# VIS4ROB-lab/covins

Measured on AMD Instinct MI355X. Metric: GBA iterations/sec, 5-agent EuRoC merged map, higher is better.
Workload: dtype f64

## Files before the change

### covins_amd/csrc/common.hpp

```cpp
#pragma once
#include <hip/hip_runtime.h>
#include <algorithm>
#include <atomic>
#include <cstdlib>
#include <stdint.h>

#include <map>
#include <unordered_map>
#include <utility>
#include <vector>

#include "../../include/covgpu.h"
#include "batch_limits.hpp"

namespace covgpu {

constexpr int kEdgeRec = 132;
constexpr int kTile = 128;

struct DevProblem {
  int K, A, L, O, I, E, S;
  int D;
  int n;
  int npad;
// ... 29 lines not shown
  double *imu_noise;
  double *pre_delta;
  double *pre_J;
  double *pre_P;
  double *pre_W;
  double *pre_bias;
  double *imu_Jw;

  int *edge_i, *edge_j;
  double *edge_meas, *edge_sqrt_info, *edge_loss_a;

  int nchains;
  int max_chain_len;
  int* perm;
  int* pos_kf;
  int* chain_ptr;
  int* pos_chain_end;

  double* Sred;
  double* bred;
  double *Ad, *Ae;
  double *Bp, *Bs, *Bn;
  int* pos_chain_begin;
  double* bp;
  double* grad;
  double* hdiag;
  double* HllInv;
  double* gn;
  double* step;
  double* vtmp;
  double* Linv;
  double* scal;
  double* part;
  int part_n, part_imu, part_edge, part_vec;
  double *imuAd, *imuBs, *imuCd, *imuG;
  double* edgeOut;
  int *kf_edge_ptr, *kf_edge_ent;
  int nepairs;
  int *epair_ptr, *epair_i, *epair_j, *epair_ent;
  int* flag;

  int shard;
  double* vw;

  int nd, nd_nnodes, nd_nlev, nd_maxd;
  int *nd_vnode, *nd_voff, *nd_vord;
  int *nd_vown;
  int *nd_ndepth, *nd_nI;
  long long* nd_ntab;
  int* nd_abase;
  int* nd_fidx;
  double *nd_M, *nd_rhs, *nd_Linv;
  double* nd_dummy;

  double* tr;
  double* scal_r; int* flag_r;

  int uni;
  int* cam_model;
  double* cam_xi;
};

enum {
  TR_RADIUS = 0, TR_MU, TR_LMDF, TR_COST, TR_ALPHA, TR_GG, TR_GN2, TR_GDOT, TR_DNORM, TR_CG, TR_CN, TR_MODEL, TR_SN, TR_RHO, TR_COSTNEW,
  TR_OK, TR_VALID, TR_ACC, TR_TERM, TR_FNCONV, TR_RETRY, TR_FIRST, TR_INITCOST, TR_REUSE,
  TR_JA, TR_JB, TR_JC, TR_VV, TR_VG, TR_NN, TR_XN2,
  TR_COUNT = 32
};
static_assert(TR_XN2 < TR_COUNT, "trust-region state slots");
struct TrConsts {
  int strategy;
  double max_radius, min_relative_decrease, function_tolerance, parameter_tolerance, gradient_tolerance;
};

__device__ __forceinline__ double* nd_entry(const DevProblem& P, int va, int vb, int ra, int rb) {
  const int na = P.nd_vnode[va], nb = P.nd_vnode[vb];
  if (na < 0 || nb < 0) return P.nd_dummy;
  if (na == nb) {
    const int oa = P.nd_voff[va] + ra, ob = P.nd_voff[vb] + rb;
    const int hi = oa > ob ? oa : ob, lo = oa > ob ? ob : oa;
    return P.nd_M + P.nd_ntab[2 * na] + (size_t)hi * (size_t)P.nd_ntab[2 * na + 1] + lo;
  }
  const int da = P.nd_ndepth[na], db = P.nd_ndepth[nb];
  const int no = da > db ? na : nb, vo = da > db ? va : vb, ro = da > db ? ra : rb;
  const int vA = da > db ? vb : va, rA = da > db ? rb : ra, dA = da > db ? db : da;
  const int base = P.nd_abase[(size_t)no * P.nd_maxd + dA];
  const int row = base < 0 ? -1 : P.nd_fidx[base + P.nd_vord[vA]];
  if (row < 0) return P.nd_dummy;
  return P.nd_M + P.nd_ntab[2 * no] + (size_t)(row + rA) * (size_t)P.nd_ntab[2 * no + 1] + (P.nd_voff[vo] + ro);
}

__device__ __forceinline__ double* c_entry(const DevProblem& P, int pi, int pj, int r, int c) {
  if (P.nd) return nd_entry(P, 2 * pi, 2 * pj, r, c);
  return P.Sred + (size_t)(6 * pi + r) * P.npad + (6 * pj + c);
}

enum { SC_COST = 0, SC_JV2 = 1, SC_GG = 2, SC_GN2 = 3, SC_GDOT = 4, SC_GMAX = 5, SC_GS = 6, SC_SN2 = 7, SC_XN2 = 8,
       SC_VV = 9, SC_VG = 10, SC_NN = 11, SC_JA = 12, SC_JB = 13, SC_JC = 14,
       SC_COUNT = 16 };

struct CholAux;
inline bool first_use_on_device(std::atomic<unsigned long long>& seen) {
  int d = 0;
  if (hipGetDevice(&d) != hipSuccess || d < 0 || d > 63) return true;
  const unsigned long long bit = 1ull << d;
  return (seen.fetch_or(bit, std::memory_order_acq_rel) & bit) == 0;
}
struct DevSignal { long long* flag = nullptr; long long seq = 0; };
inline int env_int(const char* name, int fallback) {
  const char* e = getenv(name);
  return e != nullptr ? atoi(e) : fallback;
}
size_t pair_order_slots(int npairs);
void launch_kobs_build(const DevProblem& P, int* pair_oa, int* pair_ob, size_t nent, hipStream_t st);
void launch_lm_lin(const DevProblem& P, double mu, hipStream_t st, DevSignal sig = DevSignal());
void launch_lm_build(const DevProblem& P, double mu, hipStream_t st, hipEvent_t pose_system_cleared = nullptr, hipStream_t side = nullptr,
                     hipEvent_t ev_lin = nullptr, hipEvent_t ev_kf = nullptr, CholAux* ax = nullptr);
void launch_lm_backsub(const DevProblem& P, const double* dp, double* out_all, hipStream_t st);
void launch_obs_jvp(const DevProblem& P, const double* v_all, hipStream_t st);
void launch_obs_cost(const DevProblem& P, const double* pose, const double* lm, hipStream_t st);
void launch_obs_linearize(const DevProblem& P, double* r, double* Jp, double* Jl, double* cost, hipStream_t st);
void launch_obs_norms(const DevProblem& P, double* norms, hipStream_t st);
void launch_lm_outliers(const DevProblem& P, double th, unsigned char* erase, int* left, unsigned long long* counts, hipStream_t st);

void launch_preintegrate(const DevProblem& P, hipStream_t st);
void launch_imu_build(const DevProblem& P, hipStream_t st);
void launch_imu_jvp(const DevProblem& P, const double* v_all, hipStream_t st);
void launch_imu_cost(const DevProblem& P, const double* pose, const double* sb, hipStream_t st);
void launch_imu_linearize(const DevProblem& P, double* r, double* J, hipStream_t st);

void launch_edge_build(const DevProblem& P, hipStream_t st);
void launch_edge_jvp(const DevProblem& P, const double* v_all, hipStream_t st);
void launch_edge_cost(const DevProblem& P, const double* pose, hipStream_t st);
void launch_edge_linearize(const DevProblem& P, double* r, double* J, double* cost, hipStream_t st);

void launch_finalize_diag(const DevProblem& P, double mu, int which, hipStream_t st);
void launch_part_clear(const DevProblem& P, int slot0, int nslots, hipStream_t st);
void launch_part_finish(const DevProblem& P, int slot0, int nslots, hipStream_t st);
void launch_imu_gather(const DevProblem& P, int which, hipStream_t st);
void launch_edge_gather(const DevProblem& P, hipStream_t st);
void launch_pose_finish(const DevProblem& P, double mu, hipStream_t st);
struct PgoPlan;
void launch_pose_graph_solve(const DevProblem& P, double* dst, hipStream_t st, CholAux& ax, PgoPlan* pgo);
void launch_zero_system(const DevProblem& P, hipStream_t st);
enum KernelForm {
  KF_POTRF_PANEL = 0, KF_POTRF_PANEL_FRONTS, KF_POTRF_PANEL4, KF_POTRF_PANEL4_FRONTS, KF_POTRF_SKIPPED,
  KF_TRSM_SUB4_4, KF_TRSM_SUB4_8, KF_TRSM_SUB4_12, KF_TRSM_SUB4_16,
  KF_GEMM_TRI_FULL, KF_GEMM_TRI_QUAD, KF_GEMM_TRI_GRID, KF_GEMM_RECT_FULL, KF_GEMM_RECT_QUAD, KF_DIAG_UPDATE,
  KF_BULK_ONE_LAUNCH, KF_BULK_TWO_LAUNCHES, KF_LAST_UPDATE_WHOLE, KF_LAST_UPDATE_SPLIT, KF_PANEL_ONE_TILE, KF_KD_CUT, KF_KD_ZERO, KF_GEMM_BETA0,
  KF_BWD_FRONT, KF_BWD_PIPE, KF_BWD_PIPE64, KF_BWD_TREE, KF_BWD_TREE64, KF_BWD_GIVEN, KF_BWD_STEP_SUB,
  KF_ND_EXTEND_REC, KF_ND_EXTEND, KF_ND_EXTEND_SPLIT,
  KF_ND_TOP_PACK, KF_ND_GH, KF_ND_TOP_DAMP, KF_ND_PANEL_XFER, KF_DIST_PANEL,
  KF_PGO_ARROW, KF_PGO_DENSE,
  KF_COUNT
};
extern const char* const kFormNames[KF_COUNT];
struct FormCensus { long long n[KF_COUNT] = {}; };
extern thread_local FormCensus* t_forms;
inline void form_hit(int f, long long k = 1) { if (t_forms != nullptr) t_forms->n[f] += k; }
struct FormScope {
  FormCensus* prev;
  explicit FormScope(FormCensus* c) : prev(t_forms) { t_forms = c; }
  ~FormScope() { t_forms = prev; }
  FormScope(const FormScope&) = delete; FormScope& operator=(const FormScope&) = delete;
};
struct CholAux {
  hipStream_t aux = nullptr, mid = nullptr, head = nullptr;
  hipEvent_t ev_fill = nullptr;
  hipEvent_t ev_xb = nullptr;
  int* bwd_cnt = nullptr;
  double* bwd_scr = nullptr; size_t bwd_scr_elems = 0;
  double* bwd_pipe = nullptr; size_t bwd_pipe_elems = 0;
  bool pipe_broken = false;
  hipEvent_t ev_xa = nullptr;
  hipEvent_t ev_zero = nullptr;
  hipEvent_t ev_lin = nullptr, ev_kf = nullptr;
  std::vector<hipEvent_t> ev, prof_ev, panel_ev;
  std::vector<double> prof_flops;
  std::vector<hipEvent_t> prof_ev2;
  std::vector<double> prof_flops2;
  double potrf_ms = 0, potrf_flops = 0;
  long n_potrf = 0;
  struct TriCache {
    std::vector<int*> list; std::vector<int> count; int key = -1;
    std::vector<int*> listC; std::vector<int> countC;
    int *listA = nullptr, *listB = nullptr; int countA = 0, countB = 0;
    void clear();
  };
  FormCensus forms;
  TriCache tri0;
  std::vector<TriCache> tri_lev;
  void tri_clear();
  void (*reduce)(void* ctx, double* dev, size_t n, int op, hipStream_t st) = nullptr;
  void* reduce_ctx = nullptr;
  int panel_n = 0;
  std::vector<int> panel_tag;
  void mark(hipStream_t s, int tag);
  bool profile = false;
  double syrk_ms = 0, syrk_flops = 0;
  long n_syrk = 0;
  void init();
  void destroy();
  void collect();
  static constexpr int kGateSlots = 16384;
  bool gates_on = false, gates_broken = false;
  long long* gate_flags = nullptr;
  int* gate_dead = nullptr;
  int* gate_dead_h = nullptr;
  std::unordered_map<hipEvent_t, int> gate_slot;
  std::map<std::pair<hipEvent_t, hipStream_t>, int> gate_slot_es;
  std::vector<long long> gate_seq;
  long long gate_counter = 0;
  double gate_timeout_s = 3.0;
  long gate_signals = 0, gate_waits = 0;
  void record(hipEvent_t e, hipStream_t s, int tag = 0);
  void wait(hipStream_t s, hipEvent_t e0, hipEvent_t e1 = nullptr, hipEvent_t e2 = nullptr, hipEvent_t e3 = nullptr);
  DevSignal publish_handle(hipEvent_t e, hipStream_t s, int tag = 0);
  void record_handle(DevSignal d, hipStream_t s);
  void sync(hipStream_t s, hipEvent_t r0, int tag0, hipEvent_t r1, int tag1, hipEvent_t w0 = nullptr, hipEvent_t w1 = nullptr, hipEvent_t w2 = nullptr,
            hipEvent_t w3 = nullptr);
  int gate_slot_of(hipEvent_t e, hipStream_t s);
  long long* gate_log = nullptr; int gate_log_n = 0;
  std::vector<int> gate_log_tag; std::vector<char> gate_log_kind; std::vector<int> gate_tag_of_slot;
  static constexpr int kGateLogMax = 16384;
  bool gate_failed() const { return gate_dead_h != nullptr && *(volatile int*)gate_dead_h != 0; }
  void gates_disable();
};
struct BwdXfer {
  const int* gidx = nullptr;
  const int *own_g = nullptr, *st_g = nullptr, *own_dims = nullptr, *st_dims = nullptr;
  double* x = nullptr;
  int first = 0;
};
struct DenseBatch {
  int n = 0; size_t sM = 0, sL = 0, sR = 0;
  const int* live = nullptr; int tI = 0; const int* live_h = nullptr;
  const long long* tab = nullptr;
  int tri_slot = -1;
  BwdXfer xfer;
  int split_ta = 0;
  hipEvent_t pre_trsm = nullptr;
  int* bwd_cnt = nullptr;
  double* bwd_scr = nullptr;
  double* bwd_pipe = nullptr;
  int *pipe_dead = nullptr, *pipe_dead_h = nullptr; double pipe_timeout_s = 3.0;
  const int* own_dims_h = nullptr;
  const int* own_dims = nullptr;
  const int* beta0_off = nullptr; const int* beta0 = nullptr;
  const int* plist = nullptr; const int* pbig_h = nullptr; const int* psmall_h = nullptr;
  int own_max = 0;
};
void dense_cholesky_solve_raw(double* S, double* b, double* Linv, int* flag, int npad, hipStream_t st, CholAux& ax, int tstop = -1,
                              bool solve = true, DenseBatch bt = DenseBatch());
struct DistPanels {
  int np = 0;
  const int* const* tri = nullptr;
  const int* tri_cnt = nullptr;
  bool lead = false;
  void (*exchange)(void* ctx, int P) = nullptr;
  void* ctx = nullptr;
};
void dense_cholesky_dist(double* S, double* b, double* Linv, int* flag, int npad, hipStream_t st, CholAux& ax, int tstop, DenseBatch bt,
                         const DistPanels& d);
constexpr int kBwdFrontMaxTiles = 4;
constexpr int kBwdPipeMinTiles = 2;
bool bwd_pipe_on();
void dense_backward_solve(double* S, double* b, double* Linv, int npad, hipStream_t st, int tfact, int tend, DenseBatch bt = DenseBatch());
void launch_potrf_panel(double* S, size_t ld, int t0, int w, double* Linv, int* flag, double* b, int npad, int nbt, size_t sM, size_t sL, size_t sR,
                        hipStream_t st, const long long* btab = nullptr, int nb = -1, const int* own = nullptr, const int* list = nullptr, int n_big = 0,
                        int n_small = 0);
void launch_bwd_given(const double* S, size_t ld, int r0, int r1, double* y, double* x, int ncol, int nbt, size_t sM, size_t sR, hipStream_t st,
                      const long long* btab, const int* live, int tI, BwdXfer xf = BwdXfer());
void launch_bwd_front(const double* S, int tI, int ntiles, int nchunk, double* y, const double* Linv, int nbt, size_t sL, size_t sR, hipStream_t st,
                      const long long* btab, const int* live, BwdXfer xf, int* cnt, double* scr);
void launch_bwd_pipe(const double* S, int tI, int ntiles, int nchunk, double* y, const double* Linv, int nbt, size_t sL, size_t sR, hipStream_t st,
                     const long long* btab, const int* live, BwdXfer xf, double* pipe, int* dead, int* dead_h, double timeout_s);
void launch_pipe_fill(double* buf, size_t n, hipStream_t st);
constexpr int kBwdTreeMax = 8;
constexpr int kPipeChunk = 128;
struct BwdTreeLevel {
  int nbt, T, nchunk, tI, first;
  double* y; size_t bsR; const double* Dinv; size_t bsL; const long long* btab; const int* live;
  size_t scr_off, xpub_off;
};
void launch_bwd_tree(const double* M, const BwdTreeLevel* lev, int nlev, BwdXfer xf, double* pipe, int* dead, int* dead_h, double timeout_s, hipStream_t st,
                     bool form64 = false);
unsigned long long pipe_empty_word();
void launch_trsm_sub(double* S, size_t ld, int t0, int w, int r0, int r1, const double* Linv, double* b, int npad, int nbt, size_t sM, size_t sL,
                     size_t sR, const int* live, int tI, hipStream_t st, bool chain = false, const long long* btab = nullptr, int nb = -1, const int* own = nullptr);
void launch_bwd_step_sub(const double* S, size_t ld, int p, const double* Linv_p, double* y, double* x, int ncol, int nblocks, int nbt, size_t sM,
                         size_t sL, size_t sR, hipStream_t st, const long long* btab = nullptr, const int* live = nullptr, int tI = 0,
                         BwdXfer xf = BwdXfer());

struct PgoHostPlan { std::vector<std::vector<int>> block_kf; std::vector<int> border_kf; };
bool pgo_plan_analyse(int K, int E, const int* ei, const int* ej, PgoHostPlan& out);
struct PgoPlan {
  bool active = false;
  int nblk = 0, nIpad = 0, ntot = 0;
  int nb = 0;
  int* idx = nullptr;
  double *M = nullptr, *rhs = nullptr, *Linv = nullptr;
  int* idx_b = nullptr;
  double *Sb = nullptr, *rhs_b = nullptr, *Linv_b = nullptr;
};
void launch_pgo_block_solve(const DevProblem& P, PgoPlan& plan, hipStream_t st, CholAux& ax);

struct PairLists {
  int npairs = 0; size_t nent = 0;
  int *pair_ptr = nullptr, *pair_i = nullptr, *pair_j = nullptr;
  int *pair_oa = nullptr, *pair_ob = nullptr;
};
bool build_pairs_device(int L, int K, const int* d_lm_obs_ptr, const int* d_obs_kf, const int* d_key_of_kf, bool want_obs, hipStream_t st, PairLists& out);
void launch_obs_unpack(int L, int O, const int* lm_obs_ptr, const double* uv, int* obs_lm, double* u, double* v, int* iota, hipStream_t st);
bool build_kf_lists_device(int O, int K, const int* d_obs_kf, const int* d_iota, int* kf_obs_ptr, int* kf_obs_idx, hipStream_t st);
struct Round2Lists {
  int L2 = 0, O2 = 0;
  double *lm0 = nullptr, *obs_u = nullptr, *obs_v = nullptr, *obs_sigma = nullptr;
  int *lm_obs_ptr = nullptr, *lm_old = nullptr, *obs_kf = nullptr, *obs_lm = nullptr, *kf_obs_ptr = nullptr, *kf_obs_idx = nullptr;
  void free_all() {
    for (void* q : {(void*)lm0, (void*)obs_u, (void*)obs_v, (void*)obs_sigma, (void*)lm_obs_ptr, (void*)lm_old, (void*)obs_kf, (void*)obs_lm, (void*)kf_obs_ptr, (void*)kf_obs_idx})
      if (q) (void)hipFree(q);
  }
};
bool round2_compact_device(int L, int O, int K, const unsigned char* d_erase, const int* d_left, const int* d_obs_kf, const int* d_obs_lm, const double* d_u,
                           const double* d_v, const double* d_sigma, const double* d_lm0, hipStream_t st, Round2Lists& out);

struct NdHostPlan;
constexpr int kExtRec = 144;
struct NdLevel {
  int n = 0, nI = 0, ntot = 0;
  int first = 0;
  size_t rhs_off = 0, linv_off = 0;
  int* live = nullptr;
  std::vector<int> live_h;
  int own_max = 0;
  int* plist = nullptr; std::vector<int> plist_h, pbig, psmall;
  int ext_first = 0, ext_count = 0;
  int ext_countA = 0;
  int split_ta = 0;
  int ext2_first = 0, ext2_count = 0, ext2_countA = 0;
  std::vector<int> dx_first, dx_nt, dx_nr, dt_first, dt_cnt;
  std::vector<const int*> dt_dev;
  int interior_tiles() const { return std::min(nI / kTile, (own_max + kTile - 1) / kTile); }
  int pipe_chunks() const { return (ntot - nI + kPipeChunk - 1) / kPipeChunk; }
  size_t pipe_scratch_elems() const { return (size_t)n * interior_tiles() * (pipe_chunks() + 1) * kTile; }
};
struct NdDev {
  bool active = false;
  int nnodes = 0;
  int top_lev0 = 0;
  std::vector<NdLevel> lev;
  int *own_dims = nullptr, *st_dims = nullptr, *own_g = nullptr, *st_g = nullptr;
  int *gidx = nullptr;
  int tree_levels = 0; int* tree_fill = nullptr; std::vector<int> h_tree_fill;
  int tree_top0 = 0;
  int *inv_off = nullptr, *inv = nullptr;
  int *rhs_node = nullptr;
  int *extw = nullptr, *extc = nullptr, *extc2 = nullptr;
  std::vector<int> h_extw, h_extc, h_extc2;
  int* extr = nullptr; size_t ext_over = 0; std::vector<int> h_extr;
  int *bb_off = nullptr, *bb = nullptr;
  int *top_var = nullptr, *top_r = nullptr, *top_g = nullptr;
  int ntop = 0;
  int* top_tiles = nullptr; int n_top_tiles = 0; double* top_pack = nullptr;
  std::vector<int> h_top_tiles;
  size_t M_sub = 0, rhs_top = 0, gh_off = 0;
  std::vector<int> h_vnode, h_voff, h_vord, h_vown, h_ndepth, h_nI, h_abase, h_fidx, h_own_dims, h_st_dims, h_own_g, h_st_g, h_gidx, h_inv_off, h_inv, h_rhs_node,
      h_top_var, h_top_r, h_top_g, h_bb_off, h_bb;
  std::vector<long long> h_ntab;
  bool dist = false, dist_lead = false;
  int* dist_ent = nullptr; int* dist_tri = nullptr; double* dist_buf = nullptr;
  std::vector<int> h_dist_ent, h_dist_tri;
  size_t dist_buf_elems = 0, dist_solve_elems = 0;
  size_t M_elems = 0, rhs_elems = 0, linv_elems = 0;
  double plan_flops = 0;
};
void nd_tables(const NdHostPlan& hp, const int* pos_kf, int D, int rank, NdDev& dev);
void launch_nd_init(const DevProblem& P, const NdDev& nd, hipStream_t st);
void launch_nd_zero(const DevProblem& P, const NdDev& nd, hipStream_t st);
bool launch_nd_solve(const DevProblem& P, NdDev& nd, double* dst, double mu, hipStream_t st, CholAux& ax);

void launch_tail_stats(const DevProblem& P, hipStream_t st);
void launch_tail_jvp(const DevProblem& P, bool two, hipStream_t st);
void launch_tail_cost(const DevProblem& P, hipStream_t st);
void launch_tail_finish(const DevProblem& P, TrConsts tc, int stage, bool two, bool with_logic, int fresh, hipStream_t st);
void launch_tail_logic(const DevProblem& P, TrConsts tc, int stage, int fresh, hipStream_t st);
void launch_tail_apply(const DevProblem& P, hipStream_t st);

void launch_dogleg_stats(const DevProblem& P, hipStream_t st);
void launch_cauchy_vec(const DevProblem& P, hipStream_t st);
void launch_combine_step(const DevProblem& P, double cg, double cn, hipStream_t st);
void launch_tr_after_solve(const DevProblem& P, TrConsts tc, int fresh, hipStream_t st);
void launch_combine_step_dev(const DevProblem& P, hipStream_t st);
void launch_tr_after_model(const DevProblem& P, TrConsts tc, hipStream_t st);
void launch_tr_decide(const DevProblem& P, TrConsts tc, hipStream_t st);
void launch_apply_step(const DevProblem& P, hipStream_t st);
void launch_accept(const DevProblem& P, hipStream_t st);
void launch_tr_accept(const DevProblem& P, hipStream_t st, double* box = nullptr, double seq = 0.0);
void launch_xnorm(const DevProblem& P, hipStream_t st);
void launch_relpose(int num, const int* ptr, const double* pB, const double* pA, const double* kpA, const double* kpB, const double* sigA,
                    const double* sigB, const double* camA, const int* distA, const double* camB, const int* distB, double th, int min_inliers,
                    double* T, unsigned char* outlier, int* inliers, hipStream_t st,
                    const int* modelA = nullptr, const double* xiA = nullptr, const int* modelB = nullptr, const double* xiB = nullptr);
void launch_abspose(int num, const int* ptr, const double* f, const double* P, const double* sig, const unsigned long long* seed, double* T,
                    unsigned char* inlier, int* inliers, int* iterations, int* best_draw, int min_inliers, int max_iterations, double probability,
                    double threshold, int max_n, hipStream_t st);
void launch_p3p(int num, const double* F, const double* P, double* T, int* nsol, int* chosen, hipStream_t st);
size_t match_assign_lds_bytes(int maxA, int maxB);
void launch_match(int mode, int num_jobs, int maxA, int maxB, const unsigned char* desc, const unsigned char* skip, const int* row_ptr,
                  const int* set_a, const int* set_b, const int* out_off, int* lists, int* match, int* dist, int* nmatches, int dcut,
                  float thr, float ratio, hipStream_t st);
size_t matchf_lds_bytes(int kp);
void launch_matchf_norms(int rows, int dim, const float* desc, float* norm, hipStream_t st);
void launch_matchf(int num_jobs, int maxA, int dim, const float* desc, const float* norm, const int* row_ptr, const int* set_a,
                   const int* set_b, const int* out_off, int* match, float* dist, int* nmatches, float thr, float ratio, hipStream_t st);
struct GuidedSets {
  const int4* kpr;
  const uint4* kdesc;
  const int* row_ptr;
  const int* perm;
  const double* bounds;
};
struct GuidedOptsDev { int th_low; double radius, scale_factor, log_sf; int num_octaves, agreement; };
struct GuidedSe3Args {
  GuidedSets S;
  const double* K; const double* lm_pos; const double* lm_maxd; const uint4* lm_desc; const unsigned char* lm_free;
  const int* set_1; const int* set_2; const double* T12; const int* off1; const int* off2;
  int* m1; int* m2; int* match; int* nfound;
};
struct GuidedProjArgs {
  GuidedSets S;
  const double* cam; const int* dist_type; const int* cam_model; const double* xi;
  const int* set; const double* T_cw; const int* point_ptr;
  const double* p_w; const double* normal; const double* min_d; const double* max_d; const uint4* p_desc; const unsigned char* skip;
  const int* existing;
  int* lists; int* cnt; float* target; double* rad; int* lvl; int* dold;
  int* claimed; int* remap_to; int* best_dist; int* nmatches;
};
void launch_guided_se3(const GuidedSe3Args& A, const GuidedOptsDev& O, int num_jobs, const int4* tiles, int num_tiles, hipStream_t st);
void launch_guided_projection(const GuidedProjArgs& A, const GuidedOptsDev& O, int num_jobs, const int4* tiles, int num_tiles, hipStream_t st);
struct BowVocabDev {
  int num_nodes;
  const int* child_ptr; const int* child; const uint4* desc; const int* word_id;
  const double* word_weight;
};
struct DetectOptsDev { int min_loop_dist, exclude_below, inter_only; };
struct DetectDev {
  int M;
  const int* id; const int* client; const int* vec_beg; const int* vec_end; const int* word; const double* value;
  const int* nb_beg; const int* nb_end; const int* nb;
  const int* con_beg; const int* con_end; const int* con; int con_by_query;
  const int* db_order; const int* pos_of;
  const unsigned char* dead;
  int tail;
  int inv_words; const int* inv_ptr; const int* inv_pos;
  const int* query_kf; const int* db_visible;
  double* min_score; int* max_common; int* num_sharing; int* num_scored; int* num_candidates; int* candidates; float* acc_score;
};
void launch_bow_transform(const BowVocabDev& V, const unsigned char* desc, const int* row_ptr, int num_sets, int rows, int nid_level,
                          int add_weight, int* row_word, int* row_node, int* out_word, double* out_value, int* count, hipStream_t st);
void launch_bow_score_pairs(const int* vec_beg, const int* vec_end, const int* word, const double* value, int num_pairs, const int* a,
                            const int* b, double* score, hipStream_t st);
void launch_bow_min_score(const DetectDev& D, int num_queries, const int* pair_off, const double* pair_score, double factor,
                          hipStream_t st);
void launch_bow_detect_chunk(const DetectDev& D, const DetectOptsDev& O, int q0, int nq, int cap, int hist_stride, int* common, int* first,
                             double* score, float* acc, int* best, int* order, int* hist, hipStream_t st);
constexpr int kBowDbNeighbours = 10;
struct BowDbDev {
  int* id; int* client; int* vec_beg; int* vec_end; int* pos_of; int* nb_beg; int* nb_end; int* nb;
  int* db_order; unsigned char* dead;
  int* word; double* value;
};
void launch_bowdb_tail_count(const DetectDev& D, int q0, int nq, int* common, int* first, hipStream_t st);
void launch_bowdb_store_meta(const BowDbDev& B, int n, const int* slot, const int* id, const int* client, const int* beg, const int* end,
                             hipStream_t st);
void launch_bowdb_gather(int num_sets, const int* row_ptr, const int* count, const int* dst, const int* src_word, const double* src_value,
                         int* pool_word, double* pool_value, hipStream_t st);
void launch_bowdb_set_neighbours(const BowDbDev& B, int n, const int* slot, const int* rows, const int* count, hipStream_t st);
void launch_bowdb_add(const BowDbDev& B, int n, const int* slot, int p0, hipStream_t st);
void launch_bowdb_erase(const BowDbDev& B, int n, const int* slot, hipStream_t st);
size_t bowdb_scan_tmp_ints(int n_out);
void launch_bowdb_scan(const int* in, int n_in, int* out, int n_out, int* tmp, hipStream_t st);
void launch_bowdb_renumber(const BowDbDev& B, int P, int* new_pos, int* new_order, int* scan_tmp, hipStream_t st);
void launch_bowdb_compact_pool(const BowDbDev& B, int num_slots, int* new_beg, int* new_word, double* new_value, int* scan_tmp,
                               hipStream_t st);
void launch_bowdb_histogram(const BowDbDev& B, int live, int* word_count, hipStream_t st);
void launch_bowdb_scatter(const BowDbDev& B, int live, int* cursor, int* inv_pos, hipStream_t st);
void launch_reanchor(int K, const double* pose_old, const double* pose_new, double* vel, int L, const int* ref, double* lm,
                     hipStream_t st);

struct PruneDev {
  int K, L;
  const int* lm_ptr; const int* obs_kf;
  const unsigned char* lm_invalid;
  const unsigned char* kf_invalid; const unsigned char* kf_first; const unsigned char* kf_loop; const unsigned char* kf_not_erase;
  const double* time;
  int* pred; int* succ;
  int* kf_ptr; int* kf_lm; int* cnt;
  int* lm_nobs;
  int* num; int* den; int* live; int* cand;
  int* out_num; int* out_den;
  int* round_kf; int* round_action; int cap;
  int* result;
};
struct PruneOptsDev { double th_red, max_time_dist; int max_kfs, max_rounds, valid0; };
void launch_prune_setup(const PruneDev& P, hipStream_t st);
void launch_prune_loop(const PruneDev& P, const PruneOptsDev& O, hipStream_t st);
void launch_prune_finish(const PruneDev& P, hipStream_t st);

constexpr int kLmrGroupMax = 64;
constexpr int kLmrLongThreads = 256;
constexpr int kLmrStage = 512;
constexpr int kLmrForms = 6;
struct LmRefreshDev {
  const int* lm_ptr; const int* obs_kf;
  const uint4* obs_desc;
  const int* obs_octave;
  const int* ref_obs;
  const double* pos; const double* center;
  const unsigned char* kf_invalid; const unsigned char* lm_invalid;
  const double* scale; int num_octaves;
  int* desc_obs; uint4* desc;
  double* normal; double* min_dist; double* max_dist;
  int* status;
};
void launch_lm_refresh(const LmRefreshDev& D, int lanes, const int* list, int count, hipStream_t st);

constexpr int kVtWaveMax = 256;
constexpr int kVtTile = 2048;
constexpr int kVtMaxK = 32;
constexpr int kVtThreads = 256;
struct VocTrainDev {
// ... 29 lines not shown
```

### covins_amd/csrc/k_chol.hip

```cpp
#include <algorithm>
#include <cstdio>
#include <cstdlib>
#include <mutex>

#include "common.hpp"
#include "dev_math.hpp"

namespace covgpu {
using namespace covdev;

typedef double v4f64 __attribute__((ext_vector_type(4)));

#ifdef COVGPU_PROBE
__device__ long long g_probe[8];
#define PROBE(i) do { if (threadIdx.x == 0) g_probe[i] = wall_clock64(); } while (0)
#define PROBE_ACC(i, t0) do { if (threadIdx.x == 0) g_probe[i] += wall_clock64() - (t0); } while (0)
#define PROBE_T0() wall_clock64()
#else
#define PROBE(i) do {} while (0)
#define PROBE_ACC(i, t0) do {} while (0)
#define PROBE_T0() 0
#endif

constexpr int KC = 16;
// ... 101 lines not shown
  bool fresh = false;
  if (MODE == MODE_SYRK_TRI && g.beta0 != nullptr && g.kcol0 == 0) {
    const int a = g.ra0 / kTile + ti - g.tI, b = g.cc0 / kTile + tj - g.tI;
    fresh = b >= 0 && a >= b && g.beta0[g.beta0_off[batch] + a * (a + 1) / 2 + b] == 0;
  }
  v4f64 acc[NMR][NMC];
#pragma unroll
  for (int tm = 0; tm < NMR; ++tm)
#pragma unroll
    for (int rg = 0; rg < 4; ++rg) {
      const unsigned rowoff = offc + (unsigned)(tm * 16 + 4 * rg) * ldab;
#pragma unroll
      for (int tn = 0; tn < NMC; ++tn) {
        if (fresh) acc[tm][tn][rg] = 0.0;
        else acc[tm][tn][rg] = *reinterpret_cast<const double*>(Cg + rowoff + tn * 128);
      }
    }
  const double sgn = -1.0;
  for (int kc0 = 0; kc0 < kend; kc0 += PF * KC) {
#pragma unroll
    for (int u = 0; u < PF; ++u) {
      const int kc = kc0 + u * KC;
      if (kc >= kend) break;
      lds_only_barrier();
#pragma unroll
      for (int it = 0; it < NPA; ++it) { sA[rbase + RPP * it][c2] = sgn * pa[u][it].x; sA[rbase + RPP * it][c2 + 1] = sgn * pa[u][it].y; }
#pragma unroll
      for (int it = 0; it < NPB; ++it) { sB[rbase + RPP * it][c2] = pb[u][it].x; sB[rbase + RPP * it][c2 + 1] = pb[u][it].y; }
      lds_only_barrier();
      if (kc + PF * KC < kend) gload(kc + PF * KC, u);
#pragma unroll
      for (int kk = 0; kk < KC; kk += 4) {
        double a[NMR], b[NMC];
#pragma unroll
        for (int t = 0; t < NMR; ++t) a[t] = sA[wr * WTR + t * 16 + fr][kk + fk];
#pragma unroll
        for (int t = 0; t < NMC; ++t) b[t] = sB[wc * WTC + t * 16 + fr][kk + fk];
#pragma unroll
        for (int tm = 0; tm < NMR; ++tm)
#pragma unroll
          for (int tn = 0; tn < NMC; ++tn) acc[tm][tn] = __builtin_amdgcn_mfma_f64_16x16x4f64(a[tm], b[tn], acc[tm][tn], 0, 0, 0);
      }
    }
  }
#pragma unroll
  for (int tm = 0; tm < NMR; ++tm)
#pragma unroll
    for (int rg = 0; rg < 4; ++rg) {
      const unsigned rowoff = offc + (unsigned)(tm * 16 + 4 * rg) * ldab;
#pragma unroll
      for (int tn = 0; tn < NMC; ++tn) *reinterpret_cast<double*>(Cg + rowoff + tn * 128) = acc[tm][tn][rg];
    }
}

template <int MODE>
__global__ __launch_bounds__(256, 2) void k_gemm_abt(GemmArgs g) { gemm_abt_body<MODE, kTile, kTile, KC, PFF>(g); }
template <int MODE, int TSA, int TSB>
__global__ __launch_bounds__(256, 2) void k_gemm_abt_q(GemmArgs g) { gemm_abt_body<MODE, TSA, TSB, KCQ, (MODE == MODE_SYRK_RECT ? PFR : PFQ)>(g); }

constexpr int kDiagSub = 32;
constexpr int kDiagChunks = 2 * kTile / KCQ;
__global__ __launch_bounds__(256, 2) void k_diag_update(GemmArgs g) {
  constexpr int LDQ = KCQ + kLdsPad;
  __builtin_amdgcn_s_setprio(3);
  const int batch = blockIdx.y;
  int bi = 0, bj = blockIdx.x;
  while (bj > bi) { bj -= bi + 1; ++bi; }
  const int ti = bi / (kTile / kDiagSub), tj = bj / (kTile / kDiagSub);
  if (g.live != nullptr) {
    if (!tile_live(g, batch, g.kcol0 / kTile)) return;
    if (!tile_live(g, batch, g.ra0 / kTile + ti)) return;
    if (!tile_live(g, batch, g.rb0 / kTile + tj)) return;
  }
  int kend = g.KD;
  if (g.own != nullptr) {
    const int real = g.own[batch] - g.kcol0;
    if (real <= 0) return;
    kend = min(kend, ((real + KCQ - 1) / KCQ) * KCQ);
  }
  __shared__ __attribute__((aligned(16))) double sbuf[2][2 * kDiagSub][LDQ];
  double* const Mb = g.M + (g.btab != nullptr ? (size_t)g.btab[2 * batch] : (size_t)batch * g.bsM);
  const size_t ld = g.btab != nullptr ? (size_t)g.btab[2 * batch + 1] : g.ld;
  const int tid = threadIdx.x, lane = tid & 63, wave = tid >> 6;
  const int wr = wave >> 1, wc = wave & 1;
  const char* Ag = reinterpret_cast<const char*>(Mb + (size_t)(g.ra0 + bi * kDiagSub) * ld + g.kcol0);
  const char* Bg = reinterpret_cast<const char*>(Mb + (size_t)(g.rb0 + bj * kDiagSub) * ld + g.kcol0);
  char* Cg = reinterpret_cast<char*>(Mb + (size_t)(g.ra0 + bi * kDiagSub) * ld + (size_t)(g.cc0 + bj * kDiagSub));
  const unsigned ldab = (unsigned)(ld * sizeof(double));
  constexpr int LPR = KCQ / 2, RPP = 256 / LPR, NPS = kDiagSub / RPP;
  const int c2 = (tid % LPR) * 2, rbase = tid / LPR;
  const unsigned offa = (unsigned)rbase * ldab + (unsigned)c2 * 8u;
  const int fr = lane & 15, fk = lane >> 4;
  const unsigned offc = (unsigned)(wr * 16 + fk) * ldab + (unsigned)(wc * 16 + fr) * 8u;
  v4f64 acc;
#pragma unroll
  for (int rg = 0; rg < 4; ++rg) acc[rg] = *reinterpret_cast<const double*>(Cg + offc + (unsigned)(4 * rg) * ldab);
  __builtin_amdgcn_sched_barrier(0);
  double2 pa[kDiagChunks][NPS], pb[kDiagChunks][NPS];
#pragma unroll
  for (int c = 0; c < kDiagChunks; ++c) {
    const size_t kcb = (size_t)min(c * KCQ, kend - KCQ) * sizeof(double);
#pragma unroll
    for (int it = 0; it < NPS; ++it) {
      pa[c][it] = *reinterpret_cast<const double2*>(Ag + kcb + (size_t)(RPP * it) * ldab + offa);
      pb[c][it] = *reinterpret_cast<const double2*>(Bg + kcb + (size_t)(RPP * it) * ldab + offa);
    }
  }
  __builtin_amdgcn_sched_barrier(0);
#pragma unroll
  for (int c = 0; c < kDiagChunks; ++c) {
    if (c * KCQ >= kend) break;
    double (*sA)[LDQ] = sbuf[c & 1];
    double (*sB)[LDQ] = sbuf[c & 1] + kDiagSub;
#pragma unroll
    for (int it = 0; it < NPS; ++it) {
      sA[rbase + RPP * it][c2] = -pa[c][it].x; sA[rbase + RPP * it][c2 + 1] = -pa[c][it].y;
      sB[rbase + RPP * it][c2] = pb[c][it].x; sB[rbase + RPP * it][c2 + 1] = pb[c][it].y;
    }
    lds_only_barrier();
#pragma unroll
    for (int kk = 0; kk < KCQ; kk += 4)
      acc = __builtin_amdgcn_mfma_f64_16x16x4f64(sA[wr * 16 + fr][kk + fk], sB[wc * 16 + fr][kk + fk], acc, 0, 0, 0);
  }
#pragma unroll
  for (int rg = 0; rg < 4; ++rg) *reinterpret_cast<double*>(Cg + offc + (unsigned)(4 * rg) * ldab) = acc[rg];
}

static const int kQuarterMax = env_int("COVGPU_QUARTER_MAX", 1024);
constexpr int kRectQuarterMax = 512;
static const double kChainPairs = getenv("COVGPU_CHAIN_PAIRS") ? atof(getenv("COVGPU_CHAIN_PAIRS")) : 0.0;
static const bool kTracePanels = getenv("COVGPU_TRACE_PANELS") != nullptr;
static const bool kTraceKernels = env_int("COVGPU_TRACE_PANELS", 0) >= 2;
constexpr size_t kLdsFull = (size_t)2 * kTile * LDT * sizeof(double);
constexpr size_t kLdsQuarter = (size_t)(64 + 64) * (KCQ + kLdsPad) * sizeof(double);

static hipStream_t make_side_stream(int priority) {
  hipStream_t s2 = nullptr;
  (void)hipStreamCreateWithPriority(&s2, hipStreamNonBlocking, priority);
  return s2;
}

void CholAux::init() {
  int lo = 0, hi = 0;
  (void)hipDeviceGetStreamPriorityRange(&lo, &hi);
  if (!head) (void)hipStreamCreateWithPriority(&head, hipStreamNonBlocking, hi);
  if (!mid) mid = make_side_stream(hi);
  if (!aux) aux = make_side_stream(lo);
  if (!ev_zero) (void)hipEventCreateWithFlags(&ev_zero, hipEventDisableTiming);
  if (!ev_lin) (void)hipEventCreateWithFlags(&ev_lin, hipEventDisableTiming);
  if (!ev_kf) (void)hipEventCreateWithFlags(&ev_kf, hipEventDisableTiming);
  if (!ev_fill) (void)hipEventCreateWithFlags(&ev_fill, hipEventDisableTiming);
  if (!ev_xb) (void)hipEventCreateWithFlags(&ev_xb, hipEventDisableTiming);
  if (!ev_xa) (void)hipEventCreateWithFlags(&ev_xa, hipEventDisableTiming);
  if (!bwd_cnt && hipMalloc((void**)&bwd_cnt, 65536 * sizeof(int)) == hipSuccess) (void)hipMemset(bwd_cnt, 0, 65536 * sizeof(int));
  if (!gate_dead && hipMalloc((void**)&gate_dead, sizeof(int)) == hipSuccess) (void)hipMemset(gate_dead, 0, sizeof(int));
  if (!gate_dead_h && hipHostMalloc((void**)&gate_dead_h, 4 * sizeof(int), hipHostMallocDefault) == hipSuccess) gate_dead_h[0] = gate_dead_h[1] = gate_dead_h[2] = gate_dead_h[3] = 0;
  if (const char* e = getenv("COVGPU_GATE_TIMEOUT_S")) gate_timeout_s = std::max(getenv("COVGPU_GATE_TIMEOUT_MIN") ? atof(getenv("COVGPU_GATE_TIMEOUT_MIN")) : 0.01, atof(e));
  if (!gate_flags && !gates_broken) {
    static const bool want = env_int("COVGPU_GATES", 1) != 0;
    if (want && gate_dead != nullptr && gate_dead_h != nullptr && hipMalloc((void**)&gate_flags, kGateSlots * sizeof(long long)) == hipSuccess) {
      (void)hipMemset(gate_flags, 0, kGateSlots * sizeof(long long));
      (void)hipDeviceSynchronize();
      gates_on = true;
      if (getenv("COVGPU_GATE_LOG") && hipMalloc((void**)&gate_log, 2 * (size_t)kGateLogMax * sizeof(long long)) != hipSuccess) gate_log = nullptr;
    } else gates_broken = true;
  }
}
__global__ void k_signal(long long* flag, long long seq, long long* log) {
  if (threadIdx.x == 0) {
    __hip_atomic_store(flag, seq, __ATOMIC_RELAXED, __HIP_MEMORY_SCOPE_AGENT);
    if (log) log[0] = wall_clock64();
  }
}
__global__ void k_signal2(DevSignal a, DevSignal b) {
  if (threadIdx.x != 0) return;
  if (a.flag != nullptr) __hip_atomic_store(a.flag, a.seq, __ATOMIC_RELAXED, __HIP_MEMORY_SCOPE_AGENT);
  if (b.flag != nullptr) __hip_atomic_store(b.flag, b.seq, __ATOMIC_RELAXED, __HIP_MEMORY_SCOPE_AGENT);
}
struct GateArgs { const long long* f[4]; long long s[4]; int n; int* dead; int* dead_h; long long limit; long long* log; long long* pf[2]; long long ps[2]; int np; const long long* base; };
__global__ void k_gate(GateArgs g) {
  if (threadIdx.x != 0) return;
  for (int i = 0; i < g.np; ++i) __hip_atomic_store(g.pf[i], g.ps[i], __ATOMIC_RELAXED, __HIP_MEMORY_SCOPE_AGENT);
  const long long t0 = wall_clock64();
  struct Stamp { long long* log; long long t0; __device__ ~Stamp() { if (log) { log[0] = t0; log[1] = wall_clock64(); } } } stamp{g.log, t0};
  for (int i = 0; i < g.n; ++i) {
    unsigned spins = 0;
    while (__hip_atomic_load(g.f[i], __ATOMIC_RELAXED, __HIP_MEMORY_SCOPE_AGENT) < g.s[i]) {
      __builtin_amdgcn_s_sleep(1);
      if ((++spins & 127u) == 0) {
        if (__hip_atomic_load(g.dead, __ATOMIC_RELAXED, __HIP_MEMORY_SCOPE_AGENT) != 0) return;
        if (wall_clock64() - t0 > g.limit) {
          __hip_atomic_store(g.dead, 1, __ATOMIC_RELAXED, __HIP_MEMORY_SCOPE_AGENT);
          __hip_atomic_store(g.dead_h + 1, (int)(g.f[i] - g.base), __ATOMIC_RELAXED, __HIP_MEMORY_SCOPE_SYSTEM);
          __hip_atomic_store(g.dead_h + 2, (int)g.s[i], __ATOMIC_RELAXED, __HIP_MEMORY_SCOPE_SYSTEM);
          __hip_atomic_store(g.dead_h + 3, (int)__hip_atomic_load(g.f[i], __ATOMIC_RELAXED, __HIP_MEMORY_SCOPE_AGENT), __ATOMIC_RELAXED, __HIP_MEMORY_SCOPE_SYSTEM);
          __hip_atomic_store(g.dead_h, 1, __ATOMIC_RELEASE, __HIP_MEMORY_SCOPE_SYSTEM);
          return;
        }
      }
    }
  }
}
int CholAux::gate_slot_of(hipEvent_t e, hipStream_t s) {
  const std::pair<hipEvent_t, hipStream_t> key(e, s);
  auto it = gate_slot_es.find(key);
  int slot;
  if (it != gate_slot_es.end()) slot = it->second;
  else {
    slot = (int)gate_slot_es.size();
    if (slot >= kGateSlots) return -1;
    gate_slot_es.emplace(key, slot);
    if ((int)gate_seq.size() <= slot) gate_seq.resize(slot + 1, 0);
  }
  gate_slot[e] = slot;
  return slot;
}
void CholAux::record(hipEvent_t e, hipStream_t s, int tag) {
  if (!gates_on) { (void)hipEventRecord(e, s); return; }
  const int slot = gate_slot_of(e, s);
  if (slot < 0) { gate_slot.erase(e); (void)hipEventRecord(e, s); return; }
  gate_seq[slot] = ++gate_counter;
  long long* lg = nullptr;
  if ((int)gate_tag_of_slot.size() <= slot) gate_tag_of_slot.resize(slot + 1, 0);
  gate_tag_of_slot[slot] = tag;
  if (gate_log != nullptr && gate_log_n < kGateLogMax) { lg = gate_log + 2 * (size_t)gate_log_n++; gate_log_tag.push_back(tag); gate_log_kind.push_back('S'); }
  hipLaunchKernelGGL(k_signal, dim3(1), dim3(64), 0, s, gate_flags + slot, gate_seq[slot], lg);
  ++gate_signals;
}
DevSignal CholAux::publish_handle(hipEvent_t e, hipStream_t s, int tag) {
  DevSignal d;
  if (!gates_on) return d;
  const int slot = gate_slot_of(e, s);
  if (slot < 0) { gate_slot.erase(e); return d; }
  gate_seq[slot] = ++gate_counter;
  if ((int)gate_tag_of_slot.size() <= slot) gate_tag_of_slot.resize(slot + 1, 0);
  gate_tag_of_slot[slot] = tag;
  d.flag = gate_flags + slot; d.seq = gate_seq[slot];
  ++gate_signals;
  return d;
}
void CholAux::record_handle(DevSignal d, hipStream_t s) { if (d.flag != nullptr) hipLaunchKernelGGL(k_signal2, dim3(1), dim3(64), 0, s, d, DevSignal()); }
void CholAux::wait(hipStream_t s, hipEvent_t e0, hipEvent_t e1, hipEvent_t e2, hipEvent_t e3) { sync(s, nullptr, 0, nullptr, 0, e0, e1, e2, e3); }
void CholAux::sync(hipStream_t s, hipEvent_t r0, int tag0, hipEvent_t r1, int tag1, hipEvent_t e0, hipEvent_t e1, hipEvent_t e2, hipEvent_t e3) {
  hipEvent_t es[4] = {e0, e1, e2, e3};
  if (!gates_on) {
    if (r0 != nullptr) record(r0, s, tag0);
    if (r1 != nullptr) record(r1, s, tag1);
    for (hipEvent_t e : es) if (e != nullptr) (void)hipStreamWaitEvent(s, e, 0);
    return;
  }
  GateArgs g; g.n = 0; g.dead = gate_dead; g.dead_h = gate_dead_h; g.limit = (long long)(gate_timeout_s * 1e8); g.log = nullptr; g.np = 0; g.base = gate_flags;
  g.pf[0] = g.pf[1] = nullptr; g.ps[0] = g.ps[1] = 0;
  {
    hipEvent_t rs[2] = {r0, r1}; const int tags[2] = {tag0, tag1};
    for (int i = 0; i < 2; ++i) {
      if (rs[i] == nullptr) continue;
      const int slot = gate_slot_of(rs[i], s);
      if (slot < 0) { gate_slot.erase(rs[i]); (void)hipEventRecord(rs[i], s); continue; }
      gate_seq[slot] = ++gate_counter;
      if ((int)gate_tag_of_slot.size() <= slot) gate_tag_of_slot.resize(slot + 1, 0);
      gate_tag_of_slot[slot] = tags[i];
      g.pf[g.np] = gate_flags + slot; g.ps[g.np] = gate_seq[slot]; ++g.np; ++gate_signals;
    }
  }
  int first_tag = g.np > 0 ? -(r0 != nullptr ? tag0 : tag1) : 0;
  for (hipEvent_t e : es) {
    if (e == nullptr) continue;
    auto it = gate_slot.find(e);
    if (it == gate_slot.end()) { (void)hipStreamWaitEvent(s, e, 0); continue; }
    if (gate_seq[it->second] == 0) continue;
    if (g.n == 0 && g.np == 0 && it->second < (int)gate_tag_of_slot.size()) first_tag = gate_tag_of_slot[it->second];
    g.f[g.n] = gate_flags + it->second; g.s[g.n] = gate_seq[it->second]; ++g.n;
  }
  if (g.n == 0 && g.np == 0) return;
  if (gate_log != nullptr && gate_log_n < kGateLogMax) { g.log = gate_log + 2 * (size_t)gate_log_n++; gate_log_tag.push_back(first_tag); gate_log_kind.push_back('G'); }
  for (int i = g.n; i < 4; ++i) { g.f[i] = nullptr; g.s[i] = 0; }
  hipLaunchKernelGGL(k_gate, dim3(1), dim3(64), 0, s, g);
  ++gate_waits;
}
void CholAux::gates_disable() {
  gates_on = false; gates_broken = true;
  pipe_broken = true;
  if (bwd_pipe) { launch_pipe_fill(bwd_pipe, bwd_pipe_elems, nullptr); (void)hipDeviceSynchronize(); }
  gate_slot.clear(); gate_slot_es.clear(); gate_seq.clear();
  if (gate_dead) (void)hipMemset(gate_dead, 0, sizeof(int));
  if (gate_dead_h) *gate_dead_h = 0;
}
void CholAux::TriCache::clear() {
  for (int* p : list) if (p) (void)hipFree(p);
  for (int* p : listC) if (p) (void)hipFree(p);
  listC.clear(); countC.clear();
  if (listA) (void)hipFree(listA);
  if (listB) (void)hipFree(listB);
  listA = listB = nullptr; countA = countB = 0;
  list.clear(); count.clear(); key = -1;
}
void CholAux::tri_clear() {
  tri0.clear();
  for (auto& t : tri_lev) t.clear();
}
void CholAux::destroy() {
  tri_clear();
  if (mid) { (void)hipStreamDestroy(mid); mid = nullptr; }
  if (head) { (void)hipStreamDestroy(head); head = nullptr; }
  for (auto e : ev) (void)hipEventDestroy(e);
  for (auto e : prof_ev) (void)hipEventDestroy(e);
  for (auto e : prof_ev2) (void)hipEventDestroy(e);
  prof_ev2.clear();
  for (auto e : panel_ev) (void)hipEventDestroy(e);
  panel_ev.clear();
  ev.clear(); prof_ev.clear();
  if (ev_zero) { (void)hipEventDestroy(ev_zero); ev_zero = nullptr; }
  if (ev_lin) { (void)hipEventDestroy(ev_lin); ev_lin = nullptr; }
  if (ev_kf) { (void)hipEventDestroy(ev_kf); ev_kf = nullptr; }
  if (ev_fill) { (void)hipEventDestroy(ev_fill); ev_fill = nullptr; }
  if (ev_xb) { (void)hipEventDestroy(ev_xb); ev_xb = nullptr; }
  if (ev_xa) { (void)hipEventDestroy(ev_xa); ev_xa = nullptr; }
  if (bwd_cnt) { (void)hipFree(bwd_cnt); bwd_cnt = nullptr; }
  if (gate_flags) { (void)hipFree(gate_flags); gate_flags = nullptr; }
  if (gate_dead) { (void)hipFree(gate_dead); gate_dead = nullptr; }
  if (gate_log) { (void)hipFree(gate_log); gate_log = nullptr; }
  if (gate_dead_h) { (void)hipHostFree(gate_dead_h); gate_dead_h = nullptr; }
  gates_on = false; gate_slot.clear(); gate_slot_es.clear(); gate_seq.clear();
  if (bwd_scr) { (void)hipFree(bwd_scr); bwd_scr = nullptr; bwd_scr_elems = 0; }
  if (bwd_pipe) { (void)hipFree(bwd_pipe); bwd_pipe = nullptr; bwd_pipe_elems = 0; }
  if (aux) { (void)hipStreamDestroy(aux); aux = nullptr; }
}
void CholAux::mark(hipStream_t s, int tag) {
  if (!kTracePanels) return;
  while ((int)panel_ev.size() <= panel_n) { hipEvent_t e; (void)hipEventCreate(&e); panel_ev.push_back(e); }
  if ((int)panel_tag.size() <= panel_n) panel_tag.resize(panel_n + 1);
  (void)hipEventRecord(panel_ev[panel_n], s);
  panel_tag[panel_n++] = tag;
}
void CholAux::collect() {
  if (panel_n > 1) {
    fprintf(stderr, "covgpu marks [us]:");
    for (int i = 1; i < panel_n; ++i) {
      float ms = 0;
      if (hipEventElapsedTime(&ms, panel_ev[0], panel_ev[i]) == hipSuccess) fprintf(stderr, " %d:%.0f", panel_tag[i], ms * 1e3);
    }
    fprintf(stderr, "\n");
  }
  panel_n = 0;
  if (gate_log != nullptr && gate_log_n > 0) {
    std::vector<long long> h(2 * (size_t)gate_log_n);
    (void)hipMemcpy(h.data(), gate_log, h.size() * sizeof(long long), hipMemcpyDeviceToHost);
    long long t0 = h[0];
    for (int i = 0; i < gate_log_n; ++i) t0 = std::min(t0, h[2 * i]);
    fprintf(stderr, "covgpu gate log [us]:");
    for (int i = 0; i < gate_log_n; ++i) {
      if (gate_log_kind[i] == 'S') fprintf(stderr, " S%d@%.1f", gate_log_tag[i], (h[2 * i] - t0) * 0.01);
      else fprintf(stderr, " G%d@%.1f+%.1f", gate_log_tag[i], (h[2 * i] - t0) * 0.01, (h[2 * i + 1] - h[2 * i]) * 0.01);
    }
    fprintf(stderr, "\n");
    gate_log_n = 0; gate_log_tag.clear(); gate_log_kind.clear();
  }
  if (!profile) return;
  for (size_t i = 0; i < prof_flops.size(); ++i) {
    float ms = 0;
    if (hipEventElapsedTime(&ms, prof_ev[2 * i], prof_ev[2 * i + 1]) != hipSuccess) continue;
    syrk_ms += ms; syrk_flops += prof_flops[i]; n_syrk++;
  }
  prof_flops.clear();
  for (size_t i = 0; i < prof_flops2.size(); ++i) {
    float ms = 0;
    if (hipEventElapsedTime(&ms, prof_ev2[2 * i], prof_ev2[2 * i + 1]) != hipSuccess) continue;
    potrf_ms += ms; potrf_flops += prof_flops2[i]; n_potrf++;
  }
  prof_flops2.clear();
}

thread_local FormCensus* t_forms = nullptr;
const char* const kFormNames[KF_COUNT] = {
  "k_potrf_panel", "k_potrf_panel.fronts", "k_potrf_panel4", "k_potrf_panel4.fronts", "potrf_skipped",
  "k_trsm_sub4<4>", "k_trsm_sub4<8>", "k_trsm_sub4<12>", "k_trsm_sub4<16>",
  "k_gemm_abt.tri", "k_gemm_abt_q.tri", "k_gemm_abt.tri_grid", "k_gemm_abt.rect", "k_gemm_abt_q.rect", "k_diag_update",
  "bulk_one_launch", "bulk_two_launches", "last_update_whole", "last_update_split", "panel_one_tile", "kd_cut", "kd_zero", "gemm_beta0",
  "k_bwd_front", "k_bwd_pipe", "k_bwd_pipe64", "k_bwd_tree", "k_bwd_tree64", "k_bwd_given", "k_bwd_step_sub",
  "k_nd_extend_rec", "k_nd_extend", "nd_extend_split",
  "k_nd_top_pack", "k_nd_gh", "k_nd_top_damp", "k_nd_panel_xfer", "dist_panel",
  "pgo_arrow", "pgo_dense",
};
static_assert(sizeof(kFormNames) / sizeof(kFormNames[0]) == KF_COUNT, "one name per kernel form");

struct ProfBracket {
  std::vector<hipEvent_t>* ev = nullptr; std::vector<double>* flops; hipStream_t s; double fl;
  ProfBracket(bool on, std::vector<hipEvent_t>& ev_, std::vector<double>& flops_, hipStream_t s_, double fl_) : flops(&flops_), s(s_), fl(fl_) {
    if (!on) return;
    ev = &ev_;
    while (ev->size() < 2 * (flops->size() + 1)) { hipEvent_t e; (void)hipEventCreate(&e); ev->push_back(e); }
    (void)hipEventRecord((*ev)[2 * flops->size()], s);
  }
  ~ProfBracket() { if (ev != nullptr) { (void)hipEventRecord((*ev)[2 * flops->size() + 1], s); flops->push_back(fl); } }
  ProfBracket(const ProfBracket&) = delete; ProfBracket& operator=(const ProfBracket&) = delete;
};

static std::vector<int> live_tile_list(const DenseBatch& bt, int nbt, int T, int t0, int tb, int part) {
  std::vector<int> q[8];
  for (int a = 0; a < nbt; ++a) {
    const int nI = bt.live_h[2 * a], nO = bt.live_h[2 * a + 1];
    if (t0 >= nI) continue;
    auto live = [&](int t) { return t < nI || (t >= bt.tI && t - bt.tI < nO); };
    const int nt = T - tb, Ts = (nt + 7) / 8;
    for (int si = 0; si < Ts; ++si)
      for (int sj = 0; sj <= si; ++sj) {
        std::vector<int> grp;
        for (int i = 8 * si; i < std::min(nt, 8 * si + 8); ++i)
          for (int j = 8 * sj; j < std::min(i + 1, 8 * sj + 8); ++j)
            if (live(tb + i) && live(tb + j) && (part == 0 || (part <= 2 && (i < bt.split_ta) == (part == 1)) || (part >= 3 && (j < 2 || i < bt.split_ta) == (part == 3)))) grp.push_back((a << 20) | (i << 10) | j);
        if (grp.empty()) continue;
        int best = 0;
        for (int x = 1; x < 8; ++x) if (q[x].size() < q[best].size()) best = x;
        q[best].insert(q[best].end(), grp.begin(), grp.end());
      }
  }
  size_t longest = 0;
  for (int x = 0; x < 8; ++x) longest = std::max(longest, q[x].size());
  std::vector<int> lst(8 * longest, -1);
  for (int x = 0; x < 8; ++x) for (size_t k = 0; k < q[x].size(); ++k) lst[8 * k + x] = q[x][k];
  return lst;
}
static bool upload_list(const std::vector<int>& lst, int*& d_out, int& n_out) {
  d_out = nullptr; n_out = 0;
  if (lst.empty()) return true;
  if (hipMalloc((void**)&d_out, lst.size() * sizeof(int)) != hipSuccess) { d_out = nullptr; return false; }
  (void)hipMemcpy(d_out, lst.data(), lst.size() * sizeof(int), hipMemcpyHostToDevice);
  n_out = (int)lst.size();
  return true;
}

struct PanelRun {
  double* S; double* b; double* Linv; int* flag;
  int npad, T, NP, Pstop, nbt; size_t ld;
  const DenseBatch& bt; CholAux& ax; CholAux::TriCache& tc;
  const bool chain;
  hipStream_t M, H, R, B;
  hipEvent_t* eH = nullptr;
  hipEvent_t* eB = nullptr;
  hipEvent_t* eC = nullptr;
  hipEvent_t* e1 = nullptr;
  hipEvent_t* e2 = nullptr;
  hipEvent_t* e3 = nullptr;
  hipEvent_t* eRc = nullptr;
  hipEvent_t* eHp = nullptr;
  hipEvent_t* eA = nullptr;
  int Plast;
  bool split_last = false;
  bool tail_on_chain = false;

  static CholAux::TriCache& tri_cache_of(CholAux& ax, const DenseBatch& bt) {
    if (bt.tri_slot >= (int)ax.tri_lev.size()) ax.tri_lev.resize(bt.tri_slot + 1);
    return bt.tri_slot >= 0 ? ax.tri_lev[bt.tri_slot] : ax.tri0;
  }
  PanelRun(double* S_, double* b_, double* Linv_, int* flag_, int npad_, hipStream_t st, CholAux& ax_, int tstop, const DenseBatch& bt_, bool chain_)
      : S(S_), b(b_), Linv(Linv_), flag(flag_), npad(npad_), T(npad_ / kTile), NP((T + 1) / 2), Pstop((tstop >= 0 && tstop < T) ? tstop / 2 : NP),
        nbt(bt_.n > 0 ? bt_.n : 1), ld((size_t)npad_), bt(bt_), ax(ax_), tc(tri_cache_of(ax_, bt_)), chain(chain_), Plast(NP - 1) {
    static std::atomic<unsigned long long> attr_seen{0};
    if (first_use_on_device(attr_seen)) {
      (void)hipFuncSetAttribute(reinterpret_cast<const void*>(k_gemm_abt<MODE_SYRK_TRI>), hipFuncAttributeMaxDynamicSharedMemorySize, (int)kLdsFull);
      (void)hipFuncSetAttribute(reinterpret_cast<const void*>(k_gemm_abt<MODE_SYRK_RECT>), hipFuncAttributeMaxDynamicSharedMemorySize, (int)kLdsFull);
    }
    ax.init();
    M = st; H = ax.head; R = ax.mid; B = ax.aux;
  }
  void set_up_events() {
    while ((int)ax.ev.size() < 9 * (NP + 1)) { hipEvent_t e; (void)hipEventCreateWithFlags(&e, hipEventDisableTiming); ax.ev.push_back(e); }
    hipEvent_t** const roles[9] = {&eH, &eB, &eC, &e1, &e2, &e3, &eRc, &eHp, &eA};
    for (int r = 0; r < 9; ++r) *roles[r] = ax.ev.data() + r * (NP + 1);
  }
  static int tag(int P, int k) { return 100 * (P + 1) + k; }
  void trace(hipStream_t s, int P, int k) { if (kTraceKernels) ax.mark(s, tag(P, k)); }
  int width(int t0) const { return (T - t0 >= 2) ? 2 : 1; }
  int row_h0(int t0) const { return std::min(t0 + 2, T); }
  int row_h1(int t0) const { return std::min(t0 + 4, T); }

  int kd(int P) const {
    const int full = std::min(2, T - 2 * P) * kTile;
    if (bt.own_max <= 0) return full;
    return std::max(0, std::min(full, ((bt.own_max - 2 * P * kTile + 31) / 32) * 32));
  }
  int kd_front(int P, int a, int chunk) const {
    if (bt.own_dims_h == nullptr) return kd(P);
    const int real = bt.own_dims_h[a] - 2 * P * kTile;
    return real <= 0 ? 0 : std::min(kd(P), ((real + chunk - 1) / chunk) * chunk);
  }
  int nbp(int t0, int w) const { return bt.own_max > 0 ? std::max(0, std::min(8 * w, (bt.own_max - t0 * kTile + 15) / 16)) : -1; }
  GemmArgs gemm_args(int kt0, int KD, int row_tile0, int col_tile0, int nt, bool trailing = false) const {
    GemmArgs g{};
    g.M = S; g.ld = ld; g.kcol0 = kt0 * kTile; g.KD = KD;
    g.ra0 = row_tile0 * kTile; g.rb0 = g.cc0 = col_tile0 * kTile; g.nt = nt;
    g.bsM = bt.sM; g.bsL = bt.sL; g.bsR = bt.sR; g.live = bt.live; g.tI = bt.tI; g.btab = bt.tab; g.own = bt.own_dims;
    if (trailing && chain) { g.beta0_off = bt.beta0_off; g.beta0 = bt.beta0; }
    return g;
  }

  void potrf(int t0, int w, hipStream_t s) {
    const int P = t0 / 2, nb = nbp(t0, w);
    const bool timed = chain && ax.profile && nb != 0;
    if (chain && w == 1) form_hit(KF_PANEL_ONE_TILE);
    if (chain && T > t0 + w) {
      if (kd(P) == 0) form_hit(KF_KD_ZERO);
      else if (kd(P) < w * kTile) form_hit(KF_KD_CUT);
    }
    double fl = 0.0;
    for (int a = 0; timed && a < nbt; ++a) {
      const double n = bt.own_dims_h != nullptr ? (double)std::max(0, std::min(w * kTile, bt.own_dims_h[a] - t0 * kTile)) : (double)(w * kTile);
      fl += n * n * n / 3.0 + n * n;
    }
    ProfBracket prof(timed, ax.prof_ev2, ax.prof_flops2, s, fl);
    if (bt.plist != nullptr) launch_potrf_panel(S, ld, t0, w, Linv, flag, b, npad, nbt, bt.sM, bt.sL, bt.sR, s, bt.tab, nb, bt.own_dims, bt.plist, bt.pbig_h[P], bt.psmall_h[P]);
    else launch_potrf_panel(S, ld, t0, w, Linv, flag, b, npad, nbt, bt.sM, bt.sL, bt.sR, s, bt.tab, nb);
  }
  void trsm(int t0, int w, int r0, int r1, hipStream_t s, bool on_chain, double* rhs) {
    launch_trsm_sub(S, ld, t0, w, r0, r1, Linv, rhs, npad, nbt, bt.sM, bt.sL, bt.sR, bt.live, bt.tI, s, on_chain, bt.tab, nbp(t0, w), bt.own_dims);
  }
  void rect(int r0, int r1, int tc0, int ntc, int kt0, int KD, hipStream_t s, bool quad) {
    if (r1 <= r0 || ntc <= 0 || KD <= 0) return;
    const GemmArgs g = gemm_args(kt0, KD, r0, tc0, r1 - r0);
    form_hit(quad ? KF_GEMM_RECT_QUAD : KF_GEMM_RECT_FULL);
    if (quad) hipLaunchKernelGGL((k_gemm_abt_q<MODE_SYRK_RECT, 64, 64>), dim3(ntc, r1 - r0, 4 * nbt), dim3(256), kLdsQuarter, s, g);
    else hipLaunchKernelGGL(k_gemm_abt<MODE_SYRK_RECT>, dim3(ntc, r1 - r0, nbt), dim3(256), kLdsFull, s, g);
  }
  void diag(int u0, int uw, int kt0, int KD, hipStream_t s) {
    if (bt.tab == nullptr) { rect(u0, u0 + uw, u0, uw, kt0, KD, s, true); return; }
    if (uw <= 0 || KD <= 0) return;
    const int nb = uw * (kTile / kDiagSub);
    form_hit(KF_DIAG_UPDATE);
    hipLaunchKernelGGL(k_diag_update, dim3(nb * (nb + 1) / 2, nbt), dim3(256), 0, s, gemm_args(kt0, KD, u0, u0, uw));
  }
  void tri_update(hipStream_t s, const int* list, int count, int P, int tb) {
    const int nt = T - tb;
    GemmArgs g = gemm_args(2 * P, kd(P), tb, tb, nt, true);
    g.tri = list;
    form_hit(list == nullptr ? KF_GEMM_TRI_GRID : count <= kQuarterMax ? KF_GEMM_TRI_QUAD : KF_GEMM_TRI_FULL);
// ... 235 lines not shown
```

### covins_amd/csrc/k_front.hip

```cpp
#include <algorithm>

#include "common.hpp"
#include "dev_math.hpp"

namespace covgpu {

struct NdLevArgs {
  int first, n, nI, ntot;
  double* rhs;
  const int *own_dims, *st_dims, *own_g, *st_g, *gidx, *inv_off, *inv;
};

struct NdZeroArgs { int nlev; int first[24], n[24], nI[24], T[24]; long long blk0[25]; const int *own_dims, *st_dims, *bb_off, *bb; int first_top; };
__global__ __launch_bounds__(256) void k_nd_zero(DevProblem P, NdZeroArgs z) {
  int l = 0;
  while (l + 1 < z.nlev && (long long)blockIdx.x >= z.blk0[l + 1]) ++l;
  const int T = z.T[l];
  const int q = (int)((long long)blockIdx.x - z.blk0[l]);
  const int fz = q / (T * T), rem = q - fz * T * T, tr = rem / T, tc = rem - tr * T;
  if (tc > tr) return;
  const int node = z.first[l] + fz;
  const int own_n = z.own_dims[node];
  const int nIt = z.nI[l] / kTile, lo2 = own_n <= kTile ? 1 : 2 * ((own_n + 2 * kTile - 1) / (2 * kTile)), lb = (z.st_dims[node] + kTile - 1) / kTile;
  auto live = [&](int t) { return t < lo2 || (t >= nIt && t - nIt < lb); };
  const bool pad_diag = tr >= lo2 && tr < nIt && tc >= (tr & ~1);
  if (!((live(tr) && live(tc)) || pad_diag)) return;
  if (z.bb != nullptr && tc >= nIt && (node < z.first_top || !z.bb[z.bb_off[node] + (tr - nIt) * (tr - nIt + 1) / 2 + (tc - nIt)])) return;
  const size_t ld = (size_t)P.nd_ntab[2 * node + 1];
  double* M = P.nd_M + P.nd_ntab[2 * node] + (size_t)tr * kTile * ld + (size_t)tc * kTile;
  const int own = z.own_dims[node];
  for (int e = threadIdx.x; e < kTile * kTile / 2; e += 256) {
    const int r = e / (kTile / 2), c2 = 2 * (e - r * (kTile / 2));
    double2 v = {0.0, 0.0};
    if (tr == tc && tr < nIt) {
      const int gr = tr * kTile + r;
      if (gr >= own) { if (c2 == r) v.x = 1.0; if (c2 + 1 == r) v.y = 1.0; }
    }
    *reinterpret_cast<double2*>(M + (size_t)r * ld + c2) = v;
  }
}

__global__ __launch_bounds__(256) void k_nd_assemble(DevProblem P, const int* __restrict__ rhs_off, double* __restrict__ x, const int* __restrict__ fill, int nfill,
                                                      unsigned long long empty) {
  const int t = blockIdx.x * blockDim.x + threadIdx.x;
  if (t < nfill) reinterpret_cast<unsigned long long*>(x)[fill[t]] = empty;
  if (P.vi) {
    const int pos = t / 324, e = t - 324 * pos;
    if (pos < P.K) {
      const int vs = 2 * pos + 1;
      const bool head = pos == P.pos_chain_begin[pos], tail = pos + 1 == P.pos_chain_end[pos];
      if (e < 81) {
        const int r = e / 9, c = e - 9 * r;
        if (c <= r) *nd_entry(P, vs, vs, r, c) = P.Ad[(size_t)81 * pos + e];
      } else if (e < 162) {
        const int q = e - 81, r = q / 9, c = q - 9 * r;
        if (!head) *nd_entry(P, vs, vs - 2, r, c) = P.Ae[(size_t)81 * pos + q];
      } else {
        const int q = e - 162, w = q / 54, k = q - 54 * w, r = k / 6, c = k - 6 * r;
        if (w == 0) *nd_entry(P, vs, 2 * pos, r, c) = P.Bs[(size_t)54 * pos + k];
        else if (w == 1) { if (!head) *nd_entry(P, vs, 2 * (pos - 1), r, c) = P.Bp[(size_t)54 * pos + k]; }
        else if (!tail) *nd_entry(P, vs, 2 * (pos + 1), r, c) = P.Bn[(size_t)54 * pos + k];
      }
    }
  }
  if (t < P.n) {
    const int kf = t / P.D, r = t - kf * P.D, pos = P.perm[kf];
    const int v = r < 6 ? 2 * pos : 2 * pos + 1, rr = r < 6 ? r : r - 6;
    const int node = P.nd_vnode[v];
    if (node >= 0) P.nd_rhs[rhs_off[node] + P.nd_voff[v] + rr] = P.bred[t];
  }
}

__global__ __launch_bounds__(256) void k_nd_extend(DevProblem P, NdLevArgs a, const int* __restrict__ work, const int* __restrict__ child, int second_pass, int store_border, DevSignal sig) {
  if (sig.flag != nullptr && blockIdx.x == 0 && threadIdx.x == 0) __hip_atomic_store(sig.flag, sig.seq, __ATOMIC_RELAXED, __HIP_MEMORY_SCOPE_AGENT);
  const int4 w0 = reinterpret_cast<const int4*>(work)[2 * (size_t)blockIdx.x], w1 = reinterpret_cast<const int4*>(work)[2 * (size_t)blockIdx.x + 1];
  const size_t foff = (size_t)(unsigned)w0.x | ((size_t)(unsigned)w0.y << 32);
  const size_t ld = (size_t)w0.z;
  const int rhs_p = w0.w, tr = w1.x, tc = w1.y, kbeg = w1.z, kend = w1.w;
  const int ty = threadIdx.x >> 4, tx = threadIdx.x & 15;
  double* F = P.nd_M + foff;
  const int nrow = (int)ld;
  int rr[4], cc[4];
#pragma unroll
  for (int i = 0; i < 4; ++i) { rr[i] = 64 * tr + ty + 16 * i; cc[i] = 64 * tc + tx + 16 * i; }
  struct Ch { size_t moff; int ldc, rhs, inv; };
  auto load_ch = [&](int k) {
    const int2* q = reinterpret_cast<const int2*>(child) + 3 * (size_t)k;
    const int2 a0 = q[0], a1 = q[1], a2 = q[2];
    Ch c; c.moff = (size_t)(unsigned)a0.x | ((size_t)(unsigned)a0.y << 32); c.ldc = a1.x; c.rhs = a1.y; c.inv = a2.x;
    return c;
  };
  Ch c1 = {0, 0, 0, 0}, c2 = {0, 0, 0, 0};
  if (kbeg < kend) c1 = load_ch(kbeg);
  if (kbeg + 1 < kend) c2 = load_ch(kbeg + 1);
  double v[4][4], rv[4] = {0.0, 0.0, 0.0, 0.0};
  bool hit[4][4];
  const bool own_cols = second_pass != 0 || 64 * tc < a.nI;
#pragma unroll
  for (int i = 0; i < 4; ++i)
#pragma unroll
    for (int j = 0; j < 4; ++j) {
      v[i][j] = (own_cols && rr[i] < nrow && cc[j] <= rr[i]) ? F[(size_t)rr[i] * ld + cc[j]] : 0.0;
      hit[i][j] = false;
    }
  int irn[4], icn[4];
  auto load_maps = [&](const Ch& c) {
    const int* inv = a.inv + c.inv;
#pragma unroll
    for (int i = 0; i < 4; ++i) { irn[i] = rr[i] < nrow ? inv[rr[i]] : -1; icn[i] = cc[i] < nrow ? inv[cc[i]] : -1; }
  };
  if (kbeg < kend) load_maps(c1);
  for (int k = kbeg; k < kend; ++k) {
    const Ch c = c1;
    c1 = c2;
    if (k + 2 < kend) c2 = load_ch(k + 2);
    const double* C = P.nd_M + c.moff;
    const size_t ldc = (size_t)c.ldc;
    int ir[4], ic[4];
#pragma unroll
    for (int i = 0; i < 4; ++i) { ir[i] = irn[i]; ic[i] = icn[i]; }
    if (k + 1 < kend) load_maps(c1);
#pragma unroll
    for (int i = 0; i < 4; ++i) {
      if (ir[i] < 0) continue;
      if (tr == tc && tx == 0) rv[i] += P.nd_rhs[c.rhs + ir[i]];
#pragma unroll
      for (int j = 0; j < 4; ++j) {
        if (ic[j] < 0 || cc[j] > rr[i]) continue;
        v[i][j] += C[(size_t)(ir[i] > ic[j] ? ir[i] : ic[j]) * ldc + (ir[i] > ic[j] ? ic[j] : ir[i])];
        hit[i][j] = true;
      }
    }
  }
  const bool store_all = !own_cols && store_border != 0;
#pragma unroll
  for (int i = 0; i < 4; ++i) {
#pragma unroll
    for (int j = 0; j < 4; ++j) if (hit[i][j] || (store_all && rr[i] < nrow && cc[j] <= rr[i])) F[(size_t)rr[i] * ld + cc[j]] = v[i][j];
    if (rv[i] != 0.0) P.nd_rhs[rhs_p + rr[i]] += rv[i];
  }
}

__global__ __launch_bounds__(256) void k_nd_extend_rec(DevProblem P, NdLevArgs a, const int* __restrict__ recs, const int* __restrict__ over, int second_pass, int store_border, DevSignal sig) {
  if (sig.flag != nullptr && blockIdx.x == 0 && threadIdx.x == 0) __hip_atomic_store(sig.flag, sig.seq, __ATOMIC_RELAXED, __HIP_MEMORY_SCOPE_AGENT);
  const int* rec = recs + (size_t)kExtRec * blockIdx.x;
  const int ty = threadIdx.x >> 4, tx = threadIdx.x & 15;
  const int4 w0 = reinterpret_cast<const int4*>(rec)[0], w1 = reinterpret_cast<const int4*>(rec)[1];
  int4 chn = reinterpret_cast<const int4*>(rec)[2];
  int irn[4], icn[4];
#pragma unroll
  for (int i = 0; i < 4; ++i) { irn[i] = rec[16 + ty + 16 * i]; icn[i] = rec[80 + tx + 16 * i]; }
  const size_t foff = (size_t)(unsigned)w0.x | ((size_t)(unsigned)w0.y << 32);
  const size_t ld = (size_t)w0.z;
  const int rhs_p = w0.w, tr = w1.x, tc = w1.y, nrec = w1.z, next = w1.w;
  double* F = P.nd_M + foff;
  const int nrow = (int)ld;
  int rr[4], cc[4];
#pragma unroll
  for (int i = 0; i < 4; ++i) { rr[i] = 64 * tr + ty + 16 * i; cc[i] = 64 * tc + tx + 16 * i; }
  double v[4][4], rv[4] = {0.0, 0.0, 0.0, 0.0};
  bool hit[4][4];
  const bool own_cols = second_pass != 0 || 64 * tc < a.nI;
#pragma unroll
  for (int i = 0; i < 4; ++i)
#pragma unroll
    for (int j = 0; j < 4; ++j) {
      v[i][j] = (own_cols && rr[i] < nrow && cc[j] <= rr[i]) ? F[(size_t)rr[i] * ld + cc[j]] : 0.0;
      hit[i][j] = false;
    }
  for (int k = 0; k < nrec; ++k) {
    const double* C = P.nd_M + ((size_t)(unsigned)chn.x | ((size_t)(unsigned)chn.y << 32));
    const size_t ldc = (size_t)chn.z;
    const int crhs = chn.w;
    int ir[4], ic[4];
#pragma unroll
    for (int i = 0; i < 4; ++i) { ir[i] = irn[i]; ic[i] = icn[i]; }
    if (k + 1 < nrec) {
      const int* r2 = over + (size_t)kExtRec * (next + k);
      chn = reinterpret_cast<const int4*>(r2)[2];
#pragma unroll
      for (int i = 0; i < 4; ++i) { irn[i] = r2[16 + ty + 16 * i]; icn[i] = r2[80 + tx + 16 * i]; }
    }
#pragma unroll
    for (int i = 0; i < 4; ++i) {
      if (ir[i] < 0) continue;
      if (tr == tc && tx == 0) rv[i] += P.nd_rhs[crhs + ir[i]];
#pragma unroll
      for (int j = 0; j < 4; ++j) {
        if (ic[j] < 0 || cc[j] > rr[i]) continue;
        v[i][j] += C[(size_t)(ir[i] > ic[j] ? ir[i] : ic[j]) * ldc + (ir[i] > ic[j] ? ic[j] : ir[i])];
        hit[i][j] = true;
      }
    }
  }
  const bool store_all = !own_cols && store_border != 0;
#pragma unroll
  for (int i = 0; i < 4; ++i) {
#pragma unroll
    for (int j = 0; j < 4; ++j) if (hit[i][j] || (store_all && rr[i] < nrow && cc[j] <= rr[i])) F[(size_t)rr[i] * ld + cc[j]] = v[i][j];
    if (rv[i] != 0.0) P.nd_rhs[rhs_p + rr[i]] += rv[i];
  }
}

__global__ __launch_bounds__(256) void k_nd_linv_init(double* __restrict__ Linv, size_t n) {
  const size_t q = (size_t)blockIdx.x * 256 + threadIdx.x;
  if (q < n) { const int e = (int)(q & 255); Linv[q] = ((e >> 4) == (e & 15)) ? 1.0 : 0.0; }
}

__global__ __launch_bounds__(256) void k_nd_gh(DevProblem P, const int* __restrict__ top_g, int ntop, double* __restrict__ buf, int dir) {
  const int i = blockIdx.x * blockDim.x + threadIdx.x;
  if (i >= ntop) return;
  const int q = top_g[i];
  if (dir == 0) { buf[i] = P.grad[q]; buf[ntop + i] = P.hdiag[q]; }
  else { P.grad[q] = buf[i]; P.hdiag[q] = buf[ntop + i]; }
}
__global__ __launch_bounds__(256) void k_nd_top_pack(DevProblem P, const int* __restrict__ tiles, double* __restrict__ pack, int dir) {
  const int node = tiles[3 * blockIdx.x], tr = tiles[3 * blockIdx.x + 1], tc = tiles[3 * blockIdx.x + 2];
  const size_t ld = (size_t)P.nd_ntab[2 * node + 1];
  double* M = P.nd_M + P.nd_ntab[2 * node] + (size_t)tr * kTile * ld + (size_t)tc * kTile;
  double* B = pack + (size_t)blockIdx.x * kTile * kTile;
  for (int e = threadIdx.x; e < kTile * kTile / 2; e += 256) {
    const int r = e / (kTile / 2), c2 = 2 * (e - r * (kTile / 2));
    double2* m = reinterpret_cast<double2*>(M + (size_t)r * ld + c2);
    double2* b = reinterpret_cast<double2*>(B + (size_t)r * kTile + c2);
    if (dir == 0) *b = *m; else *m = *b;
  }
}
__global__ __launch_bounds__(256) void k_nd_top_damp(DevProblem P, const int* __restrict__ top_var, const int* __restrict__ top_r,
                                                      const int* __restrict__ top_g, int ntop, const int* __restrict__ rhs_off, double mu, int lead) {
  const int i = blockIdx.x * blockDim.x + threadIdx.x;
  if (i >= ntop) return;
  const int v = top_var[i], r = top_r[i];
  const double h = P.hdiag[top_g[i]];
  double* d = nd_entry(P, v, v, r, r);
  if (h == 0.0) { *d = lead ? 1.0 : 0.0; P.nd_rhs[rhs_off[P.nd_vnode[v]] + P.nd_voff[v] + r] = 0.0; }
  else if (lead) { const double c = covdev::clamp_diag(h); *d += mu * c * c; }
}
__global__ __launch_bounds__(256) void k_nd_panel_xfer(DevProblem P, const int4* __restrict__ ent, int ntile, double* __restrict__ buf,
                                                        const int* __restrict__ rhs_node, const int* __restrict__ own_dims, int dir, int lead) {
  const int4 e = ent[blockIdx.x];
  if ((int)blockIdx.x < ntile) {
    const size_t ld = (size_t)P.nd_ntab[2 * e.x + 1];
    double* M = P.nd_M + P.nd_ntab[2 * e.x] + (size_t)e.y * kTile * ld + (size_t)e.z * kTile;
    double* B = buf + (size_t)blockIdx.x * kTile * kTile;
    const int pad0 = (dir == 0 && !lead && e.y == e.z && e.y * kTile < P.nd_nI[e.x]) ? own_dims[e.x] - e.y * kTile : kTile;
    for (int q = threadIdx.x; q < kTile * kTile / 2; q += 256) {
      const int r = q / (kTile / 2), c2 = 2 * (q - r * (kTile / 2));
      double2* m = reinterpret_cast<double2*>(M + (size_t)r * ld + c2);
      double2* b = reinterpret_cast<double2*>(B + (size_t)r * kTile + c2);
      if (dir == 0) *b = r < pad0 ? *m : double2{0.0, 0.0};
      else *m = *b;
    }
  } else {
    double* R = P.nd_rhs + rhs_node[e.x] + e.y;
    double* B = buf + (size_t)ntile * kTile * kTile + (size_t)(blockIdx.x - ntile) * 256;
    const int t = threadIdx.x;
    if (t < e.z) { if (dir == 0) B[t] = R[t]; else R[t] = B[t]; }
  }
}

static const bool kLookahead = env_int("COVGPU_ND_LOOKAHEAD", 1) != 0;
static const bool kFusedBwd = env_int("COVGPU_ND_BWD_FUSED", 1) != 0;
static const bool kBwdTree = env_int("COVGPU_BWD_TREE", 1) != 0;
static const bool kExtRecords = env_int("COVGPU_EXT_RECORDS", 1) != 0;
static const bool kBeta0 = env_int("COVGPU_BETA0", 1) != 0;

static NdLevArgs lev_args(const DevProblem& P, const NdDev& nd, int l) {
  const NdLevel& L = nd.lev[l];
  return NdLevArgs{L.first, L.n, L.nI, L.ntot, P.nd_rhs + L.rhs_off, nd.own_dims, nd.st_dims, nd.own_g, nd.st_g, nd.gidx, nd.inv_off, nd.inv};
}

void launch_nd_init(const DevProblem& P, const NdDev& nd, hipStream_t st) {
  if (nd.linv_elems) hipLaunchKernelGGL(k_nd_linv_init, dim3((unsigned)((nd.linv_elems + 255) / 256)), dim3(256), 0, st, P.nd_Linv, nd.linv_elems);
}

void launch_nd_zero(const DevProblem& P, const NdDev& nd, hipStream_t st) {
  NdZeroArgs z;
  z.nlev = 0; z.blk0[0] = 0; z.own_dims = nd.own_dims; z.st_dims = nd.st_dims; z.bb_off = nd.bb_off; z.bb = kBeta0 ? nd.bb : nullptr;
  z.first_top = !kBeta0 ? 0 : (nd.top_lev0 < (int)nd.lev.size() ? nd.lev[nd.top_lev0].first : nd.nnodes);
  auto flush = [&] {
    if (z.nlev > 0 && z.blk0[z.nlev] > 0) hipLaunchKernelGGL(k_nd_zero, dim3((unsigned)z.blk0[z.nlev]), dim3(256), 0, st, P, z);
    z.nlev = 0; z.blk0[0] = 0;
  };
  for (size_t l = 0; l < nd.lev.size(); ++l) {
    const NdLevel& L = nd.lev[l];
    if (L.n == 0) continue;
    const int T = L.ntot / kTile;
    const long long nb = (long long)T * T * L.n;
    if (z.nlev == 24 || z.blk0[z.nlev] + nb > 0x7fffff00ll) flush();
    z.first[z.nlev] = L.first; z.n[z.nlev] = L.n; z.nI[z.nlev] = L.nI; z.T[z.nlev] = T;
    z.blk0[z.nlev + 1] = z.blk0[z.nlev] + nb;
    ++z.nlev;
  }
  flush();
}

struct FrontRun {
  const DevProblem& P; NdDev& nd; double* dst; const double mu; hipStream_t st; CholAux& ax;
  const int nlev, ltop;
  bool tree_on = false, tree_top_on = false;
  FrontRun(const DevProblem& P_, NdDev& nd_, double* dst_, double mu_, hipStream_t st_, CholAux& ax_)
      : P(P_), nd(nd_), dst(dst_), mu(mu_), st(st_), ax(ax_), nlev((int)nd_.lev.size()), ltop(nd_.top_lev0) {}
  bool ensure_scratch() {
    {
      size_t need = 0;
      for (const NdLevel& L : nd.lev)
        need = std::max(need, (size_t)L.n * std::min(kBwdFrontMaxTiles, (L.own_max + kTile - 1) / kTile) * std::max(1, (L.ntot - L.nI + 255) / 256) * kTile);
      if (need > ax.bwd_scr_elems) {
        if (ax.bwd_scr) (void)hipFree(ax.bwd_scr);
        ax.bwd_scr = nullptr; ax.bwd_scr_elems = 0;
        if (hipMalloc((void**)&ax.bwd_scr, need * sizeof(double)) != hipSuccess) { ax.bwd_scr = nullptr; return false; }
        ax.bwd_scr_elems = need;
      }
    }
    if (!ax.pipe_broken && ax.gate_dead != nullptr && ax.gate_dead_h != nullptr) {
      size_t need = 0, tree = 0, tree2 = 0;
      for (int l = 0; l < nlev; ++l) {
        const NdLevel& L = nd.lev[l];
        if (L.n > 0 && bwd_pipe_on() && L.interior_tiles() >= kBwdPipeMinTiles) need = std::max(need, L.pipe_scratch_elems());
        if (l < nd.tree_levels) tree += L.pipe_scratch_elems();
        if (l >= nd.tree_top0) tree2 += L.pipe_scratch_elems();
      }
      need = std::max(need, std::max(tree, tree2));
      if (need > ax.bwd_pipe_elems) {
        if (ax.bwd_pipe) { (void)hipDeviceSynchronize(); (void)hipFree(ax.bwd_pipe); }
        ax.bwd_pipe = nullptr; ax.bwd_pipe_elems = 0;
        if (hipMalloc((void**)&ax.bwd_pipe, need * sizeof(double)) == hipSuccess) {
          ax.bwd_pipe_elems = need;
          launch_pipe_fill(ax.bwd_pipe, need, st);
        } else ax.bwd_pipe = nullptr;
      }
    }
    const bool tree_ok = kBwdTree && kFusedBwd && nd.tree_fill != nullptr && !ax.pipe_broken && ax.bwd_pipe != nullptr && ax.gate_dead != nullptr && bwd_pipe_on();
    tree_on = tree_ok && nd.tree_levels >= 2;
    tree_top_on = tree_ok && nd.tree_top0 < nlev;
    return true;
  }
  void assemble() {
    ax.mark(st, -1);
    const int nfill = (tree_on || tree_top_on) ? (int)nd.h_tree_fill.size() : 0;
    const int cnt = std::max(std::max(P.vi ? 324 * P.K : 0, P.n), nfill);
    hipLaunchKernelGGL(k_nd_assemble, dim3((cnt + 255) / 256), dim3(256), 0, st, P, (const int*)nd.rhs_node, dst, (const int*)nd.tree_fill, nfill, pipe_empty_word());
    ax.mark(st, -2);
  }
  DenseBatch batch(int l) const {
    const NdLevel& L = nd.lev[l];
    DenseBatch bt;
    bt.n = L.n; bt.sM = 0; bt.sL = (size_t)L.nI * kTile; bt.sR = (size_t)2 * L.ntot;
    bt.live = L.live; bt.tI = L.nI / kTile; bt.live_h = L.live_h.data();
    if (kBeta0 && nd.bb != nullptr) { bt.beta0_off = nd.bb_off + L.first; bt.beta0 = nd.bb; }
    if (L.plist != nullptr) { bt.plist = L.plist; bt.pbig_h = L.pbig.data(); bt.psmall_h = L.psmall.data(); }
    bt.tab = P.nd_ntab + 2 * (size_t)L.first; bt.tri_slot = l; bt.own_max = L.own_max; bt.own_dims = nd.own_dims + L.first; bt.own_dims_h = nd.h_own_dims.data() + L.first;
    return bt;
  }
  BwdXfer xfer(int first) const {
    BwdXfer xf;
    xf.gidx = nd.gidx; xf.own_g = nd.own_g; xf.st_g = nd.st_g; xf.own_dims = nd.own_dims; xf.st_dims = nd.st_dims; xf.x = dst; xf.first = first;
    return xf;
  }
  bool extend(int l, bool top_children, int part, hipStream_t s2, DevSignal sig = DevSignal()) {
    const NdLevel& L = nd.lev[l];
    int first = top_children ? L.ext2_first : L.ext_first, count = top_children ? L.ext2_count : L.ext_count;
    const int countA = top_children ? L.ext2_countA : L.ext_countA;
    if (part == 1) count = countA;
    if (part == 2) { first += countA; count -= countA; }
    const bool records = kExtRecords && nd.extr != nullptr;
    const int store_border = (!top_children && l < ltop && kBeta0) ? 1 : 0;
    if (count > 0) { form_hit(records ? KF_ND_EXTEND_REC : KF_ND_EXTEND); if (part != 0) form_hit(KF_ND_EXTEND_SPLIT); }
    if (count > 0 && records)
      hipLaunchKernelGGL(k_nd_extend_rec, dim3(count), dim3(256), 0, s2, P, lev_args(P, nd, l), (const int*)(nd.extr + (size_t)kExtRec * first),
                         (const int*)(nd.extr + (size_t)kExtRec * nd.ext_over), top_children ? 1 : 0, store_border, sig);
    else if (count > 0)
      hipLaunchKernelGGL(k_nd_extend, dim3(count), dim3(256), 0, s2, P, lev_args(P, nd, l), (const int*)(nd.extw + 8 * (size_t)first),
                         (const int*)(top_children ? nd.extc2 : nd.extc), top_children ? 1 : 0, store_border, sig);
    return count > 0;
  }
  void factor(int l, bool split, hipEvent_t pre_trsm) {
    const NdLevel& L = nd.lev[l];
    ax.mark(st, -3);
    if (L.n > 0) {
      DenseBatch bt = batch(l);
      bt.split_ta = split ? L.split_ta : 0; bt.pre_trsm = pre_trsm;
      dense_cholesky_solve_raw(P.nd_M, P.nd_rhs + L.rhs_off, P.nd_Linv + L.linv_off, P.flag, L.ntot, st, ax, L.nI / kTile, false, bt);
    }
    ax.mark(st, -4);
  }
  void run_levels(int l0, int l1, bool top_children) {
    bool prev_split = false;
    for (int l = l0; l < l1; ++l) {
      hipEvent_t pre = nullptr;
      if (prev_split) {
        DevSignal sig = ax.publish_handle(ax.ev_xa, st, 5);
        const int cntA = top_children ? nd.lev[l].ext2_countA : nd.lev[l].ext_countA;
        if (sig.flag == nullptr || cntA <= 0) { if (sig.flag != nullptr) ax.record_handle(sig, st); else ax.record(ax.ev_xa, st, 5); sig = DevSignal(); }
        extend(l, top_children, 1, st, sig);
        ax.wait(ax.aux, ax.ev_xa);
        extend(l, top_children, 2, ax.aux);
        ax.record(ax.ev_xb, ax.aux, 6);
        pre = ax.ev_xb;
      } else extend(l, top_children, 0, st);
      const NdLevel& L = nd.lev[l];
      const bool split = kLookahead && l + 1 < l1 && L.n > 0 && nd.lev[l + 1].n > 0 && L.split_ta > 0;
      factor(l, split, pre);
      prev_split = split;
    }
  }
  void top_gh_damp(bool lead) {
    double* gh = P.nd_rhs + nd.gh_off;
    const unsigned nb = (unsigned)((nd.ntop + 255) / 256);
    if (nd.ntop > 0) { form_hit(KF_ND_GH, 2); form_hit(KF_ND_TOP_DAMP); }
    if (nd.ntop > 0) hipLaunchKernelGGL(k_nd_gh, dim3(nb), dim3(256), 0, st, P, (const int*)nd.top_g, nd.ntop, gh, 0);
    if (!nd.dist) reduce_top_replicated();
    else if (nd.ntop > 0 && ax.reduce != nullptr) ax.reduce(ax.reduce_ctx, gh, 2 * (size_t)nd.ntop, 0, st);
    if (nd.ntop > 0) {
      hipLaunchKernelGGL(k_nd_gh, dim3(nb), dim3(256), 0, st, P, (const int*)nd.top_g, nd.ntop, gh, 1);
      hipLaunchKernelGGL(k_nd_top_damp, dim3(nb), dim3(256), 0, st, P, (const int*)nd.top_var, (const int*)nd.top_r, (const int*)nd.top_g, nd.ntop,
                         (const int*)nd.rhs_node, mu, lead ? 1 : 0);
    }
  }
  void reduce_top_replicated() {
    if (ax.reduce == nullptr) return;
    if (nd.n_top_tiles > 0) form_hit(KF_ND_TOP_PACK, 2);
    const size_t ntile = (size_t)nd.n_top_tiles * kTile * kTile, nvec = nd.rhs_top + 2 * (size_t)nd.ntop;
    if (nd.n_top_tiles > 0) hipLaunchKernelGGL(k_nd_top_pack, dim3(nd.n_top_tiles), dim3(256), 0, st, P, (const int*)nd.top_tiles, nd.top_pack, 0);
    if (nvec > 0) (void)hipMemcpyAsync(nd.top_pack + ntile, P.nd_rhs, nvec * sizeof(double), hipMemcpyDeviceToDevice, st);
    ax.reduce(ax.reduce_ctx, nd.top_pack, ntile + nvec, 0, st);
    if (nd.n_top_tiles > 0) hipLaunchKernelGGL(k_nd_top_pack, dim3(nd.n_top_tiles), dim3(256), 0, st, P, (const int*)nd.top_tiles, nd.top_pack, 1);
    if (nvec > 0) (void)hipMemcpyAsync(P.nd_rhs, nd.top_pack + ntile, nvec * sizeof(double), hipMemcpyDeviceToDevice, st);
  }
  struct XCtx { FrontRun* run; const NdLevel* L; };
  static void exchange_panel(void* vc, int Pp) {
    const XCtx& x = *static_cast<XCtx*>(vc);
    const FrontRun& r = *x.run;
    const NdLevel& L = *x.L;
    const int nt = L.dx_nt[Pp], ne = nt + L.dx_nr[Pp];
    if (ne == 0 || r.ax.reduce == nullptr) return;
    const int4* ent = reinterpret_cast<const int4*>(r.nd.dist_ent) + L.dx_first[Pp];
    const size_t n = (size_t)nt * kTile * kTile + (size_t)L.dx_nr[Pp] * 256;
    const int lead = r.nd.dist_lead ? 1 : 0;
    form_hit(KF_ND_PANEL_XFER, 2);
    hipLaunchKernelGGL(k_nd_panel_xfer, dim3(ne), dim3(256), 0, r.st, r.P, ent, nt, r.nd.dist_buf, (const int*)r.nd.rhs_node, (const int*)r.nd.own_dims, 0, lead);
    r.ax.reduce(r.ax.reduce_ctx, r.nd.dist_buf, n, 0, r.st);
    hipLaunchKernelGGL(k_nd_panel_xfer, dim3(ne), dim3(256), 0, r.st, r.P, ent, nt, r.nd.dist_buf, (const int*)r.nd.rhs_node, (const int*)r.nd.own_dims, 1, lead);
  }
  void dist_levels() {
    for (int l = ltop; l < nlev; ++l) {
      extend(l, true, 0, st);
      const NdLevel& L = nd.lev[l];
      ax.mark(st, -3);
      if (L.n > 0) {
        XCtx xc{this, &L};
        DistPanels d;
        d.np = (int)L.dx_nt.size(); d.tri = L.dt_dev.data(); d.tri_cnt = L.dt_cnt.data(); d.lead = nd.dist_lead; d.exchange = exchange_panel; d.ctx = &xc;
        DenseBatch bt = batch(l);
        bt.beta0 = nullptr; bt.beta0_off = nullptr;
        dense_cholesky_dist(P.nd_M, P.nd_rhs + L.rhs_off, P.nd_Linv + L.linv_off, P.flag, L.ntot, st, ax, L.nI / kTile, bt, d);
      }
      ax.mark(st, -4);
    }
  }
  void tree_launch(int l_hi, int l_lo, bool form64) {
    BwdTreeLevel tl[kBwdTreeMax];
    int nq = 0;
    for (int l = l_hi; l >= l_lo; --l) {
      const NdLevel& L = nd.lev[l];
      BwdTreeLevel& t = tl[nq++];
      t.nbt = L.n; t.T = L.interior_tiles(); t.nchunk = L.pipe_chunks(); t.tI = L.nI / kTile; t.first = L.first;
      t.y = P.nd_rhs + L.rhs_off + L.ntot; t.bsR = (size_t)2 * L.ntot; t.Dinv = P.nd_Linv + L.linv_off; t.bsL = (size_t)L.nI * kTile;
      t.btab = P.nd_ntab + 2 * (size_t)L.first; t.live = L.live; t.scr_off = t.xpub_off = 0;
    }
    launch_bwd_tree(P.nd_M, tl, nq, xfer(0), ax.bwd_pipe, ax.gate_dead, ax.gate_dead_h, ax.gate_timeout_s, st, form64);
    ax.mark(st, -5);
  }
  void backward() {
    if (tree_top_on) tree_launch(nlev - 1, nd.tree_top0, true);
    for (int l = (tree_top_on ? nd.tree_top0 : nlev) - 1; l >= (tree_on ? nd.tree_levels : 0); --l) {
      const NdLevel& L = nd.lev[l];
      if (L.n == 0) continue;
      DenseBatch bt = batch(l);
      bt.xfer = xfer(L.first);
      bt.bwd_cnt = kFusedBwd ? ax.bwd_cnt : nullptr; bt.bwd_scr = ax.bwd_scr;
      if (kFusedBwd && !ax.pipe_broken && ax.bwd_pipe != nullptr) { bt.bwd_pipe = ax.bwd_pipe; bt.pipe_dead = ax.gate_dead; bt.pipe_dead_h = ax.gate_dead_h; bt.pipe_timeout_s = ax.gate_timeout_s; }
      dense_backward_solve(P.nd_M, P.nd_rhs + L.rhs_off, P.nd_Linv + L.linv_off, L.ntot, st, L.nI / kTile, L.ntot / kTile, bt);
      ax.mark(st, -5);
    }
    if (tree_on) tree_launch(nd.tree_levels - 1, 0, false);
    ax.mark(st, -6);
  }
};

bool launch_nd_solve(const DevProblem& P, NdDev& nd, double* dst, double mu, hipStream_t st, CholAux& ax) {
  FrontRun r(P, nd, dst, mu, st, ax);
  ax.init();
  if (!r.ensure_scratch()) return false;
  r.assemble();
  r.run_levels(0, r.ltop, false);
  if (r.ltop < r.nlev) {
    for (int l = r.ltop; l < r.nlev; ++l) r.extend(l, false, 0, st);
    r.top_gh_damp(nd.dist ? nd.dist_lead : true);
    if (nd.dist) r.dist_levels(); else r.run_levels(r.ltop, r.nlev, true);
  }
  r.backward();
  return true;
}

}
```

### covins_amd/csrc/k_panel.hip

```cpp
#include <cstdio>
#include <cstdlib>

#include <algorithm>

#include "common.hpp"
#include "dev_math.hpp"

namespace covgpu {

typedef double v4f64 __attribute__((ext_vector_type(4)));

#ifdef COVGPU_PROBE
__device__ long long g_pprobe[8];
__device__ long long g_pstep[4][16];
#define PSTEP(k, j, t0) do { if ((threadIdx.x & 63) == 0) g_pstep[k][j] = clock64() - (t0); } while (0)
__device__ long long g_parr[16][16];
#define PARR(j, t0) do { if ((threadIdx.x & 63) == 0) g_parr[threadIdx.x >> 6][j] = clock64() - (t0); } while (0)
#ifndef PPROBE_WAVE
#define PPROBE_WAVE 1
#endif
#define PPROBE_DECL() long long pacc[8] = {0, 0, 0, 0, 0, 0, 0, 0}
#define PPROBE_ACC(i, t0) do { pacc[i] += clock64() - (t0); } while (0)
#define PPROBE_T0() clock64()
#define PPROBE_FLUSH() do { if (threadIdx.x == 0) for (int i_ = 1; i_ < 6; ++i_) g_pprobe[i_] = pacc[i_]; if (threadIdx.x == 64 * PPROBE_WAVE) { g_pprobe[6] = pacc[6]; g_pprobe[7] = pacc[7]; } } while (0)
#else
#define PPROBE_DECL() do {} while (0)
#define PPROBE_ACC(i, t0) do {} while (0)
#define PPROBE_T0() 0
#define PPROBE_FLUSH() do {} while (0)
#define PSTEP(k, j, t0) do {} while (0)
#define PARR(j, t0) do {} while (0)
#define PPROBE_WAVE 1
#endif

constexpr int PB = 16;
constexpr int PP = 18;
constexpr int PROWS = 256;
constexpr int NW = 16;
constexpr int NSLOT = 10;
constexpr size_t kPanelLds = (size_t)(2 * PROWS * PP + 256 + 256 + 32 + 16 * PP) * sizeof(double);
constexpr int PROWS4 = 128;
constexpr size_t kPanelLds4 = (size_t)(2 * PROWS4 * PP + 256 + PROWS4 + 32 + 16 * PP) * sizeof(double);

COV_DEV void lds_barrier() { asm volatile("s_waitcnt lgkmcnt(0)\n\ts_barrier" ::: "memory"); }

COV_DEV int hw_lane_id() {
  int l;
  asm volatile("v_mbcnt_lo_u32_b32 %0, -1, 0\n\tv_mbcnt_hi_u32_b32 %0, -1, %0" : "=v"(l));
  return l;
}

template <int C> COV_DEV double dpp_bcast(double v) {
  double d;
  asm volatile("s_nop 1\n\tv_mov_b64_dpp %0, %1 row_newbcast:%2 row_mask:0xf bank_mask:0xf" : "=v"(d) : "v"(v), "n"(C));
  return d;
}
template <int C> COV_DEV void dpp_fmac(double& acc, double m) {
  asm volatile("v_fmac_f64_dpp %0, %0, %1 row_newbcast:%2 row_mask:0xf bank_mask:0xf" : "+v"(acc) : "v"(m), "n"(C));
}
COV_DEV void dpp_fence(double (&a)[16], double (&w)[4]) {
  asm volatile("s_nop 4" : "+v"(a[0]), "+v"(a[1]), "+v"(a[2]), "+v"(a[3]), "+v"(a[4]), "+v"(a[5]), "+v"(a[6]), "+v"(a[7]), "+v"(a[8]), "+v"(a[9]),
               "+v"(a[10]), "+v"(a[11]), "+v"(a[12]), "+v"(a[13]), "+v"(a[14]), "+v"(a[15]), "+v"(w[0]), "+v"(w[1]), "+v"(w[2]), "+v"(w[3]));
}

template <int C> COV_DEV void diag_sweep(double (&a)[16], double (&w)[4], int r, bool& bad, double& rsr) {
  if constexpr (C < 16) {
    int rr = r;
    asm volatile("" : "+v"(rr));
    const double d = dpp_bcast<C>(a[C]);
    bad = bad || !(d > 0.0);
    const double r0 = __builtin_amdgcn_rcp(d);
    const double e0 = fma(-d, r0, 1.0);
    const double r1 = fma(r0, e0, r0), e1 = e0 * e0;
    const double rinv = fma(r1, e1, r1);
    const double nt = -(a[C] * rinv);
#pragma unroll
    for (int cc = C + 1; cc < 16; ++cc) dpp_fmac<C>(a[cc], nt);
    const double ntw = (rr > C) ? nt : 0.0;
#pragma unroll
    for (int e = 0; e < 4; ++e) dpp_fmac<C>(w[e], ntw);
    rsr = (rr == C) ? d : rsr;
    diag_sweep<C + 1>(a, w, r, bad, rsr);
  }
}

COV_DEV v4f64 tile_update(v4f64 acc, const double* pan, int i, int k, int fr, int fk) {
  const double* pa = pan + (PB * i + fr) * PP + 4 * fk;
  const double* pb = pan + (PB * k + fr) * PP + 4 * fk;
  const double2 a01 = *reinterpret_cast<const double2*>(pa), a23 = *reinterpret_cast<const double2*>(pa + 2);
  const double2 b01 = *reinterpret_cast<const double2*>(pb), b23 = *reinterpret_cast<const double2*>(pb + 2);
  acc = __builtin_amdgcn_mfma_f64_16x16x4f64(-a01.x, b01.x, acc, 0, 0, 0);
  acc = __builtin_amdgcn_mfma_f64_16x16x4f64(-a01.y, b01.y, acc, 0, 0, 0);
  acc = __builtin_amdgcn_mfma_f64_16x16x4f64(-a23.x, b23.x, acc, 0, 0, 0);
  acc = __builtin_amdgcn_mfma_f64_16x16x4f64(-a23.y, b23.y, acc, 0, 0, 0);
  return acc;
}

struct PanelTileTab { int v[119]; };
constexpr PanelTileTab make_panel_tiles() {
  PanelTileTab t{};
  int u = 0;
  for (int k = 1; k < 16; ++k)
    for (int i = k; i < 16; ++i) { if (i == 1 && k == 1) continue; t.v[u++] = i | (k << 8); }
  return t;
}
__constant__ PanelTileTab kPanelTile = make_panel_tiles();
struct PanelTileTab8 { int v[27]; };
constexpr PanelTileTab8 make_panel_tiles8() {
  PanelTileTab8 t{};
  int u = 0;
  for (int k = 1; k < 8; ++k)
    for (int i = k; i < 8; ++i) { if (i == 1 && k == 1) continue; t.v[u++] = i | (k << 8); }
  return t;
}
__constant__ PanelTileTab8 kPanelTile8 = make_panel_tiles8();

template <int NT>
COV_DEV void panel_out(const double* pan, double* sRhs, const double* rs, double* Mg, size_t ld, int o, int n, int u, double* yo) {
  for (int row = o + PB + (u >> 1); row < n; row += NT / 2) {
    const double2* src = reinterpret_cast<const double2*>(pan + row * PP + 8 * (u & 1));
    double2* dst = reinterpret_cast<double2*>(Mg + (size_t)row * ld + o + 8 * (u & 1));
    const double2 v0 = src[0], v1 = src[1], v2 = src[2], v3 = src[3];
    dst[0] = v0; dst[1] = v1; dst[2] = v2; dst[3] = v3;
  }
  for (int e = NT - 1 - u; e < 256; e += NT) {
    const int rr = e >> 4, cc = e & 15;
    if (cc <= rr) Mg[(size_t)(o + rr) * ld + o + cc] = pan[(o + rr) * PP + cc] * rs[cc];
  }
  for (int row = o + PB + (NT - 1 - u); row < n; row += NT) {
    double t0 = 0.0, t1 = 0.0, t2 = 0.0, t3 = 0.0;
#pragma unroll
    for (int c = 0; c < PB; c += 4) {
      t0 += sRhs[o + c] * pan[row * PP + c]; t1 += sRhs[o + c + 1] * pan[row * PP + c + 1];
      t2 += sRhs[o + c + 2] * pan[row * PP + c + 2]; t3 += sRhs[o + c + 3] * pan[row * PP + c + 3];
    }
    sRhs[row] -= (t0 + t1) + (t2 + t3);
  }
  if (yo != nullptr && u < PB) yo[o + u] = sRhs[o + u];
}

template <int NWV>
COV_DEV void potrf_panel_body(double* __restrict__ M, size_t ld, int k0, int nb, double* __restrict__ Dinv_out, int* flag,
                              const double* __restrict__ rhs, double* __restrict__ yout, size_t bsM, size_t bsL, size_t bsR,
                              const long long* __restrict__ btab, const int* __restrict__ own, const int* __restrict__ list) {
  constexpr int PROWS = (NWV == 16) ? 256 : PROWS4;
  constexpr int NTW = (NWV == 16) ? 12 : 3;
  const int front = list != nullptr ? list[blockIdx.x] : (int)blockIdx.x;
  if (own != nullptr) {
    const int real = __builtin_amdgcn_readfirstlane(own[front]) - k0;
    nb = min(nb, (real + PB - 1) / PB);
    if (nb <= 0) return;
  }
  if (btab != nullptr) { M += (size_t)btab[2 * front]; ld = (size_t)btab[2 * front + 1]; }
  else M += (size_t)front * bsM;
  Dinv_out += (size_t)front * bsL;
  if (rhs != nullptr) { rhs += (size_t)front * bsR; yout += (size_t)front * bsR; }
  extern __shared__ __attribute__((aligned(16))) double sP[];
  double* sDv = sP + 2 * PROWS * PP;
  double* sRhs = sDv + 256;
  double* sdd = sRhs + PROWS;
  double* sDg = sdd + 32;
  const int tid0 = threadIdx.x, wave = __builtin_amdgcn_readfirstlane(tid0 >> 6);
  const int n = PB * nb;
  double* Mg = M + (size_t)k0 * ld + k0;
  const long long tp0 = PPROBE_T0();

  auto fill_lds = [&]() {
    const int fid = (NWV == 16) ? 64 * (wave >> 2) + (tid0 & 63) : tid0;
    double fv[PB], frhs = 0.0, fdg = 0.0;
#pragma unroll
    for (int c = 0; c < PB; ++c) fv[c] = 0.0;
    if (fid < n) {
      if (fid >= PB) {
#pragma unroll
        for (int c = 0; c < PB; c += 2) { const double2 v = *reinterpret_cast<const double2*>(Mg + (size_t)fid * ld + c); fv[c] = v.x; fv[c + 1] = v.y; }
      } else {
#pragma unroll
        for (int c = 0; c < PB; ++c) fv[c] = Mg[(size_t)(c > fid ? c : fid) * ld + (c > fid ? fid : c)];
      }
      if (rhs != nullptr) frhs = rhs[k0 + fid];
    }
    if (nb > 1) {
      const int rr = fid >> 4, cc = fid & 15;
      fdg = Mg[(size_t)(PB + (cc <= rr ? rr : cc)) * ld + PB + (cc <= rr ? cc : rr)];
    }
    if (fid < n) {
#pragma unroll
      for (int c = 0; c < PB; c += 2) *reinterpret_cast<double2*>(sP + fid * PP + c) = double2{fv[c], fv[c + 1]};
    }
    if (fid < PROWS) sRhs[fid] = frhs;
    if (nb > 1) sDg[(fid >> 4) * PP + (fid & 15)] = fdg;
  };

  if (wave == 0) {
    PPROBE_DECL();
    fill_lds();
    PPROBE_ACC(4, tp0);
    __builtin_amdgcn_s_setprio(3);
    for (int j = 0; j < nb; ++j) {
      double* cur = sP + (j & 1) * PROWS * PP;
      double* oth = sP + ((j + 1) & 1) * PROWS * PP;
      double* dv = sDv;
      const int o = PB * j;
      const long long tq0 = PPROBE_T0();
      const int ln = hw_lane_id();
      const int r = ln & 15, g = ln >> 4;
      double a[PB], w[4];
#pragma unroll
      for (int e = 0; e < PB; e += 2) { const double2 v = *reinterpret_cast<const double2*>(cur + (o + r) * PP + e); a[e] = v.x; a[e + 1] = v.y; }
#pragma unroll
      for (int e = 0; e < 4; ++e) w[e] = (4 * g + e == r) ? 1.0 : 0.0;
      bool bad = false;
      double rsr = 1.0;
      dpp_fence(a, w);
      diag_sweep<0>(a, w, r, bad, rsr);
      if (bad && ln == 0) atomicOr(flag, 1);
      {
        const double dvv = (rsr > 0.0) ? rsr : 1.0;
        double rs = __builtin_amdgcn_rsq(dvv);
        rs = rs * (1.5 - 0.5 * dvv * rs * rs);
        rs = rs * (1.5 - 0.5 * dvv * rs * rs);
        rsr = rs;
      }
      if (ln < PB) {
        sdd[PB * (j & 1) + r] = rsr;
#pragma unroll
        for (int e = 0; e < PB; e += 2) *reinterpret_cast<double2*>(cur + (o + r) * PP + e) = double2{a[e], a[e + 1]};
      }
      double* dst = Dinv_out + (size_t)(j >> 3) * kTile * kTile + (size_t)(j & 7) * 256 + r * PB + 4 * g;
      double xv[4];
#pragma unroll
      for (int e = 0; e < 4; ++e) {
        xv[e] = (4 * g + e <= r) ? w[e] * rsr : 0.0;
        asm volatile("" : "+v"(xv[e]));
        dv[r * PB + 4 * g + e] = xv[e];
        dst[e] = xv[e];
      }
      PPROBE_ACC(5, tq0);
      PSTEP(0, j, tp0);
      lds_barrier();
      PPROBE_ACC(1, tq0);
      PSTEP(1, j, tp0);
      const long long tq1 = PPROBE_T0();
      if (j + 1 < nb) {
        double* tp = cur + (o + PB + r) * PP + 4 * g;
        const double2 ta = *reinterpret_cast<const double2*>(tp), tc = *reinterpret_cast<const double2*>(tp + 2);
        v4f64 dg;
#pragma unroll
        for (int rg = 0; rg < 4; ++rg) dg[rg] = sDg[(g + 4 * rg) * PP + r];
        v4f64 xt = v4f64{0.0, 0.0, 0.0, 0.0};
        xt = __builtin_amdgcn_mfma_f64_16x16x4f64(xv[0], ta.x, xt, 0, 0, 0);
        xt = __builtin_amdgcn_mfma_f64_16x16x4f64(xv[1], ta.y, xt, 0, 0, 0);
        xt = __builtin_amdgcn_mfma_f64_16x16x4f64(xv[2], tc.x, xt, 0, 0, 0);
        xt = __builtin_amdgcn_mfma_f64_16x16x4f64(xv[3], tc.y, xt, 0, 0, 0);
#pragma unroll
        for (int s2 = 0; s2 < 4; ++s2) dg = __builtin_amdgcn_mfma_f64_16x16x4f64(-xt[s2], xt[s2], dg, 0, 0, 0);
#pragma unroll
        for (int s2 = 0; s2 < 4; ++s2) cur[(o + PB + r) * PP + g + 4 * s2] = xt[s2];
#pragma unroll
        for (int rg = 0; rg < 4; ++rg) oth[(o + PB + g + 4 * rg) * PP + r] = dg[rg];
      }
      lds_barrier();
      PPROBE_ACC(2, tq1);
      PSTEP(2, j, tp0);
    }
    __builtin_amdgcn_s_setprio(0);
    PPROBE_FLUSH();
    return;
  }

  const int jsplit = (NWV == 16 && nb > 8) ? nb - 8 : 0;
  if (NWV == 16 && (wave & 3) == 0) {
    fill_lds();
    const int lq = tid0 & 63;
    for (int j = 0; j < nb; ++j) {
      const double* cur = sP + (j & 1) * PROWS * PP;
      const int o = PB * j;
      PARR(j, tp0);
      lds_barrier();
      if (wave == 4 && lq < PB) {
        double y0 = 0.0, y1 = 0.0, y2 = 0.0, y3 = 0.0;
#pragma unroll
        for (int k = 0; k < PB; k += 4) {
          y0 += sDv[lq * PB + k] * sRhs[o + k]; y1 += sDv[lq * PB + k + 1] * sRhs[o + k + 1];
          y2 += sDv[lq * PB + k + 2] * sRhs[o + k + 2]; y3 += sDv[lq * PB + k + 3] * sRhs[o + k + 3];
        }
        sRhs[o + lq] = (y0 + y1) + (y2 + y3);
      }
      lds_barrier();
      if (j < jsplit) panel_out<192>(cur, sRhs, sdd + PB * (j & 1), Mg, ld, o, n, 64 * ((wave >> 2) - 1) + lq, yout != nullptr ? yout + k0 : nullptr);
      if (wave == PPROBE_WAVE) PSTEP(3, j, tp0);
    }
    return;
  }


  PPROBE_DECL();
  const int lane0 = tid0 & 63, fr0 = lane0 & 15, fk0 = lane0 >> 4;
  const int tw = (NWV == 16) ? 3 * (wave >> 2) + (wave & 3) - 1 : wave - 1;
  if (NWV != 16) fill_lds();
  int tik[NSLOT];
#pragma unroll
  for (int s = 0; s < NSLOT; ++s) {
    const int u = NTW * s + tw;
    constexpr int NTILE = (NWV == 16) ? 119 : 27;
    const int pk = (NWV == 16) ? kPanelTile.v[u < NTILE ? u : 0] : kPanelTile8.v[u < NTILE ? u : 0];
    tik[s] = (u < NTILE && (pk & 255) < nb) ? pk : (99 << 8);
  }
  unsigned offn[4], offm[4];
#pragma unroll
  for (int rg = 0; rg < 4; ++rg) {
    const int rw = fk0 + 4 * rg;
    offn[rg] = (unsigned)rw * (unsigned)ld + (unsigned)fr0;
    offm[rg] = fr0 > rw ? (unsigned)fr0 * (unsigned)ld + (unsigned)rw : offn[rg];
  }
  v4f64 acc[NSLOT];
#pragma unroll
  for (int s = 0; s < NSLOT; ++s) {
    const bool on = (tik[s] >> 8) != 99;
    const int ii = on ? (tik[s] & 255) : 1, kk = on ? (tik[s] >> 8) : 1;
    const double* base = Mg + (size_t)(PB * ii) * ld + PB * kk;
#pragma unroll
    for (int rg = 0; rg < 4; ++rg) acc[s][rg] = base[ii == kk ? offm[rg] : offn[rg]];
  }
  for (int j = 0; j < nb; ++j) {
    double* cur = sP + (j & 1) * PROWS * PP;
    double* oth = sP + ((j + 1) & 1) * PROWS * PP;
    const double* dv = sDv;
    const int lq = hw_lane_id();
    const int fr = lq & 15, fk = lq >> 4;
    PARR(j, tp0);
    lds_barrier();
    if (NWV != 16 && tw == 0 && lq < PB) {
      const int o = PB * j;
      double y0 = 0.0, y1 = 0.0, y2 = 0.0, y3 = 0.0;
#pragma unroll
      for (int k = 0; k < PB; k += 4) {
        y0 += sDv[lq * PB + k] * sRhs[o + k]; y1 += sDv[lq * PB + k + 1] * sRhs[o + k + 1];
        y2 += sDv[lq * PB + k + 2] * sRhs[o + k + 2]; y3 += sDv[lq * PB + k + 3] * sRhs[o + k + 3];
      }
      sRhs[o + lq] = (y0 + y1) + (y2 + y3);
    }
    for (int i = j + 2 + tw; i < nb; i += NTW) {
      double* tp = cur + (PB * i + fr) * PP + 4 * fk;
      const double* dp = dv + fr * PB + 4 * fk;
      const double2 ta = *reinterpret_cast<const double2*>(tp), tc = *reinterpret_cast<const double2*>(tp + 2);
      const double2 tb = *reinterpret_cast<const double2*>(dp), td = *reinterpret_cast<const double2*>(dp + 2);
      v4f64 x = v4f64{0.0, 0.0, 0.0, 0.0};
      x = __builtin_amdgcn_mfma_f64_16x16x4f64(ta.x, tb.x, x, 0, 0, 0);
      x = __builtin_amdgcn_mfma_f64_16x16x4f64(ta.y, tb.y, x, 0, 0, 0);
      x = __builtin_amdgcn_mfma_f64_16x16x4f64(tc.x, td.x, x, 0, 0, 0);
      x = __builtin_amdgcn_mfma_f64_16x16x4f64(tc.y, td.y, x, 0, 0, 0);
#pragma unroll
      for (int rg = 0; rg < 4; ++rg) cur[(PB * i + fk + 4 * rg) * PP + fr] = x[rg];
    }
    lds_barrier();
    const long long tq2 = PPROBE_T0();
#pragma unroll
    for (int s = 0; s < NSLOT; ++s) {
      int pk = tik[s];
      asm volatile("" : "+s"(pk));
      const int i = pk & 255, k = pk >> 8;
      if (k >= j + 1 && k != 99 && !(k == j + 1 && i == k)) {
        acc[s] = tile_update(acc[s], cur, i, k, fr, fk);
        if (k == j + 1 || (k == j + 2 && i == k)) {
          double* dstp = (i == k) ? sDg + fk * PP + fr : oth + (PB * i + fk) * PP + fr;
#pragma unroll
          for (int rg = 0; rg < 4; ++rg) dstp[4 * rg * PP] = acc[s][rg];
        }
      }
    }
    PPROBE_ACC(6, tq2);
    if (wave == PPROBE_WAVE) PSTEP(3, j, tp0);
    const long long tq3 = PPROBE_T0();
    if (j >= jsplit) panel_out<64 * NTW>(cur, sRhs, sdd + PB * (j & 1), Mg, ld, PB * j, n, 64 * tw + lq, yout != nullptr ? yout + k0 : nullptr);
    PPROBE_ACC(7, tq3);
  }
  PPROBE_FLUSH();
}

__global__ __launch_bounds__(64 * NW) void k_potrf_panel(double* __restrict__ M, size_t ld, int k0, int nb, double* __restrict__ Dinv_out, int* flag,
                                                         const double* __restrict__ rhs, double* __restrict__ yout, size_t bsM, size_t bsL, size_t bsR,
                                                         const long long* __restrict__ btab, const int* __restrict__ own, const int* __restrict__ list) {
  potrf_panel_body<16>(M, ld, k0, nb, Dinv_out, flag, rhs, yout, bsM, bsL, bsR, btab, own, list);
}
__global__ __launch_bounds__(256) __attribute__((amdgpu_waves_per_eu(3, 3))) void k_potrf_panel4(double* __restrict__ M, size_t ld, int k0, int nb, double* __restrict__ Dinv_out, int* flag,
                                                         const double* __restrict__ rhs, double* __restrict__ yout, size_t bsM, size_t bsL, size_t bsR,
                                                         const long long* __restrict__ btab, const int* __restrict__ own, const int* __restrict__ list) {
  potrf_panel_body<4>(M, ld, k0, nb, Dinv_out, flag, rhs, yout, bsM, bsL, bsR, btab, own, list);
}

struct TrsmSubArgs {
  double* M; size_t ld;
  int k0;
  int r0;
  const double* Dinv;
  double* rhs; const double* yvec;
  size_t bsM, bsL, bsR;
  const int* live; int tI;
  int chain;
  const long long* btab;
  const int* own;
};

#ifdef COVGPU_PROBE
__device__ long long g_tprobe[4][24];
#define TPROBE(k) do { if (lane == 0 && blockIdx.x == 0 && blockIdx.y == 0) g_tprobe[wave][k] = clock64() - tstart; } while (0)
#else
#define TPROBE(k) do {} while (0)
#endif
template <int NB>
COV_DEV void trsm_sub4_body(const TrsmSubArgs& g, v4f64 (*zall)[64], int* zcount, double (*spart)[16]) {
  constexpr int MB = NB / 4;
  const int batch = blockIdx.y, lane = threadIdx.x & 63, n = lane & 15, fk = lane >> 4;
  const int wave = __builtin_amdgcn_readfirstlane(threadIdx.x >> 6);
  const int row0 = g.r0 + PB * (int)blockIdx.x;
#ifdef COVGPU_PROBE
  const long long tstart = clock64();
#endif
  if (g.chain) __builtin_amdgcn_s_setprio(3);
  double* Mb = g.M + (g.btab != nullptr ? (size_t)g.btab[2 * batch] : (size_t)batch * g.bsM);
  const size_t ld = g.btab != nullptr ? (size_t)g.btab[2 * batch + 1] : g.ld;
  const double* Db = g.Dinv + (size_t)batch * g.bsL;
  const int pr = 4 * (n & 3) + (n >> 2);
  double* Arow = Mb + (size_t)(row0 + n) * ld + g.k0 + 4 * fk;
  const double* Lrow = Mb + (size_t)(g.k0 + pr) * ld + g.k0 + 4 * fk;
  const double* Drow = Db + pr * PB + 4 * fk;
  auto Ltile = [&](int i, int j) { return *reinterpret_cast<const v4f64*>(Lrow + (size_t)(PB * i) * ld + PB * j); };
  auto Dblk = [&](int j) { return *reinterpret_cast<const v4f64*>(Drow + (size_t)(j >> 3) * kTile * kTile + (j & 7) * 256); };
  v4f64 acc[MB];
#pragma unroll
  for (int m = 0; m < MB; ++m) acc[m] = *reinterpret_cast<const v4f64*>(Arow + PB * (4 * m + wave));
  v4f64 dmine[MB];
#pragma unroll
  for (int m = 0; m < MB; ++m) dmine[m] = Dblk(4 * m + wave);
  constexpr int RING = 8;
  v4f64 ring[RING];
  int pj = 0, pm = 0, pt = 0;
  auto fetch = [&]() {
    if (pj < NB - 1) {
      ring[pt % RING] = Ltile(4 * pm + wave, pj); ++pt;
      if (++pm >= MB) { ++pj; pm = (pj + 1) >> 2; }
    }
  };
#pragma unroll
  for (int k = 0; k < RING - 1; ++k) fetch();
  auto publish = [&](int j, int m) {
    v4f64 Z = v4f64{0.0, 0.0, 0.0, 0.0};
#pragma unroll
    for (int s = 0; s < 4; ++s) Z = __builtin_amdgcn_mfma_f64_16x16x4f64(dmine[m][s], acc[m][s], Z, 0, 0, 0);
    acc[m] = Z;
    zall[j][lane] = -Z;
    if (lane == 0) __hip_atomic_store(zcount, j + 1, __ATOMIC_RELAXED, __HIP_MEMORY_SCOPE_WORKGROUP);
  };
  if (wave == 0) publish(0, 0);
  int t = 0;
#pragma unroll
  for (int j = 0; j + 1 < NB; ++j) {
    const int o1 = (j + 1) & 3, m1 = (j + 1) >> 2;
    if (wave != (j & 3)) {
      int spins = 0;
      while (__hip_atomic_load(zcount, __ATOMIC_RELAXED, __HIP_MEMORY_SCOPE_WORKGROUP) < j + 1 && ++spins < (1 << 22)) __builtin_amdgcn_s_sleep(1);
    }
    const v4f64 Zn = zall[j][lane];
    if (NB == 16) TPROBE(j);
#pragma unroll
    for (int m = m1; m < MB; ++m) {
      fetch();
      if (m > m1 || wave >= o1) {
#pragma unroll
        for (int s = 0; s < 4; ++s) acc[m] = __builtin_amdgcn_mfma_f64_16x16x4f64(ring[t % RING][s], Zn[s], acc[m], 0, 0, 0);
      }
      ++t;
      if (m == m1 && wave == o1) publish(j + 1, m1);
    }
  }
  if (NB == 16) TPROBE(16);
#pragma unroll
  for (int m = 0; m < MB; ++m) *reinterpret_cast<v4f64*>(Arow + PB * (4 * m + wave)) = acc[m];
  if (g.rhs != nullptr) {
    const double* yv = g.yvec + (size_t)batch * g.bsR + g.k0 + 4 * fk;
    double part = 0.0;
#pragma unroll
    for (int m = 0; m < MB; ++m) {
      const v4f64 y4 = *reinterpret_cast<const v4f64*>(yv + PB * (4 * m + wave));
#pragma unroll
      for (int s = 0; s < 4; ++s) part += acc[m][s] * y4[s];
    }
    part += __shfl_xor(part, 16, 64);
    part += __shfl_xor(part, 32, 64);
    if (fk == 0) spart[wave][n] = part;
    lds_barrier();
    if (wave == 0 && fk == 0) g.rhs[(size_t)batch * g.bsR + row0 + n] -= ((spart[0][n] + spart[1][n]) + spart[2][n]) + spart[3][n];
  }
}

template <int NB>
__global__ __launch_bounds__(256) void k_trsm_sub4(TrsmSubArgs g) {
  __shared__ v4f64 zall[16][64];
  __shared__ double spart[4][16];
  __shared__ int zcount;
  if (g.live != nullptr) {
    const int batch = blockIdx.y, row0 = g.r0 + PB * (int)blockIdx.x;
    const int nI = g.live[2 * batch], nO = g.live[2 * batch + 1];
    const int tp = g.k0 / kTile, tr = row0 / kTile;
    if (!(tp < nI || (tp >= g.tI && tp - g.tI < nO))) return;
    if (!(tr < nI || (tr >= g.tI && tr - g.tI < nO))) return;
  }
  int nbf = NB;
  if (g.own != nullptr) {
    const int real = g.own[blockIdx.y] - g.k0;
    if (real <= 0) return;
    nbf = (real + PB - 1) / PB;
  }
  if (threadIdx.x == 0) zcount = 0;
  __syncthreads();
  if (NB > 4 && nbf <= 4) { trsm_sub4_body<4>(g, zall, &zcount, spart); return; }
  if (NB > 8 && nbf <= 8) { trsm_sub4_body<8>(g, zall, &zcount, spart); return; }
  if (NB > 12 && nbf <= 12) { trsm_sub4_body<12>(g, zall, &zcount, spart); return; }
  trsm_sub4_body<NB>(g, zall, &zcount, spart);
}


__global__ __launch_bounds__(256) void k_bwd_step_sub(const double* __restrict__ M, size_t ld, int p, const double* __restrict__ Dinv,
                                                       double* __restrict__ y, double* __restrict__ x, int ncol, size_t bsM, size_t bsL, size_t bsR,
                                                       const long long* __restrict__ btab, const int* __restrict__ live, int tI, BwdXfer xf) {
  if (live != nullptr) {
    const int nI = live[2 * blockIdx.y], nO = live[2 * blockIdx.y + 1];
    if (!(p < nI || (p >= tI && p - tI < nO))) return;
  }
  if (btab != nullptr) { M += (size_t)btab[2 * blockIdx.y]; ld = (size_t)btab[2 * blockIdx.y + 1]; }
  else M += (size_t)blockIdx.y * bsM;
  y += (size_t)blockIdx.y * bsR; x += (size_t)blockIdx.y * bsR;
  if (Dinv != nullptr) Dinv += (size_t)blockIdx.y * bsL;
  __shared__ double sx[kTile];
  __shared__ double sv[kTile];
  __shared__ double part[8][33];
  const int tid = threadIdx.x, k0 = p * kTile;
  if (Dinv == nullptr) {
    if (tid < kTile) sx[tid] = x[k0 + tid];
    __syncthreads();
  } else {
// ... 544 lines not shown
      a0 += Lq[2 * r] * x0.x; a1 += Lq[2 * r + 1] * x0.y; a2 += Lq[2 * r + 2] * x1.x; a3 += Lq[2 * r + 3] * x1.y;
    }
  }
  {
    double acc = (a0 + a1) + (a2 + a3);
    acc += __shfl_xor(acc, 32, 64);
    if (vh) { v -= acc; sv[c] = v; }
  }
  lds_barrier();
#ifdef COVGPU_PIPE_PROBE
  tp2 = wall_clock64();
#endif
  {
    double s0 = 0.0, s1 = 0.0;
#pragma unroll
    for (int i = 0; i < 16; i += 2) { s0 += w1[i] * sv[64 + 16 * gq + i]; s1 += w1[i + 1] * sv[64 + 16 * gq + i + 1]; }
    double sum = s0 + s1;
    sum += __shfl_xor(sum, 16, 64); sum += __shfl_xor(sum, 32, 64);
    if (gq == 0) {
      sx[64 + cc] = sum;
      if (p > 0 && !(g.fault && p == nIt - 1)) __hip_atomic_store(xpub_f + (size_t)p * kTile + 64 + cc, sum, __ATOMIC_RELAXED, __HIP_MEMORY_SCOPE_AGENT);
      if (gi_hi >= 0) { if (g.tree) __hip_atomic_store(g.xf.x + gi_hi, sum, __ATOMIC_RELAXED, __HIP_MEMORY_SCOPE_AGENT); else g.xf.x[gi_hi] = sum; }
    }
  }
  lds_barrier();
  {
    double s0 = 0.0, s1 = 0.0;
#pragma unroll
    for (int i = 0; i < 16; i += 2) { s0 += bb[i] * sx[64 + 16 * gq + i]; s1 += bb[i + 1] * sx[64 + 16 * gq + i + 1]; }
    double sum = s0 + s1;
    sum += __shfl_xor(sum, 16, 64); sum += __shfl_xor(sum, 32, 64);
    if (gq == 0) svlo[cc] = sv[cc] - sum;
  }
  lds_barrier();
  {
    double s0 = 0.0, s1 = 0.0;
#pragma unroll
    for (int i = 0; i < 16; i += 2) { s0 += w0[i] * svlo[16 * gq + i]; s1 += w0[i + 1] * svlo[16 * gq + i + 1]; }
    double sum = s0 + s1;
    sum += __shfl_xor(sum, 16, 64); sum += __shfl_xor(sum, 32, 64);
    if (gq == 0) {
      if (p > 0 && !(g.fault && p == nIt - 1)) __hip_atomic_store(xpub_f + (size_t)p * kTile + cc, sum, __ATOMIC_RELAXED, __HIP_MEMORY_SCOPE_AGENT);
      if (gi_lo >= 0) { if (g.tree) __hip_atomic_store(g.xf.x + gi_lo, sum, __ATOMIC_RELAXED, __HIP_MEMORY_SCOPE_AGENT); else g.xf.x[gi_lo] = sum; }
    }
  }
#ifdef COVGPU_PIPE_PROBE
  tp3 = wall_clock64();
  asm volatile("s_waitcnt vmcnt(0)" ::: "memory");
  tp4 = wall_clock64();
  if (tid == 0 && nch == 0) printf("pipe64 tile %2d: start %lld  last x in +%lld  product +%lld  solve +%lld  stores done +%lld (10 ns ticks)\n", p, tp0 % 100000000ll, tp1 - tp0, tp2 - tp1, tp3 - tp2, tp4 - tp3);
#endif
  if (p == 0)
    for (int i = kTile + tid; i < nIt * kTile; i += 256)
      __hip_atomic_store(reinterpret_cast<unsigned long long*>(xpub_f + i), kPipeEmpty, __ATOMIC_RELAXED, __HIP_MEMORY_SCOPE_AGENT);
}
__global__ __launch_bounds__(256) void k_bwd_pipe64(BwdPipeArgs g) { bwd_pipe64_body(g, (int)blockIdx.x, (int)blockIdx.y); }
__global__ __launch_bounds__(256) void k_bwd_tree64(BwdTreeArgs a) {
  int l = 0;
  while (l + 1 < a.nlev && (int)blockIdx.x >= a.wg0[l + 1]) ++l;
  const BwdTreeLevel& L = a.lev[l];
  BwdPipeArgs g = a.base;
  g.tI = L.tI; g.T = L.T; g.nchunk = L.nchunk; g.y = L.y; g.Dinv_all = L.Dinv; g.bsL = L.bsL; g.bsR = L.bsR; g.btab = L.btab; g.live = L.live; g.xf.first = L.first;
  g.scr = a.base.scr + L.scr_off; g.xpub = a.base.scr + L.xpub_off; g.tree = 1;
  const int per = L.T * L.nchunk + L.T, local = (int)blockIdx.x - a.wg0[l];
  bwd_pipe64_body(g, local % per, local / per);
}
__global__ void k_pipe_fill(unsigned long long* p, size_t n) {
  for (size_t i = (size_t)blockIdx.x * 256 + threadIdx.x; i < n; i += (size_t)gridDim.x * 256) p[i] = kPipeEmpty;
}
unsigned long long pipe_empty_word() { return kPipeEmpty; }
void launch_pipe_fill(double* buf, size_t n, hipStream_t st) {
  if (n > 0) hipLaunchKernelGGL(k_pipe_fill, dim3((unsigned)std::min<size_t>((n + 255) / 256, 4096)), dim3(256), 0, st, reinterpret_cast<unsigned long long*>(buf), n);
}
void launch_bwd_tree(const double* M, const BwdTreeLevel* lev, int nlev, BwdXfer xf, double* pipe, int* dead, int* dead_h, double timeout_s, hipStream_t st, bool form64) {
  BwdTreeArgs a;
  a.base = BwdPipeArgs{M, 0, 0, 0, nullptr, nullptr, 0, 0, nullptr, nullptr, xf, pipe, pipe, dead, dead_h, (long long)(timeout_s * 1e8), 2047, 0, 1};
  static const int check = std::max(1, env_int("COVGPU_PIPE_SPIN_CHECK", 2048));
  static const int fault = env_int("COVGPU_PIPE_FAULT", 0);
  a.base.check = check - 1; a.base.fault = fault;
  a.nlev = nlev; a.wg0[0] = 0;
  size_t off = 0;
  for (int l = 0; l < nlev; ++l) {
    a.lev[l] = lev[l];
    a.lev[l].scr_off = off; off += (size_t)lev[l].nbt * lev[l].T * lev[l].nchunk * kTile;
    a.lev[l].xpub_off = off; off += (size_t)lev[l].nbt * lev[l].T * kTile;
    a.wg0[l + 1] = a.wg0[l] + lev[l].nbt * (lev[l].T * lev[l].nchunk + lev[l].T);
  }
  constexpr size_t lds = (size_t)128 * 7 * 8 * sizeof(double), lds64 = (size_t)kP64Doubles * sizeof(double);
  static std::atomic<unsigned long long> seen{0};
  if (first_use_on_device(seen)) {
    (void)hipFuncSetAttribute(reinterpret_cast<const void*>(k_bwd_tree), hipFuncAttributeMaxDynamicSharedMemorySize, (int)lds);
    (void)hipFuncSetAttribute(reinterpret_cast<const void*>(k_bwd_tree64), hipFuncAttributeMaxDynamicSharedMemorySize, (int)lds64);
  }
  form_hit(form64 ? KF_BWD_TREE64 : KF_BWD_TREE);
  if (form64) hipLaunchKernelGGL(k_bwd_tree64, dim3(a.wg0[nlev]), dim3(256), lds64, st, a);
  else hipLaunchKernelGGL(k_bwd_tree, dim3(a.wg0[nlev]), dim3(256), lds, st, a);
}
void launch_bwd_pipe(const double* S, int tI, int ntiles, int nchunk, double* y, const double* Linv, int nbt, size_t sL, size_t sR, hipStream_t st,
                     const long long* btab, const int* live, BwdXfer xf, double* pipe, int* dead, int* dead_h, double timeout_s) {
  BwdPipeArgs g{S, tI, ntiles, nchunk, y, Linv, sL, sR, btab, live, xf, pipe, pipe + (size_t)nbt * ntiles * nchunk * kTile, dead, dead_h, (long long)(timeout_s * 1e8), 2047, 0, 0};
  static const int fault = env_int("COVGPU_PIPE_FAULT", 0);
  g.fault = fault;
  static const int check = std::max(1, env_int("COVGPU_PIPE_SPIN_CHECK", 2048));
  g.check = check - 1;
  constexpr size_t lds = (size_t)128 * 7 * 8 * sizeof(double);
  static std::atomic<unsigned long long> seen{0}, seen64{0};
  if (first_use_on_device(seen)) (void)hipFuncSetAttribute(reinterpret_cast<const void*>(k_bwd_pipe), hipFuncAttributeMaxDynamicSharedMemorySize, (int)lds);
  constexpr int kPipe64Max = 128;
  if (nbt * ntiles <= kPipe64Max) {
    constexpr size_t lds64 = (size_t)kP64Doubles * sizeof(double);
    if (first_use_on_device(seen64)) (void)hipFuncSetAttribute(reinterpret_cast<const void*>(k_bwd_pipe64), hipFuncAttributeMaxDynamicSharedMemorySize, (int)lds64);
    form_hit(KF_BWD_PIPE64);
    hipLaunchKernelGGL(k_bwd_pipe64, dim3(ntiles * nchunk + ntiles, nbt), dim3(256), lds64, st, g);
    return;
  }
  form_hit(KF_BWD_PIPE);
  hipLaunchKernelGGL(k_bwd_pipe, dim3(ntiles * nchunk + ntiles, nbt), dim3(256), lds, st, g);
}

void launch_bwd_given(const double* S, size_t ld, int r0, int r1, double* y, double* x, int ncol, int nbt, size_t sM, size_t sR, hipStream_t st,
                      const long long* btab, const int* live, int tI, BwdXfer xf) {
  if (r1 <= r0 || ncol <= 0) return;
  form_hit(KF_BWD_GIVEN);
  hipLaunchKernelGGL(k_bwd_given, dim3((ncol + 127) / 128, nbt), dim3(256), (size_t)(r1 - r0) * sizeof(double), st, S, ld, r0, r1, y, (const double*)x, ncol, sM,
                     sR, btab, live, tI, xf);
}

void launch_potrf_panel(double* S, size_t ld, int t0, int w, double* Linv, int* flag, double* b, int npad, int nbt, size_t sM, size_t sL, size_t sR,
                        hipStream_t st, const long long* btab, int nb, const int* own, const int* list, int n_big, int n_small) {
  if (nb < 0) nb = 8 * w;
  if (nb == 0) { form_hit(KF_POTRF_SKIPPED); return; }
  static std::atomic<unsigned long long> seen{0};
  if (first_use_on_device(seen)) {
    (void)hipFuncSetAttribute(reinterpret_cast<const void*>(k_potrf_panel), hipFuncAttributeMaxDynamicSharedMemorySize, (int)kPanelLds);
    (void)hipFuncSetAttribute(reinterpret_cast<const void*>(k_potrf_panel4), hipFuncAttributeMaxDynamicSharedMemorySize, (int)kPanelLds4);
  }
  double* Lp = Linv + (size_t)t0 * kTile * kTile;
  const double* yb = b ? b + npad : nullptr;
  if (list == nullptr) {
    form_hit(KF_POTRF_PANEL); form_hit(KF_POTRF_PANEL_FRONTS, nbt);
    hipLaunchKernelGGL(k_potrf_panel, dim3(nbt), dim3(64 * NW), kPanelLds, st, S, ld, t0 * kTile, nb, Lp, flag, (const double*)b, (double*)yb, sM, sL, sR, btab, own, list);
    return;
  }
  constexpr int kSmallMin = 384;
  if (n_small <= kSmallMin) { n_big += n_small; n_small = 0; }
  if (n_big > 0) { form_hit(KF_POTRF_PANEL); form_hit(KF_POTRF_PANEL_FRONTS, n_big); }
  if (n_small > 0) { form_hit(KF_POTRF_PANEL4); form_hit(KF_POTRF_PANEL4_FRONTS, n_small); }
  if (n_big > 0) hipLaunchKernelGGL(k_potrf_panel, dim3(n_big), dim3(64 * NW), kPanelLds, st, S, ld, t0 * kTile, nb, Lp, flag, (const double*)b, (double*)yb, sM, sL, sR, btab, own, list);
  if (n_small > 0)
    hipLaunchKernelGGL(k_potrf_panel4, dim3(n_small), dim3(256), kPanelLds4, st, S, ld, t0 * kTile, std::min(nb, 8), Lp, flag, (const double*)b, (double*)yb, sM, sL, sR, btab, own,
                       list + n_big);
}

void launch_trsm_sub(double* S, size_t ld, int t0, int w, int r0, int r1, const double* Linv, double* b, int npad, int nbt, size_t sM, size_t sL,
                     size_t sR, const int* live, int tI, hipStream_t st, bool chain, const long long* btab, int nb, const int* own) {
  if (r1 <= r0 || nb == 0) return;
  TrsmSubArgs g{S, ld, t0 * kTile, r0 * kTile, Linv + (size_t)t0 * kTile * kTile, b, b ? b + npad : nullptr, sM, sL, sR, live, tI, chain ? 1 : 0, btab, own};
  const dim3 grid((r1 - r0) * (kTile / PB), nbt);
  const int need = nb > 0 ? std::min(nb, 8 * w) : 8 * w;
  form_hit(need <= 4 ? KF_TRSM_SUB4_4 : need <= 8 ? KF_TRSM_SUB4_8 : need <= 12 ? KF_TRSM_SUB4_12 : KF_TRSM_SUB4_16);
  if (need <= 4) hipLaunchKernelGGL(k_trsm_sub4<4>, grid, dim3(256), 0, st, g);
  else if (need <= 8) hipLaunchKernelGGL(k_trsm_sub4<8>, grid, dim3(256), 0, st, g);
  else if (need <= 12) hipLaunchKernelGGL(k_trsm_sub4<12>, grid, dim3(256), 0, st, g);
  else hipLaunchKernelGGL(k_trsm_sub4<16>, grid, dim3(256), 0, st, g);
}

void launch_bwd_front(const double* S, int tI, int ntiles, int nchunk, double* y, const double* Linv, int nbt, size_t sL, size_t sR, hipStream_t st,
                      const long long* btab, const int* live, BwdXfer xf, int* cnt, double* scr) {
  form_hit(KF_BWD_FRONT);
  hipLaunchKernelGGL(k_bwd_front, dim3(ntiles * nchunk, nbt), dim3(256), 0, st, S, tI, nchunk, y, Linv, sL, sR, btab, live, xf, cnt, scr);
}

void launch_bwd_step_sub(const double* S, size_t ld, int p, const double* Linv_p, double* y, double* x, int ncol, int nblocks, int nbt, size_t sM,
                         size_t sL, size_t sR, hipStream_t st, const long long* btab, const int* live, int tI, BwdXfer xf) {
  form_hit(KF_BWD_STEP_SUB);
  hipLaunchKernelGGL(k_bwd_step_sub, dim3(nblocks, nbt), dim3(256), 0, st, S, ld, p, Linv_p, y, x, ncol, sM, sL, sR, btab, live, tI, xf);
}

}
```

### covins_amd/csrc/nd_tables.hip

```cpp
#include <algorithm>

#include "common.hpp"
#include "nd_plan.hpp"

namespace covgpu {
namespace {

enum ChildKind { kSubtreeChild = 0, kTopChild = 1 };

bool live(int t, int n_int, int tI, int n_border) { return t < n_int || (t >= tI && t - tI < n_border); }

struct FrontTables {
  const NdHostPlan& hp; const int* pos_kf; const int D, rank; NdDev& dev;
  const bool sh;
  int Hs = 0, nlev = 0, nl = 0;
  std::vector<std::vector<int>> lnodes;
  std::vector<int> order, newid, ld;
  std::vector<int> cptr[2], cidx[2], ext, ext_kind;
  FrontTables(const NdHostPlan& hp_, const int* pos_kf_, int D_, int rank_, NdDev& dev_)
      : hp(hp_), pos_kf(pos_kf_), D(D_), rank(rank_), dev(dev_), sh(!hp_.node_rank.empty()) {}
  bool is_top(int n) const { return sh && hp.node_rank[n] < 0; }
  bool is_local(int n) const { return !sh || hp.node_rank[n] < 0 || hp.node_rank[n] == rank; }
  int gidx_of(int v, int r) const { return D * pos_kf[v >> 1] + ((v & 1) ? 6 + r : r); }
  template <class F> void reached_tiles(int i, int ch, int row0, int tile, int count, F&& hit) const {
    const int* inv = dev.h_inv.data() + dev.h_inv_off[ch];
    for (int t = 0; t < count; ++t) {
      bool any = false;
      for (int r = row0 + tile * t; r < std::min(ld[i], row0 + tile * t + tile) && !any; ++r) any = inv[r] >= 0;
      if (any) hit(t);
    }
  }
  void level_order() {
    const int nn = hp.nnodes;
    for (int n = 0; n < nn; ++n) if (!is_top(n)) Hs = std::max(Hs, hp.level[n] + 1);
    std::vector<int> lev(nn), toph(nn, 0);
    for (int n = nn - 1; n >= 0; --n) if (is_top(n)) for (int c : hp.child[n]) if (is_top(c)) toph[n] = std::max(toph[n], toph[c] + 1);
    nlev = Hs;
    for (int n = 0; n < nn; ++n) { lev[n] = is_top(n) ? Hs + toph[n] : hp.level[n]; nlev = std::max(nlev, lev[n] + 1); }
    lnodes.assign(nlev, {});
    for (int n = 0; n < nn; ++n) if (is_local(n)) lnodes[lev[n]].push_back(n);
    newid.assign(nn, -1);
    for (int l = 0; l < nlev; ++l) for (int n : lnodes[l]) { newid[n] = (int)order.size(); order.push_back(n); }
    nl = (int)order.size();
    dev.nnodes = nl; dev.top_lev0 = Hs; dev.plan_flops = hp.flops;
  }
  void variable_maps() {
    const int K = hp.K;
    dev.h_vnode.assign(2 * (size_t)K, -1); dev.h_voff.assign(2 * (size_t)K, 0); dev.h_vord.assign(2 * (size_t)K, 0); dev.h_vown.assign(2 * (size_t)K, 0);
    for (int v = 0; v < 2 * K; ++v)
      if (hp.vnode[v] >= 0) {
        const int n = hp.vnode[v];
        dev.h_vnode[v] = newid[n]; dev.h_voff[v] = hp.voff[v]; dev.h_vord[v] = hp.vord[v];
        dev.h_vown[v] = !is_local(n) ? 0 : (is_top(n) ? 2 : 1);
      }
  }
  void lay_front(NdLevel& L, int n, int i, size_t& moff) {
    const int nO = ((hp.st_dims[n] + kTile - 1) / kTile) * kTile;
    ld[i] = L.nI + nO;
    L.ntot = std::max(L.ntot, ld[i]);
    dev.h_ndepth[i] = hp.depth[n]; dev.h_nI[i] = L.nI;
    dev.h_ntab[2 * (size_t)i] = (long long)moff; dev.h_ntab[2 * (size_t)i + 1] = ld[i];
    moff += (size_t)ld[i] * ld[i];
    dev.h_own_dims[i] = hp.own_dims[n]; dev.h_st_dims[i] = hp.st_dims[n];
    dev.h_own_g[i] = (int)dev.h_gidx.size();
    for (int v : hp.own[n]) for (int r = 0; r < NdHostPlan::vdim(v); ++r) dev.h_gidx.push_back(gidx_of(v, r));
    dev.h_st_g[i] = (int)dev.h_gidx.size();
    for (int v : hp.strct[n]) for (int r = 0; r < NdHostPlan::vdim(v); ++r) dev.h_gidx.push_back(gidx_of(v, r));
    L.live_h.push_back((hp.own_dims[n] + kTile - 1) / kTile); L.live_h.push_back(nO / kTile);
    if (!is_top(n)) return;
    const int nIt = L.nI / kTile, lo2 = 2 * ((hp.own_dims[n] + 2 * kTile - 1) / (2 * kTile)), lb = (hp.st_dims[n] + kTile - 1) / kTile;
    const int Tn = ld[i] / kTile;
    for (int tr = 0; tr < Tn; ++tr)
      for (int tc = 0; tc <= tr; ++tc)
        if (live(tr, lo2, nIt, lb) && live(tc, lo2, nIt, lb)) { dev.h_top_tiles.push_back(i); dev.h_top_tiles.push_back(tr); dev.h_top_tiles.push_back(tc); }
    for (int v : hp.own[n]) for (int r = 0; r < NdHostPlan::vdim(v); ++r) { dev.h_top_var.push_back(v); dev.h_top_r.push_back(r); dev.h_top_g.push_back(gidx_of(v, r)); }
  }
  void panel_lists(NdLevel& L) {
    L.plist_h.resize(L.n);
    for (int k = 0; k < L.n; ++k) L.plist_h[k] = k;
    std::stable_sort(L.plist_h.begin(), L.plist_h.end(), [&](int a, int b) { return dev.h_own_dims[L.first + a] > dev.h_own_dims[L.first + b]; });
    const int np = L.nI / 256;
    L.pbig.assign(np, 0); L.psmall.assign(np, 0);
    for (int k = 0; k < L.n; ++k)
      for (int P = 0; P < np; ++P) {
        const int real = dev.h_own_dims[L.first + k] - 256 * P;
        if (real > 128) ++L.pbig[P]; else if (real > 0) ++L.psmall[P];
      }
  }
  void front_layout() {
    dev.h_ndepth.resize(nl); dev.h_nI.resize(nl); dev.h_ntab.resize(2 * (size_t)nl);
    dev.h_own_dims.resize(nl); dev.h_st_dims.resize(nl); dev.h_own_g.resize(nl); dev.h_st_g.resize(nl);
    dev.lev.resize(nlev);
    ld.resize(nl);
    size_t moff = 0, loff = 0;
    for (int l = 0, i = 0; l < nlev; ++l) {
      NdLevel& L = dev.lev[l];
      L.n = (int)lnodes[l].size(); L.first = i; L.own_max = 0;
      for (int n : lnodes[l]) L.own_max = std::max(L.own_max, hp.own_dims[n]);
      L.nI = std::max(256, ((L.own_max + 255) / 256) * 256);
      L.ntot = L.nI;
      if (l == Hs) dev.M_sub = moff;
      for (int n : lnodes[l]) lay_front(L, n, i++, moff);
      L.linv_off = loff; loff += (size_t)L.n * L.nI * kTile;
      panel_lists(L);
    }
    if (Hs >= nlev) dev.M_sub = moff;
    dev.M_elems = moff; dev.linv_elems = loff;
    dev.ntop = (int)dev.h_top_g.size(); dev.n_top_tiles = (int)(dev.h_top_tiles.size() / 3);
  }
  void rhs_layout() {
    dev.h_rhs_node.assign(nl, 0);
    size_t roff = 0;
    auto place = [&](int l) {
      NdLevel& L = dev.lev[l];
      L.rhs_off = roff;
      for (int k = 0; k < L.n; ++k) dev.h_rhs_node[L.first + k] = (int)(roff + (size_t)k * 2 * L.ntot);
      roff += (size_t)L.n * 2 * L.ntot;
    };
    for (int l = Hs; l < nlev; ++l) place(l);
    dev.rhs_top = roff; dev.gh_off = roff; roff += 2 * dev.h_top_g.size();
    for (int l = 0; l < Hs; ++l) place(l);
    dev.rhs_elems = roff;
  }
  void ancestor_rows() {
    dev.h_abase.assign((size_t)nl * hp.maxdepth, -1);
    for (int i = 0; i < nl; ++i) {
      const int n = order[i];
      for (int a = hp.parent[n]; a >= 0; a = hp.parent[a]) {
        dev.h_abase[(size_t)i * hp.maxdepth + hp.depth[a]] = (int)dev.h_fidx.size();
        dev.h_fidx.resize(dev.h_fidx.size() + hp.own[a].size(), -1);
      }
      int row = dev.h_nI[i];
      for (int v : hp.strct[n]) {
        const int a = hp.vnode[v];
        dev.h_fidx[dev.h_abase[(size_t)i * hp.maxdepth + hp.depth[a]] + hp.vord[v]] = row;
        row += NdHostPlan::vdim(v);
      }
    }
  }
  void children_and_row_maps() {
    for (int kind = 0; kind < 2; ++kind) cptr[kind].assign(nl + 1, 0);
    dev.h_inv_off.assign(nl, -1);
    for (int i = 0; i < nl; ++i) {
      const int n = order[i];
      for (int kind = 0; kind < 2; ++kind) cptr[kind][i + 1] = cptr[kind][i];
      for (int c : hp.child[n]) {
        if (!is_local(c)) continue;
        const int kind = is_top(c) ? kTopChild : kSubtreeChild;
        cidx[kind].push_back(newid[c]); ++cptr[kind][i + 1];
      }
      const int p = hp.parent[n];
      if (p < 0) continue;
      const int ip = newid[p];
      dev.h_inv_off[i] = (int)dev.h_inv.size();
      dev.h_inv.resize(dev.h_inv.size() + ld[ip], -1);
      int* inv = dev.h_inv.data() + dev.h_inv_off[i];
      int row = dev.h_nI[i];
      for (int v : hp.strct[n]) {
        const int prow = hp.vnode[v] == p ? hp.voff[v] : dev.h_fidx[dev.h_abase[(size_t)ip * hp.maxdepth + hp.depth[hp.vnode[v]]] + hp.vord[v]];
        for (int r = 0; r < NdHostPlan::vdim(v); ++r) inv[prow + r] = row + r;
        row += NdHostPlan::vdim(v);
      }
    }
  }
  static void whole_border_tiles(std::vector<char>& mark, int T, int t0) {
    for (int A = t0; A < T; A += 2)
      for (int B = t0; B <= A; B += 2) {
        bool any = false;
        for (int a = A; a < std::min(T, A + 2); ++a) for (int b = B; b < std::min(T, B + 2); ++b) if (b <= a && mark[(size_t)a * T + b]) any = true;
        if (any) for (int a = A; a < std::min(T, A + 2); ++a) for (int b = B; b < std::min(T, B + 2); ++b) if (b <= a) mark[(size_t)a * T + b] = 1;
      }
  }
  void extend_tiles(int l, ChildKind kind, int& first, int& count, int& countA) {
    const NdLevel& L = dev.lev[l];
    first = (int)ext.size() / 3;
    std::vector<int> tiles;
    for (int k = 0; k < L.n; ++k) {
      const int i = L.first + k;
      const int T = (ld[i] + 63) / 64;
      std::vector<char> mark((size_t)T * T, 0);
      for (int q = cptr[kind][i]; q < cptr[kind][i + 1]; ++q) {
        std::vector<int> rows;
        reached_tiles(i, cidx[kind][q], 0, 64, T, [&](int t) { rows.push_back(t); });
        for (int a : rows) for (int b : rows) if (b <= a) mark[(size_t)a * T + b] = 1;
      }
      if (kind == kSubtreeChild && !is_top(order[i])) whole_border_tiles(mark, T, dev.h_nI[i] / 64);
      for (int a = 0; a < T; ++a) for (int b = 0; b <= a; ++b) if (mark[(size_t)a * T + b]) { tiles.push_back(i); tiles.push_back(a); tiles.push_back(b); }
    }
    countA = 0;
    for (int pass = 0; pass < 2; ++pass)
      for (size_t q = 0; q < tiles.size(); q += 3)
        if ((tiles[q + 1] < 4) == (pass == 0)) {
          ext.insert(ext.end(), tiles.begin() + q, tiles.begin() + q + 3); countA += pass == 0 ? 1 : 0;
          ext_kind.push_back(kind);
        }
    count = (int)ext.size() / 3 - first;
  }
  void split_ta(int l) {
    NdLevel& L = dev.lev[l];
    L.split_ta = 0;
    for (int k = 0; k < L.n; ++k) {
      const int n = order[L.first + k], p = hp.parent[n];
      if (p < 0) continue;
      int d = 0;
      for (int v : hp.strct[n]) if (hp.vnode[v] == p && hp.voff[v] < 256) d += NdHostPlan::vdim(v);
      L.split_ta = std::max(L.split_ta, (d + kTile - 1) / kTile);
    }
  }
  void put_front(int* w, int node) const {
    const unsigned long long mo = (unsigned long long)dev.h_ntab[2 * (size_t)node];
    w[0] = (int)(unsigned)(mo & 0xffffffffull); w[1] = (int)(unsigned)(mo >> 32); w[2] = (int)dev.h_ntab[2 * (size_t)node + 1]; w[3] = dev.h_rhs_node[node];
  }
  void flat_lists() {
    for (int kind = 0; kind < 2; ++kind) {
      std::vector<int>& out = kind == kTopChild ? dev.h_extc2 : dev.h_extc;
      out.resize(6 * cidx[kind].size());
      for (size_t k = 0; k < cidx[kind].size(); ++k) {
        int* c = out.data() + 6 * k;
        put_front(c, cidx[kind][k]); c[4] = dev.h_inv_off[cidx[kind][k]]; c[5] = 0;
      }
    }
    const size_t nt = ext.size() / 3;
    dev.h_extw.resize(8 * nt);
    for (size_t q = 0; q < nt; ++q) {
      const int node = ext[3 * q];
      const std::vector<int>& cp = cptr[ext_kind[q]];
      int* w = dev.h_extw.data() + 8 * q;
      put_front(w, node);
      w[4] = ext[3 * q + 1]; w[5] = ext[3 * q + 2]; w[6] = cp[node]; w[7] = cp[node + 1];
    }
  }
  void records() {
    const size_t nt = ext.size() / 3;
    dev.h_extr.assign((size_t)kExtRec * nt, -1);
    dev.ext_over = nt;
    for (size_t q = 0; q < nt; ++q) {
      const int node = ext[3 * q], a = ext[3 * q + 1], b = ext[3 * q + 2], kind = ext_kind[q];
      int nrec = 0;
      const size_t next = dev.h_extr.size() / kExtRec - nt;
      for (int k = cptr[kind][node]; k < cptr[kind][node + 1]; ++k) {
        const int ch = cidx[kind][k];
        bool anyr = false, anyc = false;
        reached_tiles(node, ch, 64 * a, 64, 1, [&](int) { anyr = true; });
        reached_tiles(node, ch, 64 * b, 64, 1, [&](int) { anyc = true; });
        if (!anyr || !anyc) continue;
        if (nrec > 0) dev.h_extr.resize(dev.h_extr.size() + kExtRec, -1);
        int* r = nrec == 0 ? dev.h_extr.data() + (size_t)kExtRec * q : dev.h_extr.data() + dev.h_extr.size() - kExtRec;
        put_front(r + 8, ch);
        const int* inv = dev.h_inv.data() + dev.h_inv_off[ch];
        for (int e = 0; e < 64; ++e) {
          const int rr = 64 * a + e, cc = 64 * b + e;
          r[16 + e] = rr < ld[node] ? inv[rr] : -1; r[80 + e] = cc < ld[node] ? inv[cc] : -1;
        }
        ++nrec;
      }
      int* w = dev.h_extr.data() + (size_t)kExtRec * q;
      for (int e = 0; e < 6; ++e) w[e] = dev.h_extw[8 * q + e];
// ... 128 lines not shown
```

### covins_amd/csrc/solver.hip

```cpp
#include <algorithm>
#include <atomic>
#include <chrono>
#include <cmath>
#include <cstdio>
#include <cstdlib>
#include <cstring>
#include <string>
#include <thread>
#include <vector>

#include "host.hpp"

using namespace covgpu;

thread_local std::string g_err;
extern "C" const char* covgpu_last_error(void) { return g_err.c_str(); }

extern "C" void covgpu_default_options(covgpu_options* o) {
  std::memset(o, 0, sizeof(*o));
  o->strategy = COVGPU_DOGLEG;
  o->max_iterations = 10;
  o->reproj_loss_a = 1.0;
  o->initial_radius = 1e4; o->max_radius = 1e16; o->min_relative_decrease = 1e-3;
  o->function_tolerance = 1e-6; o->parameter_tolerance = 1e-8; o->gradient_tolerance = 1e-10;
  const double sf = std::sqrt(200.0);
  o->sigma_g = 1.7e-4 * sf; o->sigma_a = 2.0e-3 * sf; o->sigma_gw = 1.9393e-5 / sf; o->sigma_aw = 3.0e-3 / sf;
  o->gravity = 9.81;
}

extern "C" int32_t covgpu_reduced_dim(const covgpu_options* opt, const covgpu_problem* p) {
  return (opt->visual_only ? 6 : 15) * p->num_kf;
}

extern "C" int32_t covgpu_lm_group(int64_t num_obs, int32_t num_lm) {
  const double mean_track = num_lm > 0 ? (double)num_obs / num_lm : 0.0;
  return mean_track <= 5.0 ? 4 : (mean_track <= 8.0 ? 8 : 16);
}

extern "C" int covgpu_create(const covgpu_options* opt, covgpu_context** out) {
  int ndev = 0;
  if (hipGetDeviceCount(&ndev) != hipSuccess || ndev == 0) {
    g_err = "no HIP device visible: libcovgpu has no CPU fallback";
    return COVGPU_ERR_NO_DEVICE;
  }
  covgpu_context* c = new covgpu_context();
  c->device = opt ? opt->device : 0;
  if (c->device < 0 || c->device >= ndev) { g_err = "device ordinal out of range"; delete c; return COVGPU_ERR_INVALID_ARG; }
  HIPCHK(hipSetDevice(c->device));
  {
    int lo = 0, hi = 0;
    (void)hipDeviceGetStreamPriorityRange(&lo, &hi);
    HIPCHK(hipStreamCreateWithPriority(&c->st, hipStreamDefault, hi));
  }
  HIPCHK(hipHostMalloc((void**)&c->h_scal, (SC_COUNT + 4) * sizeof(double), hipHostMallocDefault));
  HIPCHK(hipHostMalloc((void**)&c->h_tr, TR_COUNT * sizeof(double), hipHostMallocDefault));
  {
    if (hipHostMalloc((void**)&c->h_box, (TR_COUNT + 1) * sizeof(double), hipHostMallocMapped | hipHostMallocCoherent) == hipSuccess) {
      std::memset(c->h_box, 0, (TR_COUNT + 1) * sizeof(double));
      if (hipHostGetDevicePointer((void**)&c->d_box, c->h_box, 0) != hipSuccess) c->d_box = nullptr;
    } else { (void)hipGetLastError(); c->h_box = nullptr; }
  }
  for (auto& e : c->ev) HIPCHK(hipEventCreate(&e));
  std::memset(&c->P, 0, sizeof(c->P));
  *out = c;
  return COVGPU_OK;
}

extern "C" void covgpu_destroy(covgpu_context* c) {
  if (!c) return;
  (void)hipSetDevice(c->device);
  while (!c->bowdbs.empty()) covgpu_bowdb_destroy(c->bowdbs.back());
  free_problem(c);
  for (auto& e : c->ev) if (e) (void)hipEventDestroy(e);
  c->chol.destroy();
  if (c->h_scal) (void)hipHostFree(c->h_scal);
  if (c->h_tr) (void)hipHostFree(c->h_tr);
  if (c->h_box) (void)hipHostFree(c->h_box);
  clear_shard(c);
  if (c->st) (void)hipStreamDestroy(c->st);
  delete c;
}

extern "C" void covgpu_set_profiling(covgpu_context* c, int on) {
  c->profiling = on; c->prof = covgpu_profile_t();
  c->chol.profile = on != 0; c->chol.syrk_ms = 0; c->chol.syrk_flops = 0; c->chol.n_syrk = 0;
  c->chol.potrf_ms = 0; c->chol.potrf_flops = 0; c->chol.n_potrf = 0;
}
extern "C" void covgpu_get_profile(covgpu_context* c, double* out) {
  out[0] = c->prof.t_build_ms; out[1] = (double)c->prof.n_build; out[2] = c->prof.t_factor_ms; out[3] = (double)c->prof.n_factor;
  out[4] = c->chol.syrk_ms; out[5] = (double)c->chol.n_syrk; out[6] = c->chol.syrk_flops;
  out[7] = (double)(c->have ? c->P.npairs + c->P.nepairs : 0);
}
extern "C" void covgpu_get_profile2(covgpu_context* c, double* out) {
  covgpu_get_profile(c, out);
  out[8] = c->chol.potrf_ms; out[9] = (double)c->chol.n_potrf; out[10] = c->chol.potrf_flops; out[11] = c->have ? c->nd.plan_flops : 0.0;
  out[12] = out[13] = out[14] = out[15] = 0.0;
}

extern "C" int covgpu_get_kernel_forms(covgpu_context* c, int64_t* out, int32_t n) {
  for (int i = 0; i < n && i < KF_COUNT; ++i) out[i] = c != nullptr ? (int64_t)c->chol.forms.n[i] : 0;
  return KF_COUNT;
}
extern "C" const char* covgpu_kernel_form_name(int32_t i) { return i >= 0 && i < KF_COUNT ? kFormNames[i] : nullptr; }

extern "C" void covgpu_get_layout(covgpu_context* c, int64_t* out) {
  for (int i = 0; i < 16; ++i) out[i] = 0;
  if (!c->have) return;
  const DevProblem& P = c->P;
  out[0] = c->sharded ? c->world : 0; out[1] = c->sharded ? c->rank : 0; out[2] = c->nd.ntop;
  out[3] = (int64_t)c->nd.lev.size() - c->nd.top_lev0;
  out[4] = c->nd.dist ? (int64_t)((c->nd.dist_solve_elems * sizeof(double)) >> 10)
                      : (int64_t)(((size_t)c->nd.n_top_tiles * kTile * kTile + c->nd.rhs_top + 2 * (size_t)c->nd.ntop) * sizeof(double)) >> 10;
  out[5] = c->chol.pipe_broken ? -1 : c->chol.gates_on ? 1 : 0;
  out[6] = P.npad; out[7] = P.npairs; out[8] = P.nepairs; out[9] = P.nchains; out[10] = (int64_t)(c->alloc_bytes >> 20);
  if (P.nd) {
    out[11] = P.nd_nnodes; out[12] = P.nd_nlev;
    for (const NdLevel& L : c->nd.lev) out[13] += L.nI / 256;
    out[14] = c->nd.lev.empty() ? 0 : c->nd.lev.back().nI; out[15] = (int64_t)((c->nd.M_elems * sizeof(double)) >> 20);
  }
}

int read_scalars(covgpu_context* c) {
  HIPCHK(hipMemcpyAsync(c->h_scal, c->P.scal, SC_COUNT * sizeof(double), hipMemcpyDeviceToHost, c->st));
  HIPCHK(hipMemcpyAsync(c->h_scal + SC_COUNT, c->P.flag, sizeof(int), hipMemcpyDeviceToHost, c->st));
  HIPCHK(hipStreamSynchronize(c->st));
  HIPCHK(hipGetLastError());
  return COVGPU_OK;
}
int chol_failed(covgpu_context* c) { int f; std::memcpy(&f, c->h_scal + SC_COUNT, sizeof(int)); return f; }

void enqueue_build(covgpu_context* c, double mu) {
  const DevProblem& P = c->P;
  c->cur_damp = mu;
  if (c->profiling) (void)hipEventRecord(c->ev[0], c->st);
  c->chol.init();
  hipStream_t side = c->chol.mid;
  {
    DevSignal sig = P.L > 0 ? c->chol.publish_handle(c->chol.ev_zero, c->st, 1) : DevSignal();
    if (sig.flag == nullptr) c->chol.record(c->chol.ev_zero, c->st, 1);
    launch_lm_lin(P, mu, c->st, sig);
  }
  c->chol.wait(side, c->chol.ev_zero);
  launch_zero_system(P, side);
  const bool forked = P.L > 0 && P.npairs > 0;
  if (!forked) { c->chol.record(c->chol.ev_lin, side, 2); c->chol.wait(c->st, c->chol.ev_lin); }
  if (P.nd) { launch_nd_zero(P, c->nd, c->chol.head); (void)hipMemsetAsync(P.nd_rhs, 0, c->nd.rhs_elems * sizeof(double), c->chol.head); }
  else (void)hipMemsetAsync(P.Sred, 0, (size_t)P.npad * P.npad * sizeof(double), c->chol.head);
  c->chol.record(c->chol.ev_fill, c->chol.head, 3);
  launch_imu_build(P, side);
  if (P.vi) {
    launch_imu_gather(P, 1, side);
    launch_finalize_diag(P, mu, 1, side);
  }
  launch_edge_build(P, side);
  launch_lm_build(P, mu, c->st, c->chol.ev_fill, side, c->chol.ev_lin, c->chol.ev_kf, &c->chol);
  if (forked) launch_part_finish(P, SC_COST, 1, side);
  c->chol.record(c->chol.ev_kf, side, 4);
  c->chol.wait(c->st, c->chol.ev_kf);
  if (P.vi && !c->edge_beside_imu) launch_pose_finish(P, mu, c->st);
  else {
    launch_imu_gather(P, 0, c->st);
    launch_edge_gather(P, c->st);
    launch_finalize_diag(P, mu, P.vi ? 0 : 2, c->st);
  }
  if (!forked) launch_part_finish(P, SC_COST, 1, c->st);
  if (c->profiling) (void)hipEventRecord(c->ev[1], c->st);
}

void enqueue_solve(covgpu_context* c, double* dst_all) {
  const DevProblem& P = c->P;
  if (c->profiling) (void)hipEventRecord(c->ev[2], c->st);
  FormScope census(&c->chol.forms);
  if (P.nd) {
    if (!launch_nd_solve(P, c->nd, dst_all, c->cur_damp, c->st, c->chol) && !c->coll_failed) { c->coll_failed = true; c->coll_err = "scratch allocation of the backward substitution failed"; }
  }
  else launch_pose_graph_solve(P, dst_all, c->st, c->chol, c->pgo_plan.active ? &c->pgo_plan : nullptr);
  if (c->profiling) (void)hipEventRecord(c->ev[3], c->st);
  launch_lm_backsub(P, dst_all, dst_all, c->st);
}

static void collect_profile(covgpu_context* c, bool built, bool solved) {
  if (solved && !c->profiling) c->chol.collect();
  if (!c->profiling) return;
  float ms = 0;
  if (built && hipEventElapsedTime(&ms, c->ev[0], c->ev[1]) == hipSuccess) { c->prof.t_build_ms += ms; c->prof.n_build++; }
  if (solved && hipEventElapsedTime(&ms, c->ev[2], c->ev[3]) == hipSuccess) { c->prof.t_factor_ms += ms; c->prof.n_factor++; }
  if (solved) c->chol.collect();
}

static void enqueue_jvp(covgpu_context* c, const double* v_all) {
  const DevProblem& P = c->P;
  launch_obs_jvp(P, v_all, c->st);
  launch_imu_jvp(P, v_all, c->st);
  launch_edge_jvp(P, v_all, c->st);
  launch_part_finish(P, SC_JV2, 1, c->st);
}

static void enqueue_cost_candidate(covgpu_context* c) {
  const DevProblem& P = c->P;
  launch_obs_cost(P, P.pose_c, P.lm_c, c->st);
  launch_imu_cost(P, P.pose_c, P.sb_c, c->st);
  launch_edge_cost(P, P.pose_c, c->st);
  launch_part_finish(P, SC_COST, 1, c->st);
}

static bool dist_sharded(const covgpu_context* c) { return c->sharded && c->shard_plan && c->shard_plan->shard_policy == 1; }
static int dist_fail(covgpu_context* c) {
  if (c->reducer) c->reducer->abort();
  if (c->peer_fail) c->peer_fail->store(1);
  const std::string why = c->coll_failed ? c->coll_err
                                         : std::string("a device-flag gate or a hand-over of the backward substitution timed out (the distributed top does not repeat a solve on one rank)");
  g_err = "sharded solve, rank " + std::to_string(c->rank) + ": " + why;
  return COVGPU_ERR_NO_DEVICE;
}

static int wait_iteration(covgpu_context* c) {
  if (c->sharded && c->reducer) {
    static const double limit = getenv("COVGPU_COLL_TIMEOUT_S") ? std::max(1.0, atof(getenv("COVGPU_COLL_TIMEOUT_S"))) : 300.0;
    const auto t0 = std::chrono::steady_clock::now();
    long spins = 0;
    for (;;) {
      const hipError_t q = hipStreamQuery(c->st);
      if (q == hipSuccess) break;
      if (q != hipErrorNotReady) { g_err = std::string("hipStreamQuery: ") + hipGetErrorString(q); return COVGPU_ERR_NO_DEVICE; }
      ++spins;
      if (spins == 256 || (spins > 256 && (spins & 63) == 0)) {
        const char* why = nullptr;
        if (c->peer_fail && c->peer_fail->load(std::memory_order_relaxed)) why = "another rank of the call gave up";
        else if (c->reducer->async_error() != 0) why = "RCCL reported an asynchronous communicator error";
        else if (std::chrono::duration<double>(std::chrono::steady_clock::now() - t0).count() > limit) why = "collective timed out (COVGPU_COLL_TIMEOUT_S)";
        if (why) { if (!c->coll_failed) { c->coll_failed = true; c->coll_err = why; } c->reducer->abort(); break; }
      } else if (spins > 256) std::this_thread::sleep_for(std::chrono::microseconds(50));
    }
  }
  HIPCHK(hipStreamSynchronize(c->st));
  return COVGPU_OK;
}

static int iteration_status(covgpu_context* c) {
  HIPCHK(hipGetLastError());
  if (dist_sharded(c) && (c->coll_failed || c->chol.gate_failed())) return dist_fail(c);
  if (c->chol.gate_failed()) {
    g_err = "solve: a device-flag gate between the context's streams timed out (COVGPU_GATE_TIMEOUT_S; COVGPU_GATES=0 selects HIP events)";
    return COVGPU_ERR_GATE_TIMEOUT;
  }
  if (c->coll_failed) {
    if (c->reducer) c->reducer->abort();
    if (c->peer_fail) c->peer_fail->store(1);
    g_err = (c->sharded ? "sharded solve, rank " + std::to_string(c->rank) + ": " : std::string("solve: ")) + c->coll_err;
    return COVGPU_ERR_NO_DEVICE;
  }
  return COVGPU_OK;
}

static int end_iteration(covgpu_context* c, bool use_box) {
  double* h = c->h_tr;
  bool got = false;
  if (use_box) {
    volatile double* box = c->h_box;
    for (unsigned spins = 1; !got; ++spins) {
      if (box[TR_COUNT] == c->box_seq) { got = true; break; }
      if ((spins & 4095u) == 0) { const hipError_t q = hipStreamQuery(c->st); if (q != hipErrorNotReady) break; }
    }
    std::atomic_thread_fence(std::memory_order_acquire);
    if (got) for (int i = 0; i < TR_COUNT; ++i) h[i] = box[i];
  }
  if (!got) {
    HIPCHK(hipMemcpyAsync(h, c->P.tr, TR_COUNT * sizeof(double), hipMemcpyDeviceToHost, c->st));
    RC(wait_iteration(c));
  }
  const int rc = iteration_status(c);
  if (rc != COVGPU_OK && got) (void)hipStreamSynchronize(c->st);
  return rc;
}

static bool enqueue_tail_fused(covgpu_context* c, const TrConsts& tc, bool reuse, double damp) {
  const DevProblem& P = c->P;
  const bool two = tc.strategy == COVGPU_DOGLEG;
  const bool coll = c->sharded && c->reducer != nullptr;
  if (!reuse) {
    enqueue_build(c, damp);
    enqueue_solve(c, P.gn);
    launch_tail_stats(P, c->st);
    launch_tail_jvp(P, two, c->st);
    launch_tail_finish(P, tc, 1, two, !coll, 1, c->st);
    if (coll) { reduce_scalars(c); launch_tail_logic(P, tc, 1, 1, c->st); }
  } else launch_tail_logic(P, tc, 1, 0, c->st);
  launch_tail_apply(P, c->st);
  launch_tail_cost(P, c->st);
  launch_tail_finish(P, tc, 2, two, !coll, 0, c->st);
  if (coll) { reduce_scalars(c); launch_tail_logic(P, tc, 2, 0, c->st); }
  static const bool dev_aids = getenv("COVGPU_TRACE_PANELS") != nullptr || getenv("COVGPU_GATE_LOG") != nullptr;
  const bool use_box = c->d_box != nullptr && !coll && !c->profiling && !dev_aids;
  if (use_box) c->box_seq += 1.0;
  launch_tr_accept(P, c->st, use_box ? c->d_box : nullptr, c->box_seq);
  return use_box;
}
static bool enqueue_tail_legacy(covgpu_context* c, const TrConsts& tc, bool reuse, double damp) {
  const DevProblem& P = c->P;
  if (!reuse) {
    enqueue_build(c, damp);
    enqueue_solve(c, P.gn);
    if (tc.strategy == COVGPU_DOGLEG) { launch_cauchy_vec(P, c->st); enqueue_jvp(c, P.vtmp); }
    launch_dogleg_stats(P, c->st);
    reduce_scalars(c);
  }
  launch_tr_after_solve(P, tc, reuse ? 0 : 1, c->st);
  launch_combine_step_dev(P, c->st);
  enqueue_jvp(c, P.step);
  launch_xnorm(P, c->st);
  reduce_scalars(c);
// ... 240 lines not shown
```

Measured before the change: 323.0.

## Factor eligible leaf fronts in one kernel, overlapped with system build

Adds a sixteen-wave leaf-front Cholesky kernel that factors each small leaf front, updates its Schur border and right-hand side in a single launch, replacing the general batched panel/trsm/gemm sequence for the lowest ND level. When the whole tree is local and the problem is visual-inertial, the leaf assembly and factorisation run on the head stream right after the IMU diagonal is finalised. This overlaps them with the edge and landmark build, and the main stream later waits on a leaf event. The cost is extra stream/event coordination, a split assemble kernel, and a remapped row layout that must stay consistent with the downstream levels. It also assumes leaf fronts only hold velocity/bias variables untouched by the later build.

```diff
diff --git a/covins_amd/csrc/common.hpp b/covins_amd/csrc/common.hpp
--- a/covins_amd/csrc/common.hpp
+++ b/covins_amd/csrc/common.hpp
@@ -205,6 +205,7 @@
   KF_ND_EXTEND_REC, KF_ND_EXTEND, KF_ND_EXTEND_SPLIT,
   KF_ND_TOP_PACK, KF_ND_GH, KF_ND_TOP_DAMP, KF_ND_PANEL_XFER, KF_DIST_PANEL,
   KF_PGO_ARROW, KF_PGO_DENSE,
+  KF_POTRF_LEAF,
   KF_COUNT
 };
 extern const char* const kFormNames[KF_COUNT];
@@ -228,6 +229,7 @@
   hipEvent_t ev_xa = nullptr;
   hipEvent_t ev_zero = nullptr;
   hipEvent_t ev_lin = nullptr, ev_kf = nullptr;
+  hipEvent_t ev_sb = nullptr, ev_leaf = nullptr;
   std::vector<hipEvent_t> ev, prof_ev, panel_ev;
   std::vector<double> prof_flops;
   std::vector<hipEvent_t> prof_ev2;
@@ -322,6 +324,8 @@
 void launch_potrf_panel(double* S, size_t ld, int t0, int w, double* Linv, int* flag, double* b, int npad, int nbt, size_t sM, size_t sL, size_t sR,
                         hipStream_t st, const long long* btab = nullptr, int nb = -1, const int* own = nullptr, const int* list = nullptr, int n_big = 0,
                         int n_small = 0);
+void launch_potrf_leaf(double* S, double* Linv, int* flag, double* b, int npad, int nbt, size_t sL, size_t sR, hipStream_t st, const long long* btab,
+                       const int* own, const int* stdim, int nI);
 void launch_bwd_given(const double* S, size_t ld, int r0, int r1, double* y, double* x, int ncol, int nbt, size_t sM, size_t sR, hipStream_t st,
                       const long long* btab, const int* live, int tI, BwdXfer xf = BwdXfer());
 void launch_bwd_front(const double* S, int tI, int ntiles, int nchunk, double* y, const double* Linv, int nbt, size_t sL, size_t sR, hipStream_t st,
@@ -387,6 +391,7 @@
   int* live = nullptr;
   std::vector<int> live_h;
   int own_max = 0;
+  bool leaf_one = false;
   int* plist = nullptr; std::vector<int> plist_h, pbig, psmall;
   int ext_first = 0, ext_count = 0;
   int ext_countA = 0;
@@ -401,6 +406,7 @@
 struct NdDev {
   bool active = false;
   int nnodes = 0;
+  bool leaves_done = false;
   int top_lev0 = 0;
   std::vector<NdLevel> lev;
   int *own_dims = nullptr, *st_dims = nullptr, *own_g = nullptr, *st_g = nullptr;
@@ -431,6 +437,8 @@
 void nd_tables(const NdHostPlan& hp, const int* pos_kf, int D, int rank, NdDev& dev);
 void launch_nd_init(const DevProblem& P, const NdDev& nd, hipStream_t st);
 void launch_nd_zero(const DevProblem& P, const NdDev& nd, hipStream_t st);
+bool nd_leaves_beside_pass(const NdDev& nd);
+bool launch_nd_leaves(const DevProblem& P, NdDev& nd, hipStream_t s, CholAux& ax);
 bool launch_nd_solve(const DevProblem& P, NdDev& nd, double* dst, double mu, hipStream_t st, CholAux& ax);
 
 void launch_tail_stats(const DevProblem& P, hipStream_t st);
diff --git a/covins_amd/csrc/k_chol.hip b/covins_amd/csrc/k_chol.hip
--- a/covins_amd/csrc/k_chol.hip
+++ b/covins_amd/csrc/k_chol.hip
@@ -277,6 +277,8 @@
   if (!ev_fill) (void)hipEventCreateWithFlags(&ev_fill, hipEventDisableTiming);
   if (!ev_xb) (void)hipEventCreateWithFlags(&ev_xb, hipEventDisableTiming);
   if (!ev_xa) (void)hipEventCreateWithFlags(&ev_xa, hipEventDisableTiming);
+  if (!ev_sb) (void)hipEventCreateWithFlags(&ev_sb, hipEventDisableTiming);
+  if (!ev_leaf) (void)hipEventCreateWithFlags(&ev_leaf, hipEventDisableTiming);
   if (!bwd_cnt && hipMalloc((void**)&bwd_cnt, 65536 * sizeof(int)) == hipSuccess) (void)hipMemset(bwd_cnt, 0, 65536 * sizeof(int));
   if (!gate_dead && hipMalloc((void**)&gate_dead, sizeof(int)) == hipSuccess) (void)hipMemset(gate_dead, 0, sizeof(int));
   if (!gate_dead_h && hipHostMalloc((void**)&gate_dead_h, 4 * sizeof(int), hipHostMallocDefault) == hipSuccess) gate_dead_h[0] = gate_dead_h[1] = gate_dead_h[2] = gate_dead_h[3] = 0;
@@ -441,6 +443,8 @@
   if (ev_fill) { (void)hipEventDestroy(ev_fill); ev_fill = nullptr; }
   if (ev_xb) { (void)hipEventDestroy(ev_xb); ev_xb = nullptr; }
   if (ev_xa) { (void)hipEventDestroy(ev_xa); ev_xa = nullptr; }
+  if (ev_sb) { (void)hipEventDestroy(ev_sb); ev_sb = nullptr; }
+  if (ev_leaf) { (void)hipEventDestroy(ev_leaf); ev_leaf = nullptr; }
   if (bwd_cnt) { (void)hipFree(bwd_cnt); bwd_cnt = nullptr; }
   if (gate_flags) { (void)hipFree(gate_flags); gate_flags = nullptr; }
   if (gate_dead) { (void)hipFree(gate_dead); gate_dead = nullptr; }
@@ -506,6 +510,7 @@
   "k_nd_extend_rec", "k_nd_extend", "nd_extend_split",
   "k_nd_top_pack", "k_nd_gh", "k_nd_top_damp", "k_nd_panel_xfer", "dist_panel",
   "pgo_arrow", "pgo_dense",
+  "k_potrf_leaf",
 };
 static_assert(sizeof(kFormNames) / sizeof(kFormNames[0]) == KF_COUNT, "one name per kernel form");
 
diff --git a/covins_amd/csrc/k_front.hip b/covins_amd/csrc/k_front.hip
--- a/covins_amd/csrc/k_front.hip
+++ b/covins_amd/csrc/k_front.hip
@@ -41,10 +41,10 @@
 }
 
 __global__ __launch_bounds__(256) void k_nd_assemble(DevProblem P, const int* __restrict__ rhs_off, double* __restrict__ x, const int* __restrict__ fill, int nfill,
-                                                      unsigned long long empty) {
+                                                      unsigned long long empty, int part, int nleaf) {
   const int t = blockIdx.x * blockDim.x + threadIdx.x;
   if (t < nfill) reinterpret_cast<unsigned long long*>(x)[fill[t]] = empty;
-  if (P.vi) {
+  if (P.vi && part != 2) {
     const int pos = t / 324, e = t - 324 * pos;
     if (pos < P.K) {
       const int vs = 2 * pos + 1;
@@ -67,7 +67,7 @@
     const int kf = t / P.D, r = t - kf * P.D, pos = P.perm[kf];
     const int v = r < 6 ? 2 * pos : 2 * pos + 1, rr = r < 6 ? r : r - 6;
     const int node = P.nd_vnode[v];
-    if (node >= 0) P.nd_rhs[rhs_off[node] + P.nd_voff[v] + rr] = P.bred[t];
+    if (node >= 0 && (part == 0 || (node < nleaf) == (part == 1))) P.nd_rhs[rhs_off[node] + P.nd_voff[v] + rr] = P.bred[t];
   }
 }
 
@@ -264,6 +264,8 @@
 static const bool kBwdTree = env_int("COVGPU_BWD_TREE", 1) != 0;
 static const bool kExtRecords = env_int("COVGPU_EXT_RECORDS", 1) != 0;
 static const bool kBeta0 = env_int("COVGPU_BETA0", 1) != 0;
+static int env_leaf_one() { static const int v = env_int("COVGPU_LEAF_ONE", 1); return v; }
+static const bool kLeafOne = env_leaf_one() != 0;
 
 static NdLevArgs lev_args(const DevProblem& P, const NdDev& nd, int l) {
   const NdLevel& L = nd.lev[l];
@@ -336,12 +338,17 @@
     tree_top_on = tree_ok && nd.tree_top0 < nlev;
     return true;
   }
-  void assemble() {
+  void assemble(bool leaves_early) {
     ax.mark(st, -1);
     const int nfill = (tree_on || tree_top_on) ? (int)nd.h_tree_fill.size() : 0;
-    const int cnt = std::max(std::max(P.vi ? 324 * P.K : 0, P.n), nfill);
-    hipLaunchKernelGGL(k_nd_assemble, dim3((cnt + 255) / 256), dim3(256), 0, st, P, (const int*)nd.rhs_node, dst, (const int*)nd.tree_fill, nfill, pipe_empty_word());
+    const int cnt = std::max(std::max(P.vi && !leaves_early ? 324 * P.K : 0, P.n), nfill);
+    hipLaunchKernelGGL(k_nd_assemble, dim3((cnt + 255) / 256), dim3(256), 0, st, P, (const int*)nd.rhs_node, dst, (const int*)nd.tree_fill, nfill, pipe_empty_word(),
+                       leaves_early ? 2 : 0, leaves_early ? nd.lev[0].n : 0);
     ax.mark(st, -2);
+  }
+  void assemble_leaves(hipStream_t s) {
+    const int cnt = std::max(P.vi ? 324 * P.K : 0, P.n);
+    hipLaunchKernelGGL(k_nd_assemble, dim3((cnt + 255) / 256), dim3(256), 0, s, P, (const int*)nd.rhs_node, (double*)nullptr, (const int*)nullptr, 0, 0ull, 1, nd.lev[0].n);
   }
   DenseBatch batch(int l) const {
     const NdLevel& L = nd.lev[l];
@@ -375,19 +382,27 @@
                          (const int*)(top_children ? nd.extc2 : nd.extc), top_children ? 1 : 0, store_border, sig);
     return count > 0;
   }
+  bool leaf_one(int l) const { return kLeafOne && l == 0 && nd.lev[0].leaf_one && nd.lev[0].n > 0; }
+  void leaf_launch(hipStream_t s) {
+    const NdLevel& L = nd.lev[0];
+    launch_potrf_leaf(P.nd_M, P.nd_Linv + L.linv_off, P.flag, P.nd_rhs + L.rhs_off, L.ntot, L.n, (size_t)L.nI * kTile, (size_t)2 * L.ntot, s,
+                      P.nd_ntab + 2 * (size_t)L.first, nd.own_dims + L.first, nd.st_dims + L.first, L.nI);
+  }
   void factor(int l, bool split, hipEvent_t pre_trsm) {
     const NdLevel& L = nd.lev[l];
     ax.mark(st, -3);
-    if (L.n > 0) {
+    if (leaf_one(l)) leaf_launch(st);
+    else if (L.n > 0) {
       DenseBatch bt = batch(l);
       bt.split_ta = split ? L.split_ta : 0; bt.pre_trsm = pre_trsm;
       dense_cholesky_solve_raw(P.nd_M, P.nd_rhs + L.rhs_off, P.nd_Linv + L.linv_off, P.flag, L.ntot, st, ax, L.nI / kTile, false, bt);
     }
     ax.mark(st, -4);
   }
-  void run_levels(int l0, int l1, bool top_children) {
+  void run_levels(int l0, int l1, bool top_children, bool leaves_early = false) {
     bool prev_split = false;
     for (int l = l0; l < l1; ++l) {
+      if (leaves_early && l == 0) { prev_split = kLookahead && l + 1 < l1 && nd.lev[1].n > 0 && nd.lev[0].split_ta > 0; continue; }
       hipEvent_t pre = nullptr;
       if (prev_split) {
         DevSignal sig = ax.publish_handle(ax.ev_xa, st, 5);
@@ -489,12 +504,24 @@
   }
 };
 
+bool nd_leaves_beside_pass(const NdDev& nd) { return kLeafOne && env_leaf_one() != 2 && !nd.lev.empty() && nd.lev[0].leaf_one && nd.lev[0].n > 0 && nd.top_lev0 == (int)nd.lev.size(); }
+bool launch_nd_leaves(const DevProblem& P, NdDev& nd, hipStream_t s, CholAux& ax) {
+  if (!nd_leaves_beside_pass(nd)) return false;
+  FrontRun r(P, nd, nullptr, 0.0, s, ax);
+  r.assemble_leaves(s);
+  r.leaf_launch(s);
+  nd.leaves_done = true;
+  return true;
+}
+
 bool launch_nd_solve(const DevProblem& P, NdDev& nd, double* dst, double mu, hipStream_t st, CholAux& ax) {
   FrontRun r(P, nd, dst, mu, st, ax);
   ax.init();
   if (!r.ensure_scratch()) return false;
-  r.assemble();
-  r.run_levels(0, r.ltop, false);
+  const bool leaves_early = nd.leaves_done;
+  nd.leaves_done = false;
+  r.assemble(leaves_early);
+  r.run_levels(0, r.ltop, false, leaves_early);
   if (r.ltop < r.nlev) {
     for (int l = r.ltop; l < r.nlev; ++l) r.extend(l, false, 0, st);
     r.top_gh_damp(nd.dist ? nd.dist_lead : true);
diff --git a/covins_amd/csrc/k_panel.hip b/covins_amd/csrc/k_panel.hip
--- a/covins_amd/csrc/k_panel.hip
+++ b/covins_amd/csrc/k_panel.hip
@@ -5,6 +5,7 @@
 
 #include "common.hpp"
 #include "dev_math.hpp"
+#include "leaf_front.hpp"
 
 namespace covgpu {
 
@@ -115,11 +116,12 @@
 }
 __constant__ PanelTileTab8 kPanelTile8 = make_panel_tiles8();
 
-template <int NT>
-COV_DEV void panel_out(const double* pan, double* sRhs, const double* rs, double* Mg, size_t ld, int o, int n, int u, double* yo) {
+template <int NT, bool LEAF = false>
+COV_DEV void panel_out(const double* pan, double* sRhs, const double* rs, double* Mg, size_t ld, int o, int n, int u, double* yo, int nown = 0, int bshift = 0,
+                       double* bo = nullptr) {
   for (int row = o + PB + (u >> 1); row < n; row += NT / 2) {
     const double2* src = reinterpret_cast<const double2*>(pan + row * PP + 8 * (u & 1));
-    double2* dst = reinterpret_cast<double2*>(Mg + (size_t)row * ld + o + 8 * (u & 1));
+    double2* dst = reinterpret_cast<double2*>(Mg + (size_t)(LEAF ? leaf_phys_row(row, nown, bshift) : row) * ld + o + 8 * (u & 1));
     const double2 v0 = src[0], v1 = src[1], v2 = src[2], v3 = src[3];
     dst[0] = v0; dst[1] = v1; dst[2] = v2; dst[3] = v3;
   }
@@ -134,15 +136,19 @@
       t0 += sRhs[o + c] * pan[row * PP + c]; t1 += sRhs[o + c + 1] * pan[row * PP + c + 1];
       t2 += sRhs[o + c + 2] * pan[row * PP + c + 2]; t3 += sRhs[o + c + 3] * pan[row * PP + c + 3];
     }
-    sRhs[row] -= (t0 + t1) + (t2 + t3);
+    const double bv = sRhs[row] - ((t0 + t1) + (t2 + t3));
+    sRhs[row] = bv;
+    if (LEAF && bo != nullptr && row >= nown) bo[row + bshift] = bv;
   }
   if (yo != nullptr && u < PB) yo[o + u] = sRhs[o + u];
 }
 
-template <int NWV>
+template <int NWV, bool LEAF = false>
 COV_DEV void potrf_panel_body(double* __restrict__ M, size_t ld, int k0, int nb, double* __restrict__ Dinv_out, int* flag,
                               const double* __restrict__ rhs, double* __restrict__ yout, size_t bsM, size_t bsL, size_t bsR,
-                              const long long* __restrict__ btab, const int* __restrict__ own, const int* __restrict__ list) {
+                              const long long* __restrict__ btab, const int* __restrict__ own, const int* __restrict__ list,
+                              const int* __restrict__ stdim = nullptr, int nI = 0) {
+  static_assert(!LEAF || NWV == 16, "the leaf form is a sixteen-wave form");
   constexpr int PROWS = (NWV == 16) ? 256 : PROWS4;
   constexpr int NTW = (NWV == 16) ? 12 : 3;
   const int front = list != nullptr ? list[blockIdx.x] : (int)blockIdx.x;
@@ -150,6 +156,12 @@
     const int real = __builtin_amdgcn_readfirstlane(own[front]) - k0;
     nb = min(nb, (real + PB - 1) / PB);
     if (nb <= 0) return;
+  }
+  const int nsteps = nb;
+  int nown = 0, bshift = 0;
+  if constexpr (LEAF) {
+    nown = PB * nsteps; bshift = leaf_border_shift(nsteps, nI);
+    nb = min(nsteps + leaf_blocks(__builtin_amdgcn_readfirstlane(stdim[front])), PROWS / PB);
   }
   if (btab != nullptr) { M += (size_t)btab[2 * front]; ld = (size_t)btab[2 * front + 1]; }
   else M += (size_t)front * bsM;
@@ -171,16 +183,17 @@
 #pragma unroll
     for (int c = 0; c < PB; ++c) fv[c] = 0.0;
     if (fid < n) {
+      const int prow = LEAF ? leaf_phys_row(fid, nown, bshift) : fid;
       if (fid >= PB) {
 #pragma unroll
-        for (int c = 0; c < PB; c += 2) { const double2 v = *reinterpret_cast<const double2*>(Mg + (size_t)fid * ld + c); fv[c] = v.x; fv[c + 1] = v.y; }
+        for (int c = 0; c < PB; c += 2) { const double2 v = *reinterpret_cast<const double2*>(Mg + (size_t)prow * ld + c); fv[c] = v.x; fv[c + 1] = v.y; }
       } else {
 #pragma unroll
         for (int c = 0; c < PB; ++c) fv[c] = Mg[(size_t)(c > fid ? c : fid) * ld + (c > fid ? fid : c)];
       }
-      if (rhs != nullptr) frhs = rhs[k0 + fid];
-    }
-    if (nb > 1) {
+      if (rhs != nullptr) frhs = rhs[k0 + prow];
+    }
+    if (nb > 1 && (!LEAF || nsteps > 1)) {
       const int rr = fid >> 4, cc = fid & 15;
       fdg = Mg[(size_t)(PB + (cc <= rr ? rr : cc)) * ld + PB + (cc <= rr ? cc : rr)];
     }
@@ -197,7 +210,7 @@
     fill_lds();
     PPROBE_ACC(4, tp0);
     __builtin_amdgcn_s_setprio(3);
-    for (int j = 0; j < nb; ++j) {
+    for (int j = 0; j < nsteps; ++j) {
       double* cur = sP + (j & 1) * PROWS * PP;
       double* oth = sP + ((j + 1) & 1) * PROWS * PP;
       double* dv = sDv;
@@ -259,6 +272,11 @@
         for (int s2 = 0; s2 < 4; ++s2) cur[(o + PB + r) * PP + g + 4 * s2] = xt[s2];
 #pragma unroll
         for (int rg = 0; rg < 4; ++rg) oth[(o + PB + g + 4 * rg) * PP + r] = dg[rg];
+        if (LEAF && j + 1 == nsteps) {
+          double* sc = Mg + (size_t)(nI + g) * ld + nI + r;
+#pragma unroll
+          for (int rg = 0; rg < 4; ++rg) sc[(size_t)(4 * rg) * ld] = dg[rg];
+        }
       }
       lds_barrier();
       PPROBE_ACC(2, tq1);
@@ -269,11 +287,12 @@
     return;
   }
 
-  const int jsplit = (NWV == 16 && nb > 8) ? nb - 8 : 0;
+  const int jsplit = LEAF ? nsteps : (NWV == 16 && nb > 8) ? nb - 8 : 0;
+  double* const bout = LEAF ? const_cast<double*>(rhs) : nullptr;
   if (NWV == 16 && (wave & 3) == 0) {
     fill_lds();
     const int lq = tid0 & 63;
-    for (int j = 0; j < nb; ++j) {
+    for (int j = 0; j < nsteps; ++j) {
       const double* cur = sP + (j & 1) * PROWS * PP;
       const int o = PB * j;
       PARR(j, tp0);
@@ -288,7 +307,9 @@
         sRhs[o + lq] = (y0 + y1) + (y2 + y3);
       }
       lds_barrier();
-      if (j < jsplit) panel_out<192>(cur, sRhs, sdd + PB * (j & 1), Mg, ld, o, n, 64 * ((wave >> 2) - 1) + lq, yout != nullptr ? yout + k0 : nullptr);
+      if (j < jsplit)
+        panel_out<192, LEAF>(cur, sRhs, sdd + PB * (j & 1), Mg, ld, o, n, 64 * ((wave >> 2) - 1) + lq, yout != nullptr ? yout + k0 : nullptr, nown, bshift,
+                             j + 1 == nsteps ? bout : nullptr);
       if (wave == PPROBE_WAVE) PSTEP(3, j, tp0);
     }
     return;
@@ -319,11 +340,16 @@
   for (int s = 0; s < NSLOT; ++s) {
     const bool on = (tik[s] >> 8) != 99;
     const int ii = on ? (tik[s] & 255) : 1, kk = on ? (tik[s] >> 8) : 1;
-    const double* base = Mg + (size_t)(PB * ii) * ld + PB * kk;
+    if (LEAF && (!on || kk >= nsteps)) {
+#pragma unroll
+      for (int rg = 0; rg < 4; ++rg) acc[s][rg] = 0.0;
+      continue;
+    }
+    const double* base = Mg + (size_t)(LEAF ? leaf_phys_row(PB * ii, nown, bshift) : PB * ii) * ld + PB * kk;
 #pragma unroll
     for (int rg = 0; rg < 4; ++rg) acc[s][rg] = base[ii == kk ? offm[rg] : offn[rg]];
   }
-  for (int j = 0; j < nb; ++j) {
+  for (int j = 0; j < nsteps; ++j) {
     double* cur = sP + (j & 1) * PROWS * PP;
     double* oth = sP + ((j + 1) & 1) * PROWS * PP;
     const double* dv = sDv;
@@ -376,6 +402,20 @@
     if (j >= jsplit) panel_out<64 * NTW>(cur, sRhs, sdd + PB * (j & 1), Mg, ld, PB * j, n, 64 * tw + lq, yout != nullptr ? yout + k0 : nullptr);
     PPROBE_ACC(7, tq3);
   }
+  if constexpr (LEAF) {
+    const int lq = hw_lane_id();
+    const int fr = lq & 15, fk = lq >> 4;
+    double* const sc = Mg + (size_t)(bshift + fk) * ld + bshift + fr;
+#pragma unroll
+    for (int s = 0; s < NSLOT; ++s) {
+      const int i = tik[s] & 255, k = tik[s] >> 8;
+      if (k != 99 && k >= nsteps && !(i == k && k == nsteps)) {
+        double* dstp = sc + (size_t)(PB * i) * ld + PB * k;
+#pragma unroll
+        for (int rg = 0; rg < 4; ++rg) dstp[(size_t)(4 * rg) * ld] = acc[s][rg];
+      }
+    }
+  }
   PPROBE_FLUSH();
 }
 
@@ -388,6 +428,11 @@
                                                          const double* __restrict__ rhs, double* __restrict__ yout, size_t bsM, size_t bsL, size_t bsR,
                                                          const long long* __restrict__ btab, const int* __restrict__ own, const int* __restrict__ list) {
   potrf_panel_body<4>(M, ld, k0, nb, Dinv_out, flag, rhs, yout, bsM, bsL, bsR, btab, own, list);
+}
+__global__ __launch_bounds__(64 * NW) void k_potrf_leaf(double* __restrict__ M, double* __restrict__ Dinv_out, int* flag, double* __restrict__ rhs,
+                                                        double* __restrict__ yout, size_t bsL, size_t bsR, const long long* __restrict__ btab,
+                                                        const int* __restrict__ own, const int* __restrict__ stdim, int nI) {
+  potrf_panel_body<16, true>(M, 0, 0, PROWS / 2 / PB, Dinv_out, flag, rhs, yout, 0, bsL, bsR, btab, own, nullptr, stdim, nI);
 }
 
 struct TrsmSubArgs {
@@ -1238,6 +1283,14 @@
                        list + n_big);
 }
 
+void launch_potrf_leaf(double* S, double* Linv, int* flag, double* b, int npad, int nbt, size_t sL, size_t sR, hipStream_t st, const long long* btab,
+                       const int* own, const int* stdim, int nI) {
+  static std::atomic<unsigned long long> seen{0};
+  if (first_use_on_device(seen)) (void)hipFuncSetAttribute(reinterpret_cast<const void*>(k_potrf_leaf), hipFuncAttributeMaxDynamicSharedMemorySize, (int)kPanelLds);
+  form_hit(KF_POTRF_PANEL); form_hit(KF_POTRF_PANEL_FRONTS, nbt); form_hit(KF_POTRF_LEAF, nbt);
+  hipLaunchKernelGGL(k_potrf_leaf, dim3(nbt), dim3(64 * NW), kPanelLds, st, S, Linv, flag, b, b + npad, sL, sR, btab, own, stdim, nI);
+}
+
 void launch_trsm_sub(double* S, size_t ld, int t0, int w, int r0, int r1, const double* Linv, double* b, int npad, int nbt, size_t sM, size_t sL,
                      size_t sR, const int* live, int tI, hipStream_t st, bool chain, const long long* btab, int nb, const int* own) {
   if (r1 <= r0 || nb == 0) return;
diff --git a/covins_amd/csrc/leaf_front.hpp b/covins_amd/csrc/leaf_front.hpp
--- /dev/null
+++ b/covins_amd/csrc/leaf_front.hpp
@@ -0,0 +1,32 @@
+#pragma once
+
+#if defined(__HIPCC__)
+#define COV_LEAF_HD __host__ __device__ __forceinline__
+#else
+#define COV_LEAF_HD inline
+#endif
+
+namespace covgpu {
+
+constexpr int kLeafBlock = 16;
+constexpr int kLeafRows = 256;
+constexpr int kLeafMaxFronts = 384;
+
+COV_LEAF_HD int leaf_blocks(int order) { return (order + kLeafBlock - 1) / kLeafBlock; }
+COV_LEAF_HD bool leaf_front_fits(int own, int st) {
+  return own >= 1 && st >= 0 && own <= kLeafRows / 2 && st <= kLeafRows / 2 && own + st <= kLeafRows &&
+         leaf_blocks(own) + leaf_blocks(st) <= kLeafRows / kLeafBlock;
+}
+COV_LEAF_HD int leaf_border_shift(int nbo, int nI) { return nI - kLeafBlock * nbo; }
+COV_LEAF_HD int leaf_phys_row(int r, int nown, int bshift) { return r >= nown ? r + bshift : r; }
+
+inline bool leaf_level_eligible(int n, const int* own_dim, const int* st_dim, const int* own_ptr, const int* own_var) {
+  if (n < 1 || n > kLeafMaxFronts) return false;
+  for (int k = 0; k < n; ++k) {
+    if (!leaf_front_fits(own_dim[k], st_dim[k])) return false;
+    for (int q = own_ptr[k]; q < own_ptr[k + 1]; ++q) if ((own_var[q] & 1) == 0) return false;
+  }
+  return true;
+}
+
+}
diff --git a/covins_amd/csrc/nd_tables.hip b/covins_amd/csrc/nd_tables.hip
--- a/covins_amd/csrc/nd_tables.hip
+++ b/covins_amd/csrc/nd_tables.hip
@@ -1,6 +1,7 @@
 #include <algorithm>
 
 #include "common.hpp"
+#include "leaf_front.hpp"
 #include "nd_plan.hpp"
 
 namespace covgpu {
@@ -87,6 +88,16 @@
         if (real > 128) ++L.pbig[P]; else if (real > 0) ++L.psmall[P];
       }
   }
+  bool leaf_one_level(const std::vector<int>& nodes) const {
+    if (sh || nlev < 2) return false;
+    std::vector<int> od, sd, ptr{0}, var;
+    for (int n : nodes) {
+      od.push_back(hp.own_dims[n]); sd.push_back(hp.st_dims[n]);
+      var.insert(var.end(), hp.own[n].begin(), hp.own[n].end());
+      ptr.push_back((int)var.size());
+    }
+    return leaf_level_eligible((int)nodes.size(), od.data(), sd.data(), ptr.data(), var.data());
+  }
   void front_layout() {
     dev.h_ndepth.resize(nl); dev.h_nI.resize(nl); dev.h_ntab.resize(2 * (size_t)nl);
     dev.h_own_dims.resize(nl); dev.h_st_dims.resize(nl); dev.h_own_g.resize(nl); dev.h_st_g.resize(nl);
@@ -103,6 +114,7 @@
       for (int n : lnodes[l]) lay_front(L, n, i++, moff);
       L.linv_off = loff; loff += (size_t)L.n * L.nI * kTile;
       panel_lists(L);
+      if (l == 0) L.leaf_one = leaf_one_level(lnodes[l]);
     }
     if (Hs >= nlev) dev.M_sub = moff;
     dev.M_elems = moff; dev.linv_elems = loff;
diff --git a/covins_amd/csrc/solver.hip b/covins_amd/csrc/solver.hip
--- a/covins_amd/csrc/solver.hip
+++ b/covins_amd/csrc/solver.hip
@@ -152,11 +152,19 @@
     launch_imu_gather(P, 1, side);
     launch_finalize_diag(P, mu, 1, side);
   }
+  bool leaves_early = false;
+  if (P.nd && P.vi && nd_leaves_beside_pass(c->nd)) {
+    c->chol.record(c->chol.ev_sb, side, 7);
+    c->chol.wait(c->chol.head, c->chol.ev_sb);
+    FormScope census(&c->chol.forms);
+    leaves_early = launch_nd_leaves(P, c->nd, c->chol.head, c->chol);
+    c->chol.record(c->chol.ev_leaf, c->chol.head, 8);
+  }
   launch_edge_build(P, side);
   launch_lm_build(P, mu, c->st, c->chol.ev_fill, side, c->chol.ev_lin, c->chol.ev_kf, &c->chol);
   if (forked) launch_part_finish(P, SC_COST, 1, side);
   c->chol.record(c->chol.ev_kf, side, 4);
-  c->chol.wait(c->st, c->chol.ev_kf);
+  c->chol.wait(c->st, c->chol.ev_kf, leaves_early ? c->chol.ev_leaf : nullptr);
   if (P.vi && !c->edge_beside_imu) launch_pose_finish(P, mu, c->st);
   else {
     launch_imu_gather(P, 0, c->st);
```

After: 329.7 (median of 6 runs). +2.1%, better.
